# Vi-Sri/CerebralSignalNetworks

Measured on AMD Instinct MI355X. Metric: EEG-segments/sec training (128ch x 500, hidden=768), higher is better.
Workload: dtype bf16

## Files before the change

### cerebralsignalnetworks_amd/cabi.py

```python
import ctypes
import os

import torch

_HERE = os.path.dirname(os.path.abspath(__file__))
LIB_PATH = os.environ.get("CSN_LIB_PATH") or os.path.join(_HERE, "lib", "libcsn_hip.so")

CSN_F32, CSN_BF16 = 0, 1
STATUS_TIMEOUT, STATUS_NONFINITE, STATUS_STALE_SLOT = 1, 2, 4
ABI_VERSION = 6
LSTM_STATE = 0x100
GRAD_OVERWRITE, GRAD_ACCUMULATE = 0, 1

_c_void_p, _c_int, _c_i64, _c_size_t, _c_float = (ctypes.c_void_p, ctypes.c_int, ctypes.c_int64,
                                                  ctypes.c_size_t, ctypes.c_float)


class LstmDesc(ctypes.Structure):
    _fields_ = [("B", ctypes.c_int32), ("T", ctypes.c_int32), ("I", ctypes.c_int32),
                ("H", ctypes.c_int32), ("L", ctypes.c_int32), ("dtype", ctypes.c_int32)]


SIGNATURES = {
    "csn_abi_version": (_c_int, []),
    "csn_last_error": (ctypes.c_char_p, []),
    "csn_target_arch": (ctypes.c_char_p, []),
    "csn_eeg_bandpass_znorm": (_c_int, [_c_void_p, _c_int, _c_int, _c_int, ctypes.POINTER(ctypes.c_double), _c_int,
                                        _c_int, _c_void_p, _c_int, _c_int, _c_void_p]),
    "csn_eeg_filtfilt_scratch_bytes": (_c_size_t, [_c_int, _c_int, _c_int, _c_int]),
    "csn_eeg_filtfilt": (_c_int, [_c_void_p, _c_int, _c_int, _c_int, ctypes.POINTER(ctypes.c_double), _c_int,
                                  _c_void_p, _c_void_p, _c_void_p]),
    "csn_lstm_plan_create": (_c_int, [ctypes.POINTER(LstmDesc), _c_int, ctypes.POINTER(_c_void_p)]),
    "csn_lstm_plan_destroy": (None, [_c_void_p]),
    "csn_lstm_plan_workspace_bytes": (_c_size_t, [_c_void_p]),
    "csn_lstm_plan_path": (_c_int, [_c_void_p]),
    "csn_lstm_plan_dgates_copies": (_c_int, [_c_void_p]),
    "csn_lstm_plan_half_tile_launches": (_c_int, [_c_void_p, _c_int]),
    "csn_lstm_plan_kernel_name": (ctypes.c_char_p, [_c_void_p, _c_int]),
    "csn_lstm_plan_set_grad_callback": (_c_int, [_c_void_p, _c_void_p, _c_void_p]),
    "csn_lstm_plan_set_grad_mode": (_c_int, [_c_void_p, _c_int]),
    "csn_lstm_plan_set_lengths": (_c_int, [_c_void_p, ctypes.POINTER(ctypes.c_int32)]),
    "csn_lstm_workspace_bytes": (_c_size_t, [ctypes.POINTER(LstmDesc), _c_int]),
    "csn_lstm_forward": (_c_int, [_c_void_p, _c_void_p, _c_i64, _c_i64,
                                  ctypes.POINTER(_c_void_p), ctypes.POINTER(_c_void_p),
                                  ctypes.POINTER(_c_void_p), ctypes.POINTER(_c_void_p),
                                  _c_void_p, _c_void_p,
                                  _c_void_p, _c_void_p, _c_void_p,
                                  _c_void_p, _c_void_p, _c_void_p]),
    "csn_lstm_backward": (_c_int, [_c_void_p, _c_void_p, _c_void_p,
                                   _c_void_p, _c_void_p,
                                   _c_void_p,
                                   ctypes.POINTER(_c_void_p), ctypes.POINTER(_c_void_p),
                                   ctypes.POINTER(_c_void_p), ctypes.POINTER(_c_void_p),
                                   _c_void_p, _c_void_p, _c_void_p, _c_void_p]),
    "csn_lstm_workspace_init": (_c_int, [_c_void_p, _c_void_p, _c_void_p]),
    "csn_lstm_status_clear": (_c_int, [_c_void_p, _c_void_p, _c_void_p]),
    "csn_lstm_status_read": (_c_int, [_c_void_p, _c_void_p, ctypes.POINTER(_c_int)]),
    "csn_lstm_status_raise": (_c_int, [_c_void_p, _c_void_p, _c_void_p]),
    "csn_lstm_profile_enable": (_c_int, [_c_void_p, _c_int]),
    "csn_lstm_profile_read": (_c_int, [_c_void_p, ctypes.POINTER(ctypes.c_double), ctypes.POINTER(_c_int),
                                       ctypes.POINTER(_c_int), ctypes.POINTER(ctypes.c_double), ctypes.POINTER(_c_int),
                                       ctypes.POINTER(_c_int)]),
    "csn_gemm_nt": (_c_int, [_c_void_p, _c_void_p, _c_void_p, _c_void_p, _c_i64, _c_i64, _c_i64,
                             _c_int, _c_int, _c_int, _c_void_p]),
    "csn_gemm_tn_scratch_bytes": (_c_size_t, [_c_i64, _c_i64, _c_i64]),
    "csn_gemm_tn": (_c_int, [_c_void_p, _c_void_p, _c_void_p, _c_i64, _c_i64, _c_i64, _c_int, _c_void_p, _c_void_p]),
    "csn_lstm_cell_forward": (_c_int, [_c_void_p, _c_void_p, _c_void_p, _c_i64, _c_void_p, _c_void_p, _c_void_p,
                                       _c_void_p, _c_int, _c_int, _c_int, _c_void_p]),
    "csn_lstm_cell_backward": (_c_int, [_c_void_p, _c_void_p, _c_void_p, _c_i64, _c_void_p, _c_void_p, _c_void_p,
                                        _c_void_p, _c_void_p, _c_int, _c_int, _c_int, _c_void_p]),
    "csn_cosine_loss_scratch_bytes": (_c_size_t, [_c_int]),
    "csn_cosine_loss": (_c_int, [_c_void_p, _c_void_p, _c_int, _c_int, _c_void_p, _c_void_p, _c_float, _c_void_p, _c_void_p]),
    "csn_rmsprop_step": (_c_int, [_c_void_p, _c_void_p, _c_void_p, _c_i64, _c_float, _c_float, _c_float, _c_void_p]),
    "csn_barlow_offdiag_sqsum": (_c_int, [_c_void_p, _c_int, _c_void_p, _c_void_p]),
    "csn_l2_topk_scratch_bytes": (_c_size_t, [_c_i64, _c_i64]),
    "csn_l2_topk": (_c_int, [_c_void_p, _c_void_p, _c_i64, _c_i64, _c_int, _c_int, _c_void_p, _c_void_p,
                             _c_void_p, _c_void_p]),
}


GRAD_READY_FN = ctypes.CFUNCTYPE(None, ctypes.c_void_p, ctypes.c_int)


class CsnError(RuntimeError):
    pass


_lib = None


def load():
    global _lib
    if _lib is not None:
        return _lib
    if not os.path.exists(LIB_PATH):
        raise CsnError(f"{LIB_PATH} not found: build it with `python -c 'import __graft_entry__ as g; g.build()'` "
                       "(there is no CPU fallback)")
    lib = ctypes.CDLL(LIB_PATH, mode=ctypes.RTLD_LOCAL)
    for name, (res, args) in SIGNATURES.items():
        fn = getattr(lib, name)
        fn.restype, fn.argtypes = res, args
    if lib.csn_abi_version() != ABI_VERSION:
        raise CsnError(f"libcsn_hip.so ABI {lib.csn_abi_version()} != binding ABI {ABI_VERSION}")
    _lib = lib
    return lib


def _check(rc):
    if rc != 0:
        raise CsnError(f"libcsn_hip status {rc}: {load().csn_last_error().decode()}")


def _ptr(t):
    return None if t is None else ctypes.c_void_p(t.data_ptr())


def _stream():
    return ctypes.c_void_p(torch.cuda.current_stream().cuda_stream)


def _dt(dtype):
    if dtype in (torch.float32, "f32", "float32", CSN_F32):
        return CSN_F32
    if dtype in (torch.bfloat16, "bf16", "bfloat16", CSN_BF16):
        return CSN_BF16
    raise CsnError(f"unsupported dtype {dtype}")


def torch_dtype(code):
    return torch.bfloat16 if code == CSN_BF16 else torch.float32

# ... 73 lines not shown
    return h_out, c_out, gates


def lstm_cell_backward(dgates_next, w_hh_t, dy, gates, c, c_prev, dc_carry):
    _need_cuda(gates, c, dc_carry)
    B, G = gates.shape
    H = G // 4
    out = torch.empty_like(gates)
    _check(load().csn_lstm_cell_backward(_ptr(dgates_next), _ptr(w_hh_t), _ptr(dy), H, _ptr(gates), _ptr(c),
                                         _ptr(c_prev), _ptr(dc_carry), _ptr(out), B, H, _dt(gates.dtype), _stream()))
    return out


def _ptr_array(tensors):
    arr = (ctypes.c_void_p * len(tensors))()
    for i, t in enumerate(tensors):
        arr[i] = t.data_ptr()
    return arr


class LstmPlan:

    def __init__(self, B, T, I, H, L, dtype, device, training=True, state=False):
        self.desc = LstmDesc(B, T, I, H, L, _dt(dtype))
        self.training = bool(training)
        self.state = bool(state)
        self.device = torch.device(device)
        lib = load()
        handle = _c_void_p()
        with torch.cuda.device(self.device):
            _check(lib.csn_lstm_plan_create(ctypes.byref(self.desc), int(self.training) | (LSTM_STATE if self.state else 0),
                                            ctypes.byref(handle)))
        self._plan = handle
        nbytes = lib.csn_lstm_plan_workspace_bytes(self._plan)
        self.workspace = torch.empty(nbytes + 256, dtype=torch.uint8, device=self.device)
        off = (-self.workspace.data_ptr()) % 256
        self._ws_ptr = ctypes.c_void_p(self.workspace.data_ptr() + off)
        self.busy = False
        with torch.cuda.device(self.device):
            _check(lib.csn_lstm_workspace_init(self._plan, self._ws_ptr, _stream()))

    def __del__(self):
        plan, self._plan = getattr(self, "_plan", None), None
        if plan and _lib is not None:
            _lib.csn_lstm_plan_destroy(plan)

    def key(self):
        d = self.desc
        return (d.B, d.T, d.I, d.H, d.L, d.dtype, self.training) + ((True,) if self.state else ())

    def path(self):
        return load().csn_lstm_plan_path(self._plan)

    def kernel_names(self):
        lib = load()
        return tuple((lib.csn_lstm_plan_kernel_name(self._plan, k) or b"").decode() for k in (0, 1))

    def set_grad_callback(self, fn):
        if getattr(self, "_grad_cb_fn", None) is fn and (fn is None or getattr(self, "_grad_cb", None) is not None):
            return
        self._grad_cb_fn = fn
        self._grad_cb = GRAD_READY_FN(lambda _user, layer: fn(int(layer))) if fn is not None else None
        _check(load().csn_lstm_plan_set_grad_callback(self._plan, ctypes.cast(self._grad_cb, _c_void_p) if fn is not None
                                                      else None, None))

    def set_grad_mode(self, accumulate):
        _check(load().csn_lstm_plan_set_grad_mode(self._plan, GRAD_ACCUMULATE if accumulate else GRAD_OVERWRITE))

    def set_lengths(self, lengths):
        if lengths is None:
            _check(load().csn_lstm_plan_set_lengths(self._plan, None))
            return
        vals = [int(v) for v in (lengths.tolist() if isinstance(lengths, torch.Tensor) else lengths)]
        if len(vals) != self.desc.B:
            raise CsnError(f"LSTM lengths: {len(vals)} entries for a batch of {self.desc.B}")
        _check(load().csn_lstm_plan_set_lengths(self._plan, (ctypes.c_int32 * len(vals))(*vals)))

    def dgates_copies(self):
        return load().csn_lstm_plan_dgates_copies(self._plan)

    def half_tile_launches(self, which):
        return load().csn_lstm_plan_half_tile_launches(self._plan, which)

    def forward(self, x_bti, w_ih, w_hh, b_ih, b_hh, want_all=False, h0=None, c0=None, want_state=False):
        d = self.desc
        _need_cuda(x_bti)
        if x_bti.dtype != torch.float32 or x_bti.stride(2) != 1:
            x_bti = x_bti.float().contiguous()
        assert x_bti.shape == (d.B, d.T, d.I), (tuple(x_bti.shape), (d.B, d.T, d.I))
        y_last = torch.empty((d.B, d.H), dtype=torch.float32, device=x_bti.device)
        y_all = torch.empty((d.B, d.T, d.H), dtype=torch.float32, device=x_bti.device) if want_all else None
        ws = [[p.detach() for p in group] for group in (w_ih, w_hh, b_ih, b_hh)]
        for group in ws:
            for p in group:
                assert p.dtype == torch.float32 and p.is_contiguous() and p.is_cuda
        h0, c0 = self._state_in(h0), self._state_in(c0)
        h_n = torch.empty((d.L, d.B, d.H), dtype=torch.float32, device=x_bti.device) if want_state else None
        c_n = torch.empty((d.L, d.B, d.H), dtype=torch.float32, device=x_bti.device) if want_state else None
        with torch.cuda.device(self.device):
            _check(load().csn_lstm_forward(self._plan, _ptr(x_bti), x_bti.stride(0), x_bti.stride(1),
                                           _ptr_array(ws[0]), _ptr_array(ws[1]), _ptr_array(ws[2]), _ptr_array(ws[3]),
                                           _ptr(h0), _ptr(c0), self._ws_ptr, _ptr(y_last), _ptr(y_all),
                                           _ptr(h_n), _ptr(c_n), _stream()))
        if want_state:
            return y_last, y_all, h_n, c_n
        return y_last, y_all

    def _state_in(self, t):
        if t is None:
            return None
        d = self.desc
        t = t.detach()
        if tuple(t.shape) != (d.L, d.B, d.H):
            raise CsnError(f"LSTM state must be [L, B, H] = {[d.L, d.B, d.H]}, got {list(t.shape)}")
        return t.to(device=self.device, dtype=torch.float32).contiguous()

    def backward(self, dy_last, dy_all, grads, dx=None, dh_n=None, dc_n=None, dh0=None, dc0=None):
        if dy_last is not None:
            dy_last = dy_last.float().contiguous()
        if dy_all is not None:
            dy_all = dy_all.float().contiguous()
        dh_n, dc_n = self._state_in(dh_n), self._state_in(dc_n)
        for out in (dh0, dc0):
            if out is not None:
                assert out.dtype == torch.float32 and out.is_contiguous() and out.shape == (self.desc.L, self.desc.B,
                                                                                            self.desc.H)
        with torch.cuda.device(self.device):
            _check(load().csn_lstm_backward(self._plan, _ptr(dy_last), _ptr(dy_all), _ptr(dh_n), _ptr(dc_n), self._ws_ptr,
                                            _ptr_array(grads[0]), _ptr_array(grads[1]), _ptr_array(grads[2]),
                                            _ptr_array(grads[3]), _ptr(dx), _ptr(dh0), _ptr(dc0), _stream()))

    def clear_status(self):
        with torch.cuda.device(self.device):
            _check(load().csn_lstm_status_clear(self._plan, self._ws_ptr, _stream()))

    def inject_timeout(self):
        with torch.cuda.device(self.device):
            _check(load().csn_lstm_status_raise(self._plan, self._ws_ptr, _stream()))

    def status(self, clear=False):
        out = _c_int(0)
        _check(load().csn_lstm_status_read(self._plan, self._ws_ptr, ctypes.byref(out)))
        if clear and out.value != 0:
            self.clear_status()
        return out.value

    def profile_enable(self, on=True):
        _check(load().csn_lstm_profile_enable(self._plan, int(on)))

    def profile_read(self):
        fm, bm = ctypes.c_double(), ctypes.c_double()
        fl, fc, bl, bc = _c_int(), _c_int(), _c_int(), _c_int()
        _check(load().csn_lstm_profile_read(self._plan, ctypes.byref(fm), ctypes.byref(fl), ctypes.byref(fc),
                                            ctypes.byref(bm), ctypes.byref(bl), ctypes.byref(bc)))
        return dict(fwd_ms=fm.value, fwd_launches=fl.value, fwd_cells=fc.value,
                    bwd_ms=bm.value, bwd_launches=bl.value, bwd_cells=bc.value)


def cosine_loss(student, teacher, want_grad=True, grad_scale=1.0):
    _need_cuda(student, teacher)
    s, t = student.float().contiguous(), teacher.float().contiguous()
    B, D = s.shape
    loss = torch.empty(1, dtype=torch.float32, device=s.device)
    ds = torch.empty_like(s) if want_grad else None
    lib = load()
    scratch = torch.empty(lib.csn_cosine_loss_scratch_bytes(B) // 8, dtype=torch.float64, device=s.device)
    with torch.cuda.device(s.device):
        _check(lib.csn_cosine_loss(_ptr(s), _ptr(t), B, D, _ptr(loss), _ptr(ds), float(grad_scale), _ptr(scratch), _stream()))
    return loss, ds


def rmsprop_step(params_flat, grads_flat, square_avg_flat, lr, alpha=0.99, eps=1e-8):
    _need_cuda(params_flat, grads_flat, square_avg_flat)
    n = params_flat.numel()
    assert grads_flat.numel() == n and square_avg_flat.numel() == n
    assert params_flat.dtype == grads_flat.dtype == square_avg_flat.dtype == torch.float32
    with torch.cuda.device(params_flat.device):
        _check(load().csn_rmsprop_step(_ptr(params_flat), _ptr(grads_flat), _ptr(square_avg_flat), n, float(lr), float(alpha),
                                       float(eps), _stream()))


def barlow_offdiag_sqsum(c):
    _need_cuda(c)
    if c.dim() != 2 or c.shape[0] != c.shape[1]:
        raise CsnError(f"barlow_offdiag_sqsum expects a square matrix, got shape {tuple(c.shape)}")
    c = c.float().contiguous()
# ... 18 lines not shown
```

### cerebralsignalnetworks_amd/csrc/csn_common.h

```cpp
#pragma once
#include <hip/hip_runtime.h>
#include <stdint.h>
#include <stdio.h>
#include <stdlib.h>
#include <atomic>
#include <string>

#include "../../include/csn_hip.h"

namespace csn {

typedef __bf16 bf16_t;
typedef __attribute__((ext_vector_type(8))) __bf16 bf16x8;
typedef __attribute__((ext_vector_type(4))) __bf16 bf16x4;
typedef __attribute__((ext_vector_type(4))) float f32x4;
typedef __attribute__((ext_vector_type(4))) short s16x4;

void set_error(const std::string& msg);
int fail(int status, const char* fmt, ...);

#define CSN_HIP_CHECK(expr)                                                              \
  do {                                                                                   \
    hipError_t _e = (expr);                                                              \
    if (_e != hipSuccess)                                                                \
      return ::csn::fail(CSN_ERR_HIP, "%s failed: %s (%s:%d)", #expr, hipGetErrorString(_e), \
                         __FILE__, __LINE__);                                            \
  } while (0)

#define CSN_LAUNCH_CHECK()                                                               \
  do {                                                                                   \
    hipError_t _e = hipGetLastError();                                                   \
    if (_e != hipSuccess)                                                                \
      return ::csn::fail(CSN_ERR_HIP, "kernel launch failed: %s (%s:%d)",                \
                         hipGetErrorString(_e), __FILE__, __LINE__);                     \
  } while (0)

#define CSN_REQUIRE(cond, ...)                                                           \
  do {                                                                                   \
    if (!(cond)) return ::csn::fail(CSN_ERR_INVALID_ARGUMENT, __VA_ARGS__);              \
  } while (0)

struct Options {
  bool cell_v1, no_persist, no_persist_bwd, persist_streams, no_xcd_local, no_rotate, no_fuse_x, no_beside,
      no_side_stream, gemm_slot, fwd_ksplit, fwd_nsplit, fwd_flags, bwd_flags, dpoll_no_hint, fwd_hint, gemm_no_dma, gemm_no_256, gemm_generic, gemm_lds64, tn_no_tr, tn_no_stagger, filter_v1, tags_no_rearm, gemm_no_192, no_half_tiles;
  int chunk;
  int tn_stages;
  int fwd_nk;
};
static inline Options options_from_env() {
  auto on = [](const char* name) { return getenv(name) != nullptr; };
  auto num = [](const char* name, int dflt) {
    const char* e = getenv(name);
    return e ? atoi(e) : dflt;
  };
  Options o{};
  o.cell_v1 = on("CSN_CELL_V1");
  o.no_persist = on("CSN_NO_PERSIST");
  o.no_persist_bwd = on("CSN_NO_PERSIST_BWD");
  o.persist_streams = on("CSN_PERSIST_STREAMS");
  o.no_xcd_local = on("CSN_NO_XCD_LOCAL");
  o.no_rotate = on("CSN_NO_ROTATE");
  o.no_fuse_x = on("CSN_NO_FUSE_X");
  o.no_beside = on("CSN_NO_BESIDE");
  o.no_half_tiles = on("CSN_NO_HALF_TILES");
  o.no_side_stream = on("CSN_NO_SIDE_STREAM");
  o.gemm_slot = on("CSN_GEMM_SLOT");
  o.fwd_ksplit = on("CSN_FWD_KSPLIT");
  o.fwd_nsplit = on("CSN_FWD_NSPLIT");
  o.fwd_flags = on("CSN_FWD_FLAGS");
  o.bwd_flags = on("CSN_BWD_FLAGS");
  o.dpoll_no_hint = on("CSN_DPOLL_NO_HINT");
  o.fwd_hint = on("CSN_FWD_HINT");
  o.tn_no_stagger = on("CSN_TN_NO_STAGGER");
  o.gemm_no_dma = on("CSN_GEMM_NO_DMA");
  o.gemm_no_256 = on("CSN_GEMM_NO_256");
  o.gemm_no_192 = on("CSN_GEMM_NO_192");
  o.gemm_generic = on("CSN_GEMM_GENERIC");
  o.gemm_lds64 = on("CSN_GEMM_LDS64");
  o.tn_no_tr = on("CSN_TN_NO_TR");
  o.filter_v1 = on("CSN_FILTER_V1");
#ifdef CSN_SLAB_TAGS
  o.tags_no_rearm = on("CSN_TAGS_NO_REARM");
#endif
  o.chunk = num("CSN_LSTM_CHUNK", 32);
  if (o.chunk < 1) o.chunk = 1;
  o.tn_stages = num("CSN_TN_STAGES", 4);
  o.fwd_nk = num("CSN_FWD_NK", 1);
  return o;
}

static inline hipStream_t as_stream(csnStream_t s) { return reinterpret_cast<hipStream_t>(s); }
template <auto Kernel>
static int ensure_dyn_lds(int bytes) {
  static std::atomic<unsigned> done{0u};
  int dev = 0;
  CSN_HIP_CHECK(hipGetDevice(&dev));
  const unsigned bit = 1u << (dev & 31);
  if ((done.load(std::memory_order_acquire) & bit) == 0u) {
    CSN_HIP_CHECK(hipFuncSetAttribute(reinterpret_cast<const void*>(Kernel), hipFuncAttributeMaxDynamicSharedMemorySize, bytes));
    done.fetch_or(bit, std::memory_order_release);
  }
  return CSN_OK;
}

static inline size_t align_up(size_t v, size_t a) { return (v + a - 1) / a * a; }
static inline size_t dtype_size(int dtype) { return dtype == CSN_BF16 ? 2 : 4; }

__device__ __forceinline__ float to_f32(float v) { return v; }
__device__ __forceinline__ float to_f32(bf16_t v) { return (float)v; }
template <typename T> __device__ __forceinline__ T from_f32(float v);
template <> __device__ __forceinline__ float from_f32<float>(float v) { return v; }
template <> __device__ __forceinline__ bf16_t from_f32<bf16_t>(float v) { return (bf16_t)v; }

__device__ __forceinline__ float sigmoid_f32(float x) { return 1.0f / (1.0f + expf(-x)); }
__device__ __forceinline__ float tanh_f32(float x) { return tanhf(x); }

struct CellFwdOne {
  const void* h_prev; const void* w_hh; const float* xproj; int64_t xproj_ld; const float* c_prev;
  void* gates_out; float* c_out; void* h_out;
};
struct CellFwdBatch { CellFwdOne p[4]; };
struct CellBwdOne {
  const void* dg_next; const void* w_hh_t; const float* dy; int64_t dy_ld; const void* gates; const float* c;
  const float* c_prev; float* dc_carry; void* dg_out;
};
struct CellBwdBatch { CellBwdOne p[4]; };
struct CellMask {
  const int* lengths;
  int t[4];
};
struct CellNoMask {};
template <bool MASK> struct CellMaskArg { typedef CellNoMask type; };
template <> struct CellMaskArg<true> { typedef CellMask type; };
int launch_cell_fwd_batch(const CellFwdBatch& b, int np, int B, int H, int dtype, hipStream_t st);
int launch_cell_bwd_batch(const CellBwdBatch& b, int np, int B, int H, int dtype, hipStream_t st,
                          const CellMask* mask = nullptr);

int launch_cast_strided(const float* src, int64_t s0, int64_t s1, int64_t n0, int64_t n1, int64_t n2,
                        void* dst, int dtype, hipStream_t st);
int launch_transpose_cast(const float* src, int64_t R, int64_t C, void* dst, int dtype, hipStream_t st);
int launch_cast(const float* src, void* dst, int64_t n, int dtype, hipStream_t st);
int launch_upcast(const void* src, int dtype, float* dst, int64_t n, hipStream_t st);
int launch_add_vec(const float* a, const float* b, float* out, int64_t n, hipStream_t st);
int launch_reduce_slabs(const float* slabs, int64_t stride, int S, float* out, float* out2, int64_t n, int accumulate,
                        hipStream_t st);
size_t colsum_scratch_bytes(int64_t N);
int launch_colsum(const void* X, int64_t R, int64_t N, int dtype, float* out, float* out2, int accumulate, void* scratch,
// ... 13 lines not shown
```

### cerebralsignalnetworks_amd/csrc/lstm.hip

```cpp
#include <algorithm>
#include <cstring>
#include <vector>

#include "csn_common.h"
#include "lstm_cell_blk.h"
#include "lstm_cell_common.h"
#include "lstm_f32_persist.h"

namespace csn {

int launch_cell_fwd(const void* h_prev, const void* w_hh, const float* xproj, int64_t xproj_ld, const float* c_prev,
                    void* gates_out, float* c_out, void* h_out, int B, int H, int dtype, hipStream_t st);
int launch_cell_bwd(const void* dg_next, const void* w_hh_t, const float* dy, int64_t dy_ld, const void* gates,
                    const float* c, const float* c_prev, float* dc_carry, void* dg_out, int B, int H, int dtype,
                    hipStream_t st);

struct LayerWs {
  size_t wih, whh, whht, wiht, whh_blk, whht_blk, bias, xproj, gates, c_all, h_all, dgates, dx, dc_carry, hblk[2],
      dgblk[2], h_blk_all, counters, dg_blk_all, bflags;
};
struct WsLayout {
  LayerWs layer[8];
  size_t x_c, x_blk, wih0_blk, dy_tm, tn_scratch, colsum, status, agree, agree_b, zeros_bh, f32_bias_part, total;
  size_t zero_fwd, zero_fwd_bytes, zero_bwd, zero_bwd_bytes;
  bool fuse_x;
  bool il, persist, persist_bwd;
  bool fwd_ns;
  bool f32_persist;
};

static bool whole_chip() {
  int dev = 0, cus = 0;
  if (hipGetDevice(&dev) != hipSuccess) return false;
  return hipDeviceGetAttribute(&cus, hipDeviceAttributeMultiprocessorCount, dev) == hipSuccess && cus >= 256;
}

static WsLayout make_layout(const csnLstmDesc& d, int training, const Options& opt) {
  WsLayout w{};
  w.il = cell_blk_supported(d.H, d.dtype, opt);
  const bool slabs_fit = ((size_t)d.T + 1) * (((size_t)d.B + 63) / 64 * 64) * (size_t)d.H * 8 < ((size_t)1 << 32);
  w.fwd_ns = w.il && fwd_ns_supported(d.B, d.H, d.dtype, opt) && d.L <= 4;
  w.persist = w.fwd_ns || (w.il && slabs_fit && fwd_persist_supported(d.B, d.H, d.dtype, opt) && d.L <= 4);
  w.persist_bwd = w.persist && slabs_fit && training && bwd_persist_supported(d.B, d.H, d.dtype, opt);
  size_t off = 0;
  const size_t es = dtype_size(d.dtype);
  auto take = [&](size_t bytes) {
    size_t o = off;
    off += align_up(bytes, 256);
    return o;
  };
  const size_t TB = (size_t)d.T * d.B, H = d.H, G = 4 * (size_t)d.H;
  const size_t Bpad = ((size_t)d.B + 63) / 64 * 64;
  size_t tn_bytes = 0;
  for (int l = 0; l < d.L; ++l) {
    const size_t I = l == 0 ? d.I : d.H;
    LayerWs& L = w.layer[l];
    L.wih = take(G * I * es);
    L.wiht = take(G * I * es);
    L.bias = take(G * 4);
    if (w.il) {
      L.whh_blk = take(G * H * 2);
      L.whht_blk = take(G * H * 2);
      L.hblk[0] = take(Bpad * H * 2);
      L.hblk[1] = take(Bpad * H * 2);
      if (w.persist) L.h_blk_all = take(((size_t)(d.T < 3 ? 3 : d.T) + 1) * Bpad * H * 2);
    } else {
      L.whh = take(G * H * es);
      L.whht = take(G * H * es);
    }
    L.xproj = take(TB * G * 4);
    L.gates = take(TB * G * es);
    L.c_all = take((TB + d.B) * H * 4);
    L.h_all = take((TB + d.B) * H * es);
    if (training) {
      L.dgates = take(TB * G * es);
      L.dx = take(TB * I * 4);
      if (!w.persist_bwd) L.dc_carry = take((size_t)d.B * H * 4);
      if (w.il) {
        L.dgblk[0] = take(Bpad * G * 2);
        L.dgblk[1] = take(Bpad * G * 2);
      }
      if (w.persist_bwd) L.dg_blk_all = take((size_t)(d.T < 4 ? 4 : d.T) * Bpad * G * 2);
    }
    size_t a = gemm_tn_scratch_bytes(G, I, TB, opt), b = gemm_tn_scratch_bytes(G, H, TB, opt);
    if (a > tn_bytes) tn_bytes = a;
    if (b > tn_bytes) tn_bytes = b;
  }
  w.x_c = take(TB * d.I * es);
  w.status = take(256);
  w.fuse_x = w.persist && !opt.no_fuse_x &&
             (w.fwd_ns ? d.I == 128 : (d.I % 32 == 0 && d.I <= 128 && d.H != 512));
  if (w.fuse_x) {
    w.x_blk = take((size_t)d.T * Bpad * d.I * 2);
    w.wih0_blk = take(G * d.I * 2);
  }
  if (w.persist_bwd) w.zeros_bh = take((size_t)d.B * H * 4);
  w.f32_persist = !w.il && d.dtype == CSN_F32 && !opt.no_persist && !opt.cell_v1 && f32_persist_supported(d.B, d.H) && whole_chip();
  if (w.f32_persist) {
    const size_t MTt = Bpad / 64;
    w.zero_fwd = off;
    for (int l = 0; l < d.L; ++l) w.layer[l].counters = take(((size_t)d.T + 1) * MTt * kF32FlagLine * 4);
    w.zero_fwd_bytes = off - w.zero_fwd;
    for (int l = 0; l < d.L; ++l) w.layer[l].h_blk_all = take(((size_t)d.T + 1) * Bpad * H * 4);
    if (training) {
      for (int l = 0; l < d.L; ++l) w.layer[l].dg_blk_all = take((size_t)d.T * Bpad * G * 4);
      w.zeros_bh = take((size_t)d.B * H * 4);
      w.f32_bias_part = take(MTt * 4 * G * 4);
      w.zero_bwd = off;
      for (int l = 0; l < d.L; ++l) w.layer[l].bflags = take((size_t)d.T * MTt * kF32FlagLine * 4);
      w.zero_bwd_bytes = off - w.zero_bwd;
    }
  }
  if (w.persist) {
    w.zero_fwd = off;
    for (int l = 0; l < d.L; ++l) w.layer[l].counters = take(((size_t)d.T + 1) * (Bpad / 64) * 4 * kPersistFlagLine * 4);
    w.agree = take(((size_t)d.T + 8) * 8 * sizeof(unsigned long long));
    w.zero_fwd_bytes = off - w.zero_fwd;
  }
  if (w.persist_bwd) {
    w.zero_bwd = off;
    for (int l = 0; l < d.L; ++l) {
      w.layer[l].dc_carry = take((size_t)d.B * H * 4);
      w.layer[l].bflags = take((size_t)d.T * (Bpad / 64) * 3 * kPersistFlagLine * 4);
    }
    w.agree_b = take(((size_t)d.T + 8) * 8 * sizeof(unsigned long long));
    w.zero_bwd_bytes = off - w.zero_bwd;
  }
  if (training) {
    w.dy_tm = take(TB * H * 4);
    w.tn_scratch = take(tn_bytes);
    w.colsum = take(colsum_scratch_bytes(G));
  }
  w.total = off;
  return w;
}

static int check_desc(const char* fn, const csnLstmDesc* d) {
  CSN_REQUIRE(d != nullptr, "%s: null descriptor", fn);
  CSN_REQUIRE(d->B > 0 && d->T > 0 && d->I > 0 && d->H > 0, "%s: bad shape B=%d T=%d I=%d H=%d", fn, d->B, d->T,
              d->I, d->H);
  CSN_REQUIRE(d->L >= 1 && d->L <= 8, "%s: L=%d outside 1..8", fn, d->L);
  CSN_REQUIRE(d->H % 32 == 0, "%s: H=%d must be a multiple of 32", fn, d->H);
  CSN_REQUIRE(d->dtype == CSN_F32 || d->dtype == CSN_BF16, "%s: bad dtype %d", fn, d->dtype);
  return CSN_OK;
}

template <typename T>
__global__ void gather_y_all_kernel(const T* __restrict__ h_all, float* __restrict__ y, int B, int Tn, int H) {
  const int64_t total = (int64_t)B * Tn * H;
  const int64_t stride = (int64_t)gridDim.x * blockDim.x;
  for (int64_t i = (int64_t)blockIdx.x * blockDim.x + threadIdx.x; i < total; i += stride) {
    const int64_t h = i % H, r = i / H, t = r % Tn, b = r / Tn;
    y[i] = to_f32(h_all[((t + 1) * B + b) * (int64_t)H + h]);
  }
}

__global__ void bt_to_tb_kernel(const float* __restrict__ src, float* __restrict__ dst, int B, int Tn, int H) {
  const int64_t total = (int64_t)B * Tn * H;
  const int64_t stride = (int64_t)gridDim.x * blockDim.x;
  for (int64_t i = (int64_t)blockIdx.x * blockDim.x + threadIdx.x; i < total; i += stride) {
    const int64_t h = i % H, r = i / H, b = r % B, t = r / B;
    dst[i] = src[(b * Tn + t) * (int64_t)H + h];
  }
}

__global__ void tb_to_bt_kernel(const float* __restrict__ src, float* __restrict__ dst, int B, int Tn, int H) {
  const int64_t total = (int64_t)B * Tn * H;
// ... 137 lines not shown
  hipStream_t layer[8] = {nullptr};
  std::vector<hipEvent_t> events;
  size_t next = 0;
};

static int side_ctx(SideCtx& c) {
  if (c.side == nullptr) {
    CSN_HIP_CHECK(hipStreamCreateWithFlags(&c.side, hipStreamNonBlocking));
    for (int l = 1; l < 8; ++l) CSN_HIP_CHECK(hipStreamCreateWithFlags(&c.layer[l], hipStreamNonBlocking));
  }
  c.next = 0;
  return CSN_OK;
}
static int next_event(SideCtx* c, hipEvent_t* ev) {
  if (c->next == c->events.size()) {
    hipEvent_t e;
    CSN_HIP_CHECK(hipEventCreateWithFlags(&e, hipEventDisableTiming));
    c->events.push_back(e);
  }
  *ev = c->events[c->next++];
  return CSN_OK;
}
static int hand_off(SideCtx* c, hipStream_t from, hipStream_t to) {
  hipEvent_t ev;
  if (int rc = next_event(c, &ev)) return rc;
  CSN_HIP_CHECK(hipEventRecord(ev, from));
  CSN_HIP_CHECK(hipStreamWaitEvent(to, ev, 0));
  return CSN_OK;
}

struct Prof {
  bool on = false;
  hipEvent_t ev[4] = {nullptr, nullptr, nullptr, nullptr};
  int launches[2] = {0, 0}, cells[2] = {0, 0};
  bool have[2] = {false, false};
  std::vector<hipEvent_t> pair[2];
  size_t pairs_used[2] = {0, 0};
};
static int prof_mark(Prof& g_prof, int which, hipStream_t st) {
  if (!g_prof.on) return CSN_OK;
  if ((which & 1) == 0) g_prof.pairs_used[which >> 1] = 0;
  if (g_prof.ev[which] == nullptr) CSN_HIP_CHECK(hipEventCreate(&g_prof.ev[which]));
  CSN_HIP_CHECK(hipEventRecord(g_prof.ev[which], st));
  return CSN_OK;
}

static int prof_pair(Prof& g_prof, int k, bool end, hipStream_t st) {
  if (!g_prof.on) return CSN_OK;
  const size_t i = 2 * g_prof.pairs_used[k] + (end ? 1 : 0);
  while (g_prof.pair[k].size() <= i) {
    hipEvent_t e;
    CSN_HIP_CHECK(hipEventCreate(&e));
    g_prof.pair[k].push_back(e);
  }
  CSN_HIP_CHECK(hipEventRecord(g_prof.pair[k][i], st));
  if (end) ++g_prof.pairs_used[k];
  return CSN_OK;
}

}

struct csnLstmPlan {
  csnLstmDesc d;
  int training;
  int state;
  bool state_seen = false;
  int device;
  csn::Options opt;
  csn::WsLayout w;
  csn::SideCtx sc;
  csn::Prof prof;
  int dgates_copies = 0;
  int half_launches[2] = {0, 0};
  csnGradReadyFn grad_cb = nullptr;
  void* grad_cb_user = nullptr;
  int grad_accumulate = 0;
  std::vector<int32_t> lengths;
  int t_eff = 0;
  int T_full = 0;
  const int* dlen = nullptr;
  int32_t* len_dev = nullptr;
  int32_t* len_pin = nullptr;
  hipEvent_t len_ev = nullptr;
  void grads_ready(int layer) const {
    if (grad_cb != nullptr) grad_cb(grad_cb_user, layer);
  }
};

using namespace csn;
typedef csnLstmPlan Plan;

extern "C" int csn_lstm_plan_create(const csnLstmDesc* d, int training, csnLstmPlan** out) {
  if (int rc = check_desc("csn_lstm_plan_create", d)) return rc;
  CSN_REQUIRE(out != nullptr, "csn_lstm_plan_create: null output pointer");
  Plan* P = new Plan();
  P->d = *d;
  P->state = (training & CSN_LSTM_STATE) != 0;
  P->training = (training & ~CSN_LSTM_STATE) != 0;
  if (hipGetDevice(&P->device) != hipSuccess) {
    delete P;
    return fail(CSN_ERR_HIP, "csn_lstm_plan_create: hipGetDevice failed");
  }
  P->opt = options_from_env();
  if (P->state && d->dtype == CSN_F32) P->opt.no_persist = true;
  {
    const unsigned long long Bp = ((unsigned long long)d->B + 63) / 64 * 64;
    const unsigned long long per_step = std::max({(unsigned long long)d->B * d->H * 16ull, Bp * (unsigned long long)d->I * 2ull, Bp * (unsigned long long)d->H * 2ull});
    const unsigned long long cmax = ((1ull << 32) - 1ull) / per_step;
    if (cmax >= 3 && (unsigned long long)P->opt.chunk > cmax - 2) P->opt.chunk = (int)(cmax - 2);
  }
  P->w = make_layout(*d, P->training, P->opt);
  P->T_full = d->T;
  *out = P;
  return CSN_OK;
}

extern "C" void csn_lstm_plan_destroy(csnLstmPlan* P) {
  if (P == nullptr) return;
  int cur = 0;
  const bool switched = hipGetDevice(&cur) == hipSuccess && cur != P->device && hipSetDevice(P->device) == hipSuccess;
  for (hipEvent_t e : P->sc.events) (void)hipEventDestroy(e);
  if (P->sc.side) (void)hipStreamDestroy(P->sc.side);
  for (int l = 1; l < 8; ++l)
    if (P->sc.layer[l]) (void)hipStreamDestroy(P->sc.layer[l]);
  for (int i = 0; i < 4; ++i)
    if (P->prof.ev[i]) (void)hipEventDestroy(P->prof.ev[i]);
  for (int k = 0; k < 2; ++k)
    for (hipEvent_t e : P->prof.pair[k]) (void)hipEventDestroy(e);
  if (P->len_ev) (void)hipEventDestroy(P->len_ev);
  if (P->len_pin) (void)hipHostFree(P->len_pin);
  if (P->len_dev) (void)hipFree(P->len_dev);
  if (switched) (void)hipSetDevice(cur);
  delete P;
}

extern "C" size_t csn_lstm_plan_workspace_bytes(const csnLstmPlan* P) { return P ? P->w.total : 0; }

extern "C" int csn_lstm_plan_path(const csnLstmPlan* P) {
  if (P == nullptr) return -1;
  return P->w.f32_persist ? 4 : (P->w.persist_bwd ? 3 : (P->w.persist ? 2 : (P->w.il ? 1 : 0)));
}

extern "C" int csn_lstm_plan_dgates_copies(const csnLstmPlan* P) { return P == nullptr ? -1 : P->dgates_copies; }

extern "C" int csn_lstm_plan_half_tile_launches(const csnLstmPlan* P, int which) {
  return (P == nullptr || which < 0 || which > 1) ? -1 : P->half_launches[which];
}

static bool bwd_grouped(const csnLstmPlan* P) {
  if (!P->w.persist_bwd) return false;
  const int MTg = (P->d.B + 63) / 64, nchg = (P->d.T + P->opt.chunk - 1) / P->opt.chunk;
  const int slots = P->d.L < nchg ? P->d.L : nchg;
  return slots <= 4 && slots * MTg <= 8 && !P->opt.persist_streams;
}

extern "C" const char* csn_lstm_plan_kernel_name(const csnLstmPlan* P, int which) {
  if (P == nullptr) return nullptr;
  const bool ks = (P->d.dtype == CSN_F32 ? P->d.H % 128 == 0 : P->d.H % 256 == 0);
  if (P->w.f32_persist) return which == 0 ? "lstm_fwd_f32_persist_kernel" : (which == 1 ? "lstm_bwd_f32_persist_kernel" : nullptr);
  if (which == 0) {
    if (P->w.fwd_ns) return "lstm_fwd_ns_kernel";
    if (P->w.persist) return "lstm_fwd_persist_kernel";
    if (P->w.il) return "lstm_cell_fwd_il_kernel";
    return ks ? "lstm_cell_fwd_ks_kernel" : "lstm_cell_fwd_kernel";
  }
  if (which == 1) {
    if (bwd_grouped(P)) return "lstm_bwd_persist_kernel";
    if (P->w.il) return "lstm_cell_bwd_il_kernel";
    return ks ? "lstm_cell_bwd_ks_kernel" : "lstm_cell_bwd_kernel";
  }
  return nullptr;
}

extern "C" int csn_lstm_plan_set_grad_callback(csnLstmPlan* P, csnGradReadyFn fn, void* user) {
  CSN_REQUIRE(P != nullptr, "csn_lstm_plan_set_grad_callback: null plan");
  P->grad_cb = fn;
  P->grad_cb_user = fn ? user : nullptr;
  return CSN_OK;
}

extern "C" int csn_lstm_plan_set_grad_mode(csnLstmPlan* P, int mode) {
  CSN_REQUIRE(P != nullptr, "csn_lstm_plan_set_grad_mode: null plan");
  CSN_REQUIRE(mode == CSN_GRAD_OVERWRITE || mode == CSN_GRAD_ACCUMULATE, "csn_lstm_plan_set_grad_mode: unknown mode %d", mode);
  P->grad_accumulate = mode == CSN_GRAD_ACCUMULATE;
  return CSN_OK;
}

extern "C" int csn_lstm_plan_set_lengths(csnLstmPlan* P, const int32_t* lengths) {
  CSN_REQUIRE(P != nullptr, "csn_lstm_plan_set_lengths: null plan");
  CSN_REQUIRE(P->state, "csn_lstm_plan_set_lengths: the plan was created without CSN_LSTM_STATE");
  if (lengths == nullptr) {
    P->lengths.clear();
    P->t_eff = 0;
    return CSN_OK;
  }
  int longest = 0;
  for (int b = 0; b < P->d.B; ++b) {
    CSN_REQUIRE(lengths[b] >= 0 && lengths[b] <= P->d.T, "csn_lstm_plan_set_lengths: lengths[%d] = %d outside [0, %d]", b,
                (int)lengths[b], P->d.T);
    longest = std::max(longest, (int)lengths[b]);
  }
  P->lengths.assign(lengths, lengths + P->d.B);
  P->t_eff = longest;
  return CSN_OK;
}

struct EffectiveT {
  csnLstmDesc& d;
  const int T;
  EffectiveT(csnLstmDesc& d_, int Te) : d(d_), T(d_.T) { d.T = Te; }
  ~EffectiveT() { d.T = T; }
};
static int upload_lengths(csnLstmPlan* P, hipStream_t st) {
  P->dlen = nullptr;
  if (P->lengths.empty()) return CSN_OK;
  const size_t bytes = (size_t)P->d.B * 4;
  if (P->len_pin == nullptr) {
    CSN_HIP_CHECK(hipMalloc((void**)&P->len_dev, bytes));
    CSN_HIP_CHECK(hipHostMalloc((void**)&P->len_pin, bytes, hipHostMallocDefault));
    CSN_HIP_CHECK(hipEventCreateWithFlags(&P->len_ev, hipEventDisableTiming));
  } else {
    CSN_HIP_CHECK(hipEventSynchronize(P->len_ev));
  }
  memcpy(P->len_pin, P->lengths.data(), bytes);
  CSN_HIP_CHECK(hipMemcpyAsync(P->len_dev, P->len_pin, bytes, hipMemcpyHostToDevice, st));
  CSN_HIP_CHECK(hipEventRecord(P->len_ev, st));
  P->dlen = P->len_dev;
  return CSN_OK;
}
static int emit_dx(const csnLstmPlan& P, const float* dx_tm, float* dx, int64_t I, hipStream_t st) {
  const int B = P.d.B, T = P.d.T;
// ... 27 lines not shown
              "csn_lstm_profile_read: null pointer");
  Prof& g_prof = P->prof;
  *fwd_ms = *bwd_ms = 0.0;
  *fwd_launches = *fwd_cells = *bwd_launches = *bwd_cells = 0;
  for (int k = 0; k < 2; ++k) {
    if (!g_prof.have[k]) continue;
    float ms = 0.f;
    CSN_HIP_CHECK(hipEventSynchronize(g_prof.ev[2 * k + 1]));
    if (g_prof.pairs_used[k] > 0) {
      for (size_t i = 0; i < g_prof.pairs_used[k]; ++i) {
        float one = 0.f;
        CSN_HIP_CHECK(hipEventElapsedTime(&one, g_prof.pair[k][2 * i], g_prof.pair[k][2 * i + 1]));
        ms += one;
      }
    } else {
      CSN_HIP_CHECK(hipEventElapsedTime(&ms, g_prof.ev[2 * k], g_prof.ev[2 * k + 1]));
    }
    (k == 0 ? *fwd_ms : *bwd_ms) = ms;
    (k == 0 ? *fwd_launches : *bwd_launches) = g_prof.launches[k];
    (k == 0 ? *fwd_cells : *bwd_cells) = g_prof.cells[k];
  }
  return CSN_OK;
}

extern "C" int csn_lstm_workspace_init(const csnLstmPlan* P, void* workspace, csnStream_t stream) {
  CSN_REQUIRE(P && workspace, "csn_lstm_workspace_init: null pointer");
  CSN_REQUIRE((reinterpret_cast<uintptr_t>(workspace) & 255) == 0, "csn_lstm_workspace_init: workspace must be 256-B aligned");
  hipStream_t st = as_stream(stream);
  char* ws = (char*)workspace;
  const WsLayout& w = P->w;
  const size_t es = dtype_size(P->d.dtype);
  CSN_HIP_CHECK(hipMemsetAsync(ws + w.status, 0, 256, st));
  for (int l = 0; l < P->d.L; ++l) {
    CSN_HIP_CHECK(hipMemsetAsync(ws + w.layer[l].h_all, 0, (size_t)P->d.B * P->d.H * es, st));
    CSN_HIP_CHECK(hipMemsetAsync(ws + w.layer[l].c_all, 0, (size_t)P->d.B * P->d.H * 4, st));
  }
  if (w.persist_bwd || (w.f32_persist && P->training))
    CSN_HIP_CHECK(hipMemsetAsync(ws + w.zeros_bh, 0, (size_t)P->d.B * P->d.H * 4, st));
  return CSN_OK;
}

extern "C" int csn_lstm_status_clear(const csnLstmPlan* P, void* workspace, csnStream_t stream) {
  CSN_REQUIRE(P && workspace, "csn_lstm_status_clear: null pointer");
  CSN_HIP_CHECK(hipMemsetAsync((char*)workspace + P->w.status, 0, 256, as_stream(stream)));
  return CSN_OK;
}
extern "C" int csn_lstm_status_raise(const csnLstmPlan* P, void* workspace, csnStream_t stream) {
  CSN_REQUIRE(P && workspace, "csn_lstm_status_raise: null pointer");
  CSN_HIP_CHECK(hipMemsetAsync((char*)workspace + P->w.status, 1, 1, as_stream(stream)));
  return CSN_OK;
}
extern "C" int csn_lstm_status_read(const csnLstmPlan* P, const void* workspace, int* status) {
  CSN_REQUIRE(P && workspace && status, "csn_lstm_status_read: null pointer");
  unsigned flag[3] = {0u, 0u, 0u};
  CSN_HIP_CHECK(hipMemcpy(flag, (const char*)workspace + P->w.status, sizeof(flag), hipMemcpyDeviceToHost));
  *status = (flag[0] ? CSN_STATUS_TIMEOUT : 0) | (flag[1] ? CSN_STATUS_NONFINITE : 0) | (flag[2] ? CSN_STATUS_STALE_SLOT : 0);
#ifdef CSN_SLAB_TAGS
  if (flag[2] && getenv("CSN_TAGS_VERBOSE")) {
    unsigned dbg[24];
    CSN_HIP_CHECK(hipMemcpy(dbg, (const char*)workspace + P->w.status + 28, sizeof(dbg), hipMemcpyDeviceToHost));
    if (dbg[0])
      fprintf(stderr, "stale piece (backward): t=%u step-in-launch=%u group=%u slice=%u wave=%u lane=%u kb*4+rg=%u u0=%08x local=%u redone=%u "
              "single=%u phase=%u rot=%u nsteps=%u xcc=%u lanes=%u\n", dbg[1], dbg[2], dbg[3], dbg[4], dbg[5], dbg[6], dbg[7], dbg[8],
              dbg[9], dbg[10], dbg[11], dbg[12], dbg[13], dbg[14], dbg[15], dbg[16]);
  }
#endif
  return CSN_OK;
}

extern "C" size_t csn_lstm_workspace_bytes(const csnLstmDesc* d, int training) {
  if (check_desc("csn_lstm_workspace_bytes", d) != CSN_OK) return 0;
  Options opt = options_from_env();
  if ((training & CSN_LSTM_STATE) && d->dtype == CSN_F32) opt.no_persist = true;
  return make_layout(*d, (training & ~CSN_LSTM_STATE) != 0, opt).total;
}

static int gemm_tn_full(const void* A, const void* B, float* C, int64_t M, int64_t N, int64_t K, int dtype, void* scratch,
                        int accumulate, hipStream_t st, const Options& opt) {
  int S = 1;
  if (int rc = launch_gemm_tn_slabs(A, B, (float*)scratch, M, N, K, dtype, st, &S, nullptr, nullptr, opt)) return rc;
  return launch_reduce_slabs((const float*)scratch, M * N, S, C, nullptr, M * N, accumulate, st);
}

static int mask_x(const csnLstmPlan& P, char* ws, hipStream_t st) {
  if (P.dlen == nullptr) return CSN_OK;
  const csnLstmDesc& d = P.d;
  const int64_t n = (int64_t)d.T * d.B * d.I;
  if (d.dtype == CSN_BF16) mask_tm_kernel<bf16_t><<<grid_for(n), 256, 0, st>>>((bf16_t*)(ws + P.w.x_c), P.dlen, d.B, d.T, d.I);
  else mask_tm_kernel<float><<<grid_for(n), 256, 0, st>>>((float*)(ws + P.w.x_c), P.dlen, d.B, d.T, d.I);
  CSN_LAUNCH_CHECK();
  if (P.w.fuse_x) {
    const int64_t Bpad = ((int64_t)d.B + 63) / 64 * 64;
    mask_x_blk_kernel<<<grid_for((int64_t)d.T * Bpad * d.I / 8), 256, 0, st>>>((bf16_t*)(ws + P.w.x_blk), P.dlen, d.B, Bpad, d.T, d.I);
    CSN_LAUNCH_CHECK();
  }
  return CSN_OK;
}

static int forward_v1(Plan& P, char* ws, const float* x, int64_t xsb, int64_t xst,
                      const float* const* w_ih, const float* const* w_hh, const float* const* b_ih,
                      const float* const* b_hh, const float* h0, const float* c0, int training, csnStream_t stream) {
  const csnLstmDesc* d = &P.d;
  const WsLayout& w = P.w;
  hipStream_t st = as_stream(stream);
  const int B = d->B, T = d->T, H = d->H, dt = d->dtype, NL = d->L;
  const int64_t G = 4 * (int64_t)H, TB = (int64_t)T * B;
  const size_t es = dtype_size(dt);
  const int Cz = P.opt.chunk, lag = Cz;
  int rc;
  if ((rc = launch_cast_strided(x, xsb, xst, B, T, d->I, ws + w.x_c, dt, st))) return rc;
  if ((rc = mask_x(P, ws, st))) return rc;
  for (int l = 0; l < NL; ++l) {
    const LayerWs& L = w.layer[l];
    const int64_t I = l == 0 ? d->I : H;
    if ((rc = launch_cast(w_ih[l], ws + L.wih, G * I, dt, st))) return rc;
    if ((rc = launch_cast(w_hh[l], ws + L.whh, G * H, dt, st))) return rc;
    if (training) {
      if ((rc = launch_transpose_cast(w_hh[l], G, H, ws + L.whht, dt, st))) return rc;
      if ((rc = launch_transpose_cast(w_ih[l], G, I, ws + L.wiht, dt, st))) return rc;
    }
    if ((rc = launch_add_vec(b_ih[l], b_hh[l], (float*)(ws + L.bias), G, st))) return rc;
    if (h0) {
      if ((rc = launch_cast(h0 + (size_t)l * B * H, ws + L.h_all, (int64_t)B * H, dt, st))) return rc;
    } else {
      CSN_HIP_CHECK(hipMemsetAsync(ws + L.h_all, 0, (size_t)B * H * es, st));
    }
    if (c0)
      CSN_HIP_CHECK(hipMemcpyAsync(ws + L.c_all, c0 + (size_t)l * B * H, (size_t)B * H * 4, hipMemcpyDeviceToDevice, st));
    else
      CSN_HIP_CHECK(hipMemsetAsync(ws + L.c_all, 0, (size_t)B * H * 4, st));
  }
  if ((rc = gemm_nt(ws + w.x_c, ws + w.layer[0].wih, (const float*)(ws + w.layer[0].bias), ws + w.layer[0].xproj, TB, G,
                    d->I, dt, CSN_F32, 0, st, P.opt)))
    return rc;
  const int D = T + lag * (NL - 1);
  for (int dg = 0; dg < D; ++dg) {
    CellFwdBatch b{};
    int np = 0;
    for (int l = 0; l < NL; ++l) {
      const int t = dg - lag * l;
      if (t < 0 || t >= T) continue;
      const LayerWs& L = w.layer[l];
      if (np == 4) {
        if ((rc = launch_cell_fwd_batch(b, np, B, H, dt, st))) return rc;
        np = 0;
      }
      b.p[np++] = CellFwdOne{ws + L.h_all + (size_t)t * B * H * es, ws + L.whh, (const float*)(ws + L.xproj) + (size_t)t * B * G, G,
                             (const float*)(ws + L.c_all) + (size_t)t * B * H,
                             training ? ws + L.gates + (size_t)t * B * G * es : nullptr,
                             (float*)(ws + L.c_all) + (size_t)(t + 1) * B * H, ws + L.h_all + (size_t)(t + 1) * B * H * es};
    }
    if (np > 0 && (rc = launch_cell_fwd_batch(b, np, B, H, dt, st))) return rc;
    for (int l = 0; l + 1 < NL; ++l) {
      const int t = dg - lag * l;
      if (t < 0 || t >= T || ((t + 1) % Cz != 0 && t != T - 1)) continue;
      const int t0 = (t / Cz) * Cz, nsteps = t - t0 + 1;
      const LayerWs& Ln = w.layer[l + 1];
      if ((rc = gemm_nt(ws + w.layer[l].h_all + (size_t)(t0 + 1) * B * H * es, ws + Ln.wih, (const float*)(ws + Ln.bias),
                        (float*)(ws + Ln.xproj) + (size_t)t0 * B * G, (int64_t)nsteps * B, G, H, dt, CSN_F32, 0, st, P.opt)))
        return rc;
    }
  }
  return CSN_OK;
}

static int backward_v1(Plan& P, char* ws, const float* dy_last, const float* dy_tm, const float* dh_n, const float* dc_n,
                       float* const* dw_ih, float* const* dw_hh, float* const* db_ih, float* const* db_hh, float* dx,
                       csnStream_t stream) {
  const csnLstmDesc* d = &P.d;
  const WsLayout& w = P.w;
  hipStream_t st = as_stream(stream);
  const int B = d->B, T = d->T, H = d->H, dt = d->dtype, NL = d->L;
  const int64_t G = 4 * (int64_t)H, TB = (int64_t)T * B;
  const size_t es = dtype_size(dt);
  const int Cz = P.opt.chunk, lag = Cz;
  const int acc = P.grad_accumulate;
  int rc;
  for (int l = 0; l < NL; ++l) {
    if (dc_n)
      CSN_HIP_CHECK(hipMemcpyAsync(ws + w.layer[l].dc_carry, dc_n + (size_t)l * B * H, (size_t)B * H * 4, hipMemcpyDeviceToDevice, st));
    else
      CSN_HIP_CHECK(hipMemsetAsync(ws + w.layer[l].dc_carry, 0, (size_t)B * H * 4, st));
  }
  const int D = T + lag * (NL - 1);
  for (int dg = 0; dg < D; ++dg) {
    CellBwdBatch b{};
    CellMask mask{P.dlen, {0, 0, 0, 0}};
    const CellMask* mk = P.dlen ? &mask : nullptr;
    int np = 0;
    for (int l = NL - 1; l >= 0; --l) {
      const int r = dg - lag * (NL - 1 - l);
      if (r < 0 || r >= T) continue;
      const int t = T - 1 - r;
      const LayerWs& L = w.layer[l];
      const bool top = (l == NL - 1);
      if (np == 4) {
        if ((rc = launch_cell_bwd_batch(b, np, B, H, dt, st, mk))) return rc;
        np = 0;
      }
      mask.t[np] = t;
      const float* dy_t = top ? (dy_tm ? dy_tm + (size_t)t * B * H : (t == T - 1 ? dy_last : nullptr))
                              : (const float*)(ws + w.layer[l + 1].dx) + (size_t)t * B * H;
      b.p[np++] = CellBwdOne{(t == T - 1) ? nullptr : (const void*)(ws + L.dgates + (size_t)(t + 1) * B * G * es), ws + L.whht, dy_t, H,
                             ws + L.gates + (size_t)t * B * G * es, (const float*)(ws + L.c_all) + (size_t)(t + 1) * B * H,
                             (const float*)(ws + L.c_all) + (size_t)t * B * H, (float*)(ws + L.dc_carry),
                             ws + L.dgates + (size_t)t * B * G * es};
    }
    if (np > 0 && (rc = launch_cell_bwd_batch(b, np, B, H, dt, st, mk))) return rc;
    for (int l = NL - 1; l >= 1; --l) {
      const int r = dg - lag * (NL - 1 - l);
      if (r < 0 || r >= T || ((r + 1) % Cz != 0 && r != T - 1)) continue;
      const int t_lo = T - 1 - r, t_hi = T - 1 - (r / Cz) * Cz;
      const LayerWs& L = w.layer[l];
      if ((rc = gemm_nt(ws + L.dgates + (size_t)t_lo * B * G * es, ws + L.wiht, nullptr, (float*)(ws + L.dx) + (size_t)t_lo * B * H,
                        (int64_t)(t_hi - t_lo + 1) * B, H, G, dt, CSN_F32, 0, st, P.opt)))
        return rc;
      if (dh_n && (rc = add_dh_n_rows(P, dh_n + (size_t)(l - 1) * B * H, (float*)(ws + L.dx), t_lo, t_hi, st))) return rc;
    }
  }
  for (int l = NL - 1; l >= 0; --l) {
    const LayerWs& L = w.layer[l];
    const int64_t I = l == 0 ? d->I : H;
    const void* inp = l == 0 ? (const void*)(ws + w.x_c)
                             : (const void*)(ws + w.layer[l - 1].h_all + (size_t)B * H * es);
    if ((rc = gemm_tn_full(ws + L.dgates, ws + L.h_all, dw_hh[l], G, H, TB, dt, ws + w.tn_scratch, acc, st, P.opt))) return rc;
    if ((rc = gemm_tn_full(ws + L.dgates, inp, dw_ih[l], G, I, TB, dt, ws + w.tn_scratch, acc, st, P.opt))) return rc;
    if ((rc = launch_colsum(ws + L.dgates, TB, G, dt, db_ih[l], db_hh[l], acc, ws + w.colsum, st))) return rc;
    P.grads_ready(l);
  }
  if (dx) {
    const LayerWs& L = w.layer[0];
    if ((rc = gemm_nt(ws + L.dgates, ws + L.wiht, nullptr, ws + L.dx, TB, d->I, G, dt, CSN_F32, 0, st, P.opt))) return rc;
    if ((rc = emit_dx(P, (const float*)(ws + L.dx), dx, d->I, st))) return rc;
  }
  return CSN_OK;
}

static int forward_f32p(Plan& P, char* ws, const float* x, int64_t xsb, int64_t xst,
                        const float* const* w_ih, const float* const* w_hh, const float* const* b_ih,
                        const float* const* b_hh, int training, csnStream_t stream) {
  const csnLstmDesc* d = &P.d;
  const WsLayout& w = P.w;
  Prof& g_prof = P.prof;
  hipStream_t st = as_stream(stream);
  const int B = d->B, T = d->T, H = d->H, NL = d->L;
  const int64_t G = 4 * (int64_t)H, TB = (int64_t)T * B;
  const int MTt = (B + 63) / 64, per = f32_persist_tiles_per_launch(H);
  int rc;
  if ((rc = launch_cast_strided(x, xsb, xst, B, T, d->I, ws + w.x_c, CSN_F32, st))) return rc;
  for (int l = 0; l < NL; ++l) {
    const LayerWs& L = w.layer[l];
    const int64_t I = l == 0 ? d->I : H;
    if ((rc = launch_cast(w_ih[l], ws + L.wih, G * I, CSN_F32, st))) return rc;
    if ((rc = launch_cast(w_hh[l], ws + L.whh, G * H, CSN_F32, st))) return rc;
    if (training) {
      if ((rc = launch_transpose_cast(w_hh[l], G, H, ws + L.whht, CSN_F32, st))) return rc;
      if ((rc = launch_transpose_cast(w_ih[l], G, I, ws + L.wiht, CSN_F32, st))) return rc;
    }
    if ((rc = launch_add_vec(b_ih[l], b_hh[l], (float*)(ws + L.bias), G, st))) return rc;
    CSN_HIP_CHECK(hipMemsetAsync(ws + L.h_all, 0, (size_t)B * H * 4, st));
    CSN_HIP_CHECK(hipMemsetAsync(ws + L.c_all, 0, (size_t)B * H * 4, st));
  }
  CSN_HIP_CHECK(hipMemsetAsync(ws + w.zero_fwd, 0, w.zero_fwd_bytes, st));
  int n_launch = 0;
  if ((rc = prof_mark(g_prof, 0, st))) return rc;
  for (int l = 0; l < NL; ++l) {
    const LayerWs& L = w.layer[l];
    const void* inp = l == 0 ? (const void*)(ws + w.x_c) : (const void*)(ws + w.layer[l - 1].h_all + (size_t)B * H * 4);
    if ((rc = gemm_nt(inp, ws + L.wih, (const float*)(ws + L.bias), ws + L.xproj, TB, G, l == 0 ? d->I : H, CSN_F32, CSN_F32, 0, st, P.opt)))
      return rc;
    F32PersistFwdArgs a{};
    a.w_hh = (const float*)(ws + L.whh);
    a.xproj = (const float*)(ws + L.xproj);
    a.gates = training ? (float*)(ws + L.gates) : nullptr;
    a.c_all = (float*)(ws + L.c_all);
    a.h_all = (float*)(ws + L.h_all);
    a.h_blk = (float*)(ws + L.h_blk_all);
    a.flags = (unsigned*)(ws + L.counters);
    a.error_flag = (unsigned*)(ws + w.status);
    a.B = B; a.T = T; a.MT_total = MTt;
    for (int m = 0; m < MTt; m += per) {
      a.mt0 = m;
      a.MT = MTt - m < per ? MTt - m : per;
      if ((rc = prof_pair(g_prof, 0, false, st))) return rc;
      if ((rc = launch_fwd_f32_persist(a, H, st))) return rc;
      if ((rc = prof_pair(g_prof, 0, true, st))) return rc;
      ++n_launch;
    }
  }
  if ((rc = prof_mark(g_prof, 1, st))) return rc;
  g_prof.launches[0] = n_launch;
  g_prof.cells[0] = T * NL;
  g_prof.have[0] = g_prof.on;
  return CSN_OK;
}

static int backward_f32p(Plan& P, char* ws, const float* dy_last, const float* dy_tm,
                         float* const* dw_ih, float* const* dw_hh, float* const* db_ih, float* const* db_hh, float* dx,
                         csnStream_t stream) {
  const csnLstmDesc* d = &P.d;
  const WsLayout& w = P.w;
  Prof& g_prof = P.prof;
  hipStream_t st = as_stream(stream);
  const int B = d->B, T = d->T, H = d->H, NL = d->L;
  const int64_t G = 4 * (int64_t)H, TB = (int64_t)T * B;
  const int MTt = (B + 63) / 64, per = f32_persist_tiles_per_launch(H);
  int rc;
  CSN_HIP_CHECK(hipMemsetAsync(ws + w.zero_bwd, 0, w.zero_bwd_bytes, st));
  int n_launch = 0;
  if ((rc = prof_mark(g_prof, 2, st))) return rc;
  for (int l = NL - 1; l >= 0; --l) {
    const LayerWs& L = w.layer[l];
    const bool top = (l == NL - 1);
    F32PersistBwdArgs a{};
    a.w_hh_t = (const float*)(ws + L.whht);
    a.gates = (const float*)(ws + L.gates);
    a.c_all = (const float*)(ws + L.c_all);
    a.dy = top ? dy_tm : (const float*)(ws + w.layer[l + 1].dx);
    a.dy_last = (top && dy_tm == nullptr) ? dy_last : nullptr;
    a.zeros = (const float*)(ws + w.zeros_bh);
    a.dgates = (float*)(ws + L.dgates);
    a.dg_blk = (float*)(ws + L.dg_blk_all);
    a.bias_part = (float*)(ws + w.f32_bias_part);
    a.flags = (unsigned*)(ws + L.bflags);
    a.error_flag = (unsigned*)(ws + w.status);
    a.B = B; a.T = T; a.MT_total = MTt;
    for (int m = 0; m < MTt; m += per) {
      a.mt0 = m;
      a.MT = MTt - m < per ? MTt - m : per;
      if ((rc = prof_pair(g_prof, 1, false, st))) return rc;
      if ((rc = launch_bwd_f32_persist(a, H, st))) return rc;
      if ((rc = prof_pair(g_prof, 1, true, st))) return rc;
      ++n_launch;
    }
    sum_rows_kernel<<<(unsigned)((G + 255) / 256), 256, 0, st>>>((const float*)(ws + w.f32_bias_part), MTt * 4, G, db_ih[l], db_hh[l], P.grad_accumulate);
    CSN_LAUNCH_CHECK();
    if (l > 0 && (rc = gemm_nt(ws + L.dgates, ws + L.wiht, nullptr, ws + L.dx, TB, H, G, CSN_F32, CSN_F32, 0, st, P.opt))) return rc;
  }
  if ((rc = prof_mark(g_prof, 3, st))) return rc;
  g_prof.launches[1] = n_launch;
  g_prof.cells[1] = T * NL;
  g_prof.have[1] = g_prof.on;
  for (int l = NL - 1; l >= 0; --l) {
    const LayerWs& L = w.layer[l];
    const int64_t I = l == 0 ? d->I : H;
    const void* inp = l == 0 ? (const void*)(ws + w.x_c) : (const void*)(ws + w.layer[l - 1].h_all + (size_t)B * H * 4);
    if ((rc = gemm_tn_full(ws + L.dgates, ws + L.h_all, dw_hh[l], G, H, TB, CSN_F32, ws + w.tn_scratch, P.grad_accumulate, st, P.opt))) return rc;
    if ((rc = gemm_tn_full(ws + L.dgates, inp, dw_ih[l], G, I, TB, CSN_F32, ws + w.tn_scratch, P.grad_accumulate, st, P.opt))) return rc;
    P.grads_ready(l);
  }
  if (dx) {
    const LayerWs& L = w.layer[0];
    if ((rc = gemm_nt(ws + L.dgates, ws + L.wiht, nullptr, ws + L.dx, TB, d->I, G, CSN_F32, CSN_F32, 0, st, P.opt))) return rc;
    tb_to_bt_kernel<<<grid_for(TB * d->I), 256, 0, st>>>((const float*)(ws + L.dx), dx, B, T, d->I);
    CSN_LAUNCH_CHECK();
  }
  return CSN_OK;
}

static int forward_persist(Plan& P, char* ws, const float* h0, const float* c0, int training, hipStream_t st, SideCtx* sc,
                           hipStream_t side);

static int forward_il(Plan& P, char* ws, const float* x, int64_t xsb, int64_t xst,
                      const float* const* w_ih, const float* const* w_hh, const float* const* b_ih,
                      const float* const* b_hh, const float* h0, const float* c0, int training, csnStream_t stream) {
  const csnLstmDesc* d = &P.d;
  const WsLayout& w = P.w;
  Prof& g_prof = P.prof;
  hipStream_t st = as_stream(stream);
  SideCtx* sc = &P.sc;
  int rc;
  if ((rc = side_ctx(P.sc))) return rc;
  hipStream_t side = P.opt.no_side_stream ? st : sc->side;
  const int B = d->B, T = d->T, H = d->H, NL = d->L;
  const int64_t G = 4 * (int64_t)H, TB = (int64_t)T * B;
  const size_t Bpad = ((size_t)B + 63) / 64 * 64;
  const int Cz = P.opt.chunk, lag = 2 * Cz;

  PrepArgs pa{};
  int prep_rc = CSN_OK;
  auto job = [&](int kind, const float* a_, const float* b_, void* dst, int64_t n0, int64_t n1, int64_t n2, int64_t s0,
                 int64_t s1, int64_t Hh, int pr, int pk, int64_t work) {
    if (prep_rc != CSN_OK) return;
    if (pa.njobs == kPrepMaxJobs) {
      if ((prep_rc = launch_prep_multi(pa, st)) != CSN_OK) return;
      pa.njobs = 0;
    }
    PrepJob& J = pa.job[pa.njobs++];
    J = PrepJob{kind, a_, b_, dst, n0, n1, n2, s0, s1, Hh, pr, pk, work, 0u, 0u};
  };
  job(kPrepCastX, x, nullptr, ws + w.x_c, B, T, d->I, xsb, xst, 0, 0, 0, TB * d->I);
  for (int l = 0; l < NL; ++l) {
    const LayerWs& L = w.layer[l];
    const int64_t I = l == 0 ? d->I : H;
    job(kPrepPermRows, w_ih[l], nullptr, ws + L.wih, 0, I, 0, 0, 0, H, 0, 0, G * I);
    job(kPrepBlockify, w_hh[l], nullptr, ws + L.whh_blk, G, H, 0, H, 1, H, 1, 0, G * H / 8);
    job(kPrepBias, b_ih[l], b_hh[l], ws + L.bias, 0, 0, 0, 0, 0, H, 0, 0, G);
    if (training) {
      job(kPrepTransPerm, w_ih[l], nullptr, ws + L.wiht, 0, I, 0, 0, 0, H, 0, 0, G * I);
      job(kPrepBlockify, w_hh[l], nullptr, ws + L.whht_blk, H, G, 0, 1, H, H, 0, 1, H * G / 8);
    }
    if (!w.persist) {
      CSN_HIP_CHECK(hipMemsetAsync(ws + L.hblk[0], 0, Bpad * H * 2, st));
      CSN_HIP_CHECK(hipMemsetAsync(ws + L.hblk[1], 0, Bpad * H * 2, st));
      CSN_HIP_CHECK(hipMemsetAsync(ws + L.h_all, 0, (size_t)B * H * 2, st));
      CSN_HIP_CHECK(hipMemsetAsync(ws + L.c_all, 0, (size_t)B * H * 4, st));
      if (h0) {
        if ((rc = launch_blockify_x(h0 + (size_t)l * B * H, H, 0, B, 1, H, ws + L.hblk[0], st))) return rc;
        if ((rc = launch_cast(h0 + (size_t)l * B * H, ws + L.h_all, (int64_t)B * H, CSN_BF16, st))) return rc;
      }
      if (c0)
        CSN_HIP_CHECK(hipMemcpyAsync(ws + L.c_all, c0 + (size_t)l * B * H, (size_t)B * H * 4, hipMemcpyDeviceToDevice, st));
    }
  }
  if (w.fuse_x) {
    job(kPrepBlockifyX, x, nullptr, ws + w.x_blk, B, T, d->I, xsb, xst, (int64_t)Bpad, 0, 0, (int64_t)T * Bpad * d->I / 8);
    job(kPrepBlockify, w_ih[0], nullptr, ws + w.wih0_blk, G, d->I, 0, d->I, 1, H, 1, 0, G * d->I / 8);
  }
  if (prep_rc != CSN_OK) return prep_rc;
  if ((rc = launch_prep_multi(pa, st))) return rc;
  if ((rc = mask_x(P, ws, st))) return rc;
  if (!w.fuse_x) {
    if ((rc = gemm_nt(ws + w.x_c, ws + w.layer[0].wih, (const float*)(ws + w.layer[0].bias), ws + w.layer[0].xproj,
                          TB, G, d->I, CSN_BF16, CSN_F32, 0, st, P.opt)))
      return rc;
  }
  if (w.persist) return forward_persist(P, ws, h0, c0, training, st, sc, side);
  if (NL > 1 && (rc = hand_off(sc, st, side))) return rc;

  const int nch = (T + Cz - 1) / Cz;
  std::vector<hipEvent_t> xproj_ready((size_t)NL * nch, nullptr);
  const int D = T + lag * (NL - 1);
  int n_launch = 0, n_cells = 0;
  if ((rc = prof_mark(g_prof, 0, st))) return rc;
  for (int dg = 0; dg < D; ++dg) {
    CellFwdArgs a{};
    a.B = B;
    a.H = H;
    int np = 0;
    for (int l = 0; l < NL; ++l) {
      const int t = dg - lag * l;
      if (t < 0 || t >= T) continue;
      const LayerWs& L = w.layer[l];
      if (np == 4) {
        if ((rc = launch_cell_fwd_il(a, np, st, P.opt.fwd_nk))) return rc;
        ++n_launch;
        n_cells += np;
        np = 0;
      }
      if (l > 0 && t % Cz == 0) CSN_HIP_CHECK(hipStreamWaitEvent(st, xproj_ready[(size_t)l * nch + t / Cz], 0));
      CellFwdProb& P = a.p[np++];
      P.h_prev_blk = (t == 0 && !h0) ? nullptr : (const bf16_t*)(ws + L.hblk[t & 1]);
      P.w_blk = (const bf16_t*)(ws + L.whh_blk);
      P.xproj = (const float*)(ws + L.xproj) + (size_t)t * B * G;
      P.c_prev = (t == 0 && !c0) ? nullptr : (const float*)(ws + L.c_all) + (size_t)t * B * H;
      P.gates_out = training ? (bf16_t*)(ws + L.gates) + (size_t)t * B * G : nullptr;
      P.c_out = (float*)(ws + L.c_all) + (size_t)(t + 1) * B * H;
      P.h_out = (bf16_t*)(ws + L.h_all) + (size_t)(t + 1) * B * H;
      P.h_out_blk = (bf16_t*)(ws + L.hblk[(t + 1) & 1]);
    }
    if (np == 0) continue;
    if ((rc = launch_cell_fwd_il(a, np, st, P.opt.fwd_nk))) return rc;
    ++n_launch;
    n_cells += np;
    for (int l = 0; l + 1 < NL; ++l) {
      const int t = dg - lag * l;
      if (t < 0 || t >= T) continue;
      if ((t + 1) % Cz != 0 && t != T - 1) continue;
      const int c = t / Cz, t0 = c * Cz, nsteps = t - t0 + 1;
      if ((rc = hand_off(sc, st, side))) return rc;
      const LayerWs& Ln = w.layer[l + 1];
      rc = gemm_nt((const bf16_t*)(ws + w.layer[l].h_all) + (size_t)(t0 + 1) * B * H, ws + Ln.wih,
                       (const float*)(ws + Ln.bias), (float*)(ws + Ln.xproj) + (size_t)t0 * B * G,
                       (int64_t)nsteps * B, G, H, CSN_BF16, CSN_F32, 0, side, P.opt);
      if (rc) return rc;
      hipEvent_t ev;
      if ((rc = next_event(sc, &ev))) return rc;
      CSN_HIP_CHECK(hipEventRecord(ev, side));
      xproj_ready[(size_t)(l + 1) * nch + c] = ev;
    }
  }
  if ((rc = prof_mark(g_prof, 1, st))) return rc;
  g_prof.launches[0] = n_launch;
  g_prof.cells[0] = n_cells;
  g_prof.have[0] = g_prof.on;
  return CSN_OK;
}

static int forward_persist(Plan& P, char* ws, const float* h0, const float* c0, int training, hipStream_t st, SideCtx* sc,
                           hipStream_t side) {
  const csnLstmDesc* d = &P.d;
  const WsLayout& w = P.w;
  Prof& g_prof = P.prof;
  const int B = d->B, T = d->T, H = d->H, NL = d->L;
  const int64_t G = 4 * (int64_t)H;
  const int Bpad = (B + 63) / 64 * 64, MT = Bpad / 64;
  const int Cz = P.opt.chunk;
  const int nch = (T + Cz - 1) / Cz;
  int rc;
  CSN_HIP_CHECK(hipMemsetAsync(ws + w.zero_fwd, 0, w.zero_fwd_bytes, st));
  auto fill_slot = [&](PersistFwdSlot& S, int l, int c) {
    const LayerWs& L = w.layer[l];
    S.w_blk = (const bf16_t*)(ws + L.whh_blk);
    S.xproj = (const float*)(ws + L.xproj);
    S.gates = training ? (bf16_t*)(ws + L.gates) : nullptr;
    S.c_all = (float*)(ws + L.c_all);
    S.h_all = (bf16_t*)(ws + L.h_all);
    S.h_blk_all = (bf16_t*)(ws + L.h_blk_all);
    S.flags = (unsigned*)(ws + L.counters);
    S.x_blk = nullptr;
    S.wih_blk = nullptr;
    S.bias = nullptr;
    S.I = 0;
    if (l == 0 && w.fuse_x) {
      S.x_blk = (const bf16_t*)(ws + w.x_blk);
      S.wih_blk = (const bf16_t*)(ws + w.wih0_blk);
      S.bias = (const float*)(ws + L.bias);
      S.I = d->I;
    }
    S.t0 = c * Cz;
    S.nsteps = (S.t0 + Cz <= T) ? Cz : T - S.t0;
  };
  auto xproj_gemm = [&](int l, int c, hipStream_t on) {
    const LayerWs& L = w.layer[l];
    const LayerWs& Ln = w.layer[l + 1];
    const int t0 = c * Cz, nsteps = (t0 + Cz <= T) ? Cz : T - t0;
    return gemm_nt((const bf16_t*)(ws + L.h_all) + (size_t)(t0 + 1) * B * H, ws + Ln.wih,
                       (const float*)(ws + Ln.bias), (float*)(ws + Ln.xproj) + (size_t)t0 * B * G,
                       (int64_t)nsteps * B, G, H, CSN_BF16, CSN_F32, 0, on, P.opt);
  };
  PersistFwdArgs a{};
  a.error_flag = (unsigned*)(ws + w.status);
  a.B = B; a.H = H; a.T = T; a.Bpad = Bpad; a.MT = MT;
  a.rotate = !P.opt.no_rotate;
  a.data_polls = (!w.fwd_ns && !P.opt.fwd_flags) ? (P.opt.fwd_hint && !P.opt.dpoll_no_hint ? 1 : 2) : 0;
#ifdef CSN_SLAB_TAGS
  if (a.data_polls && P.opt.tags_no_rearm) a.data_polls |= 4;
#endif
  if (a.data_polls)
    for (int l = 0; l < NL; ++l)
      CSN_HIP_CHECK(hipMemsetAsync(ws + w.layer[l].h_blk_all, 0xff, (size_t)4 * Bpad * H * 2, st));
  a.state = (h0 || c0) ? 1 : 0;
  if (a.state) P.state_seen = true;
  for (int l = 0; l < NL && P.state_seen; ++l) {
    const LayerWs& L = w.layer[l];
    if (h0) {
      if ((rc = launch_blockify_x(h0 + (size_t)l * B * H, H, 0, B, 1, H, ws + L.h_blk_all, st))) return rc;
      if ((rc = launch_cast(h0 + (size_t)l * B * H, ws + L.h_all, (int64_t)B * H, CSN_BF16, st))) return rc;
    } else {
      if (a.state) CSN_HIP_CHECK(hipMemsetAsync(ws + L.h_blk_all, 0, (size_t)Bpad * H * 2, st));
      CSN_HIP_CHECK(hipMemsetAsync(ws + L.h_all, 0, (size_t)B * H * 2, st));
    }
    if (c0)
      CSN_HIP_CHECK(hipMemcpyAsync(ws + L.c_all, c0 + (size_t)l * B * H, (size_t)B * H * 4, hipMemcpyDeviceToDevice, st));
    else
      CSN_HIP_CHECK(hipMemsetAsync(ws + L.c_all, 0, (size_t)B * H * 4, st));
  }
  int n_launch = 0;
  P.half_launches[0] = 0;

  const int max_slots = NL < nch ? NL : nch;
  const int fwd_slices = w.fwd_ns ? fwd_ns_slices(H) : fwd_persist_slices(H);
  auto launch_fwd = [&](const PersistFwdArgs& args, hipStream_t on) {
    return w.fwd_ns ? launch_fwd_ns(args, on) : launch_fwd_persist(args, on);
  };
  const bool grouped = max_slots <= 4 && max_slots * MT <= 8 && fwd_slices <= 32 &&
                       !P.opt.persist_streams;
  if (grouped) {
    const int ndiag = nch + NL - 1;
    const bool try_local = !P.opt.no_xcd_local;
    if ((rc = prof_mark(g_prof, 0, st))) return rc;
    for (int dg = 0; dg < ndiag; ++dg) {
      int lay[4], chk[4], ns = 0;
      for (int l = 0; l < NL; ++l) {
        const int c = dg - l;
        if (c < 0 || c >= nch) continue;
        lay[ns] = l;
        chk[ns] = c;
        fill_slot(a.slot[ns], l, c);
        ++ns;
      }
      a.nslots = ns;
      a.xcd_groups = 1;
      const bool half = !w.fwd_ns && !P.opt.no_half_tiles && 2 * ns * MT <= 8;
      a.half_tiles = half ? 1 : 0;
      a.MT = half ? 2 * MT : MT;
      if (half) {
        for (int i = 0; i < ns; ++i) a.slot[i].flags += ((size_t)T + 1) * MT * kPersistFlagLine;
        ++P.half_launches[0];
      }
      a.agree = try_local ? (unsigned long long*)(ws + w.agree) + (size_t)dg * 8 : nullptr;
      if ((rc = prof_pair(g_prof, 0, false, st))) return rc;
      if ((rc = launch_fwd(a, st))) return rc;
      if ((rc = prof_pair(g_prof, 0, true, st))) return rc;
      ++n_launch;
      for (int i = 0; i < ns; ++i)
        if (lay[i] + 1 < NL && (rc = xproj_gemm(lay[i], chk[i], st))) return rc;
    }
    if ((rc = prof_mark(g_prof, 1, st))) return rc;
    g_prof.launches[0] = n_launch;
    g_prof.cells[0] = T * NL;
    g_prof.have[0] = g_prof.on;
    return CSN_OK;
  }

  if (NL * fwd_slices * MT > 256) side = st;
  hipStream_t ls[8];
  ls[0] = st;
  for (int l = 1; l < NL; ++l) {
    ls[l] = (side == st) ? st : sc->layer[l];
    if (ls[l] != st && (rc = hand_off(sc, st, ls[l]))) return rc;
  }
  if (side != st && (rc = hand_off(sc, st, side))) return rc;
  const bool gemm_slot = P.opt.gemm_slot;
  if ((rc = prof_mark(g_prof, 0, st))) return rc;
  a.nslots = 1;
  a.xcd_groups = 0;
  a.agree = nullptr;
  a.half_tiles = 0;
  a.MT = MT;
  for (int c = 0; c < nch; ++c) {
    for (int l = 0; l < NL; ++l) {
      fill_slot(a.slot[0], l, c);
      if ((rc = launch_fwd(a, ls[l]))) return rc;
      ++n_launch;
      if (l + 1 < NL) {
        if ((rc = hand_off(sc, ls[l], side))) return rc;
        if ((rc = xproj_gemm(l, c, side))) return rc;
        if (side != ls[l + 1] && (rc = hand_off(sc, side, ls[l + 1]))) return rc;
        if (gemm_slot && side != ls[l] && (rc = hand_off(sc, side, ls[l]))) return rc;
      }
    }
  }
  for (int l = 1; l < NL; ++l)
    if (ls[l] != st && (rc = hand_off(sc, ls[l], st))) return rc;
  if (side != st && (rc = hand_off(sc, side, st))) return rc;
  if ((rc = prof_mark(g_prof, 1, st))) return rc;
  g_prof.launches[0] = n_launch;
  g_prof.cells[0] = T * NL;
  g_prof.have[0] = g_prof.on;
  return CSN_OK;
}

static int backward_persist(Plan& P, char* ws, const float* dy_last, const float* dy_tm, const float* dh_n,
                            const float* dc_n, float* const* dw_ih, float* const* dw_hh, float* const* db_ih,
                            float* const* db_hh, float* dx, hipStream_t st);

static int backward_il(Plan& P, char* ws, const float* dy_last, const float* dy_tm, const float* dh_n, const float* dc_n,
                       float* const* dw_ih, float* const* dw_hh, float* const* db_ih, float* const* db_hh, float* dx,
                       csnStream_t stream) {
  const csnLstmDesc* d = &P.d;
  const WsLayout& w = P.w;
  Prof& g_prof = P.prof;
  hipStream_t st = as_stream(stream);
  if (bwd_grouped(&P)) return backward_persist(P, ws, dy_last, dy_tm, dh_n, dc_n, dw_ih, dw_hh, db_ih, db_hh, dx, st);
  SideCtx* sc = &P.sc;
  int rc;
  if ((rc = side_ctx(P.sc))) return rc;
  hipStream_t side = P.opt.no_side_stream ? st : sc->side;
  const int B = d->B, T = d->T, H = d->H, NL = d->L;
  const int64_t G = 4 * (int64_t)H, TB = (int64_t)T * B;
  const size_t Bpad = ((size_t)B + 63) / 64 * 64;
  const int Cz = P.opt.chunk, lag = 2 * Cz;
  const int nch = (T + Cz - 1) / Cz;
  const bool state = P.state != 0;

  for (int l = 0; l < NL; ++l) {
    const LayerWs& L = w.layer[l];
    if (dc_n)
      CSN_HIP_CHECK(hipMemcpyAsync(ws + L.dc_carry, dc_n + (size_t)l * B * H, (size_t)B * H * 4, hipMemcpyDeviceToDevice, st));
    else
      CSN_HIP_CHECK(hipMemsetAsync(ws + L.dc_carry, 0, (size_t)B * H * 4, st));
    CSN_HIP_CHECK(hipMemsetAsync(ws + L.dgblk[0], 0, Bpad * G * 2, st));
    CSN_HIP_CHECK(hipMemsetAsync(ws + L.dgblk[1], 0, Bpad * G * 2, st));
  }
  if ((rc = hand_off(sc, st, side))) return rc;

  auto weight_grads = [&](int l) -> int {
    const LayerWs& L = w.layer[l];
    const int64_t I = l == 0 ? d->I : H;
    const void* inp = l == 0 ? (const void*)(ws + w.x_c)
                             : (const void*)((const bf16_t*)(ws + w.layer[l - 1].h_all) + (size_t)B * H);
    float* slabs = (float*)(ws + w.tn_scratch);
    const int acc = P.grad_accumulate;
    int S = 1, r;
    int cs_done = 0, S_cs = 1;
    if ((r = launch_gemm_tn_slabs(ws + L.dgates, ws + L.h_all, slabs, G, H, TB, CSN_BF16, side, &S, (float*)(ws + w.colsum), &cs_done, P.opt))) return r;
    S_cs = S;
    if ((r = launch_reduce_slabs_unperm(slabs, G * H, S, H, H, dw_hh[l], nullptr, acc, side))) return r;
    if ((r = launch_gemm_tn_slabs(ws + L.dgates, inp, slabs, G, I, TB, CSN_BF16, side, &S, nullptr, nullptr, P.opt))) return r;
    if ((r = launch_reduce_slabs_unperm(slabs, G * I, S, H, I, dw_ih[l], nullptr, acc, side))) return r;
    if (!cs_done) {
      if ((r = launch_colsum_partial(ws + L.dgates, TB, G, CSN_BF16, ws + w.colsum, side))) return r;
      S_cs = colsum_chunks();
    }
    if ((r = launch_reduce_slabs_unperm((const float*)(ws + w.colsum), G, S_cs, H, 1, db_ih[l], db_hh[l], acc, side)))
      return r;
    return CSN_OK;
  };

  std::vector<hipEvent_t> dx_ready((size_t)NL * nch, nullptr);
  const int D = T + lag * (NL - 1);
  int n_launch = 0, n_cells = 0;
  if ((rc = prof_mark(g_prof, 2, st))) return rc;
  for (int dg = 0; dg < D; ++dg) {
    CellBwdArgs a{};
    a.B = B;
    a.H = H;
    CellMask mask{P.dlen, {0, 0, 0, 0}};
    const CellMask* mk = P.dlen ? &mask : nullptr;
    int np = 0;
    for (int l = NL - 1; l >= 0; --l) {
      const int r = dg - lag * (NL - 1 - l);
      if (r < 0 || r >= T) continue;
      const int t = T - 1 - r;
      const LayerWs& L = w.layer[l];
      const bool top = (l == NL - 1);
      if (np == 4) {
        if ((rc = launch_cell_bwd_il(a, np, st, mk))) return rc;
        ++n_launch;
        n_cells += np;
        np = 0;
      }
      mask.t[np] = t;
      if (!top && r % Cz == 0) CSN_HIP_CHECK(hipStreamWaitEvent(st, dx_ready[(size_t)(l + 1) * nch + r / Cz], 0));
      CellBwdProb& P = a.p[np++];
      P.dg_next_blk = (t == T - 1) ? nullptr : (const bf16_t*)(ws + L.dgblk[(t + 1) & 1]);
      P.wt_blk = (const bf16_t*)(ws + L.whht_blk);
      if (top) {
        P.dy = dy_tm ? dy_tm + (size_t)t * B * H : (t == T - 1 ? dy_last : nullptr);
      } else {
        P.dy = (const float*)(ws + w.layer[l + 1].dx) + (size_t)t * B * H;
      }
      P.dy_ld = H;
      P.gates = (const bf16_t*)(ws + L.gates) + (size_t)t * B * G;
      P.c = (const float*)(ws + L.c_all) + (size_t)(t + 1) * B * H;
      P.c_prev = (t == 0 && !state) ? nullptr : (const float*)(ws + L.c_all) + (size_t)t * B * H;
      P.dc_carry = (float*)(ws + L.dc_carry);
      P.dg_out = (bf16_t*)(ws + L.dgates) + (size_t)t * B * G;
      P.dg_out_blk = (bf16_t*)(ws + L.dgblk[t & 1]);
    }
    if (np == 0) continue;
    if ((rc = launch_cell_bwd_il(a, np, st, mk))) return rc;
    ++n_launch;
    n_cells += np;
    for (int l = NL - 1; l >= 0; --l) {
      const int r = dg - lag * (NL - 1 - l);
      if (r < 0 || r >= T) continue;
      const bool chunk_end = ((r + 1) % Cz == 0) || r == T - 1;
      if (!chunk_end) continue;
      const LayerWs& L = w.layer[l];
      const int64_t I = l == 0 ? d->I : H;
      const int cr = r / Cz;
      const int t_lo = T - 1 - r, t_hi = T - 1 - cr * Cz;
      const bool last = (r == T - 1);
      if (l > 0 || last) {
        if ((rc = hand_off(sc, st, side))) return rc;
      }
      if (l > 0) {
        rc = gemm_nt((const bf16_t*)(ws + L.dgates) + (size_t)t_lo * B * G, ws + L.wiht, nullptr,
                         (float*)(ws + L.dx) + (size_t)t_lo * B * I, (int64_t)(t_hi - t_lo + 1) * B, I, G, CSN_BF16,
                         CSN_F32, 0, side, P.opt);
        if (rc) return rc;
        if (dh_n && (rc = add_dh_n_rows(P, dh_n + (size_t)(l - 1) * B * H, (float*)(ws + L.dx), t_lo, t_hi, side))) return rc;
        hipEvent_t ev;
        if ((rc = next_event(sc, &ev))) return rc;
        CSN_HIP_CHECK(hipEventRecord(ev, side));
        dx_ready[(size_t)l * nch + cr] = ev;
      } else if (last && dx != nullptr) {
        rc = gemm_nt(ws + L.dgates, ws + L.wiht, nullptr, ws + L.dx, TB, I, G, CSN_BF16, CSN_F32, 0,
                         side, P.opt);
        if (rc) return rc;
        if ((rc = emit_dx(P, (const float*)(ws + L.dx), dx, I, side))) return rc;
      }
      if (last && (rc = weight_grads(l))) return rc;
    }
  }
  if ((rc = prof_mark(g_prof, 3, st))) return rc;
  g_prof.launches[1] = n_launch;
  g_prof.cells[1] = n_cells;
  g_prof.have[1] = g_prof.on;
  if ((rc = hand_off(sc, side, st))) return rc;
  for (int l = NL - 1; l >= 0; --l) P.grads_ready(l);
  return CSN_OK;
}

static int backward_persist(Plan& P, char* ws, const float* dy_last, const float* dy_tm, const float* dh_n,
                            const float* dc_n, float* const* dw_ih, float* const* dw_hh, float* const* db_ih,
                            float* const* db_hh, float* dx, hipStream_t st) {
  const csnLstmDesc* d = &P.d;
  const WsLayout& w = P.w;
  Prof& g_prof = P.prof;
  const int B = d->B, T = d->T, H = d->H, NL = d->L;
  const int64_t G = 4 * (int64_t)H, TB = (int64_t)T * B;
  const int Bpad = (B + 63) / 64 * 64, MT = Bpad / 64;
  const int Cz = P.opt.chunk;
  const int nch = (T + Cz - 1) / Cz;
  const bool beside = NL > 1 && NL <= 4 && bwd_persist_slices(H) <= 28 && G % 64 == 0 && !P.opt.no_beside;
  const int lag = beside ? 2 : 1;
  const int ndiag = nch + lag * (NL - 1);
  int rc;
  CSN_HIP_CHECK(hipMemsetAsync(ws + w.zero_bwd, 0, w.zero_bwd_bytes, st));
  if (dc_n)
    for (int l = 0; l < NL; ++l)
      CSN_HIP_CHECK(hipMemcpyAsync(ws + w.layer[l].dc_carry, dc_n + (size_t)l * B * H, (size_t)B * H * 4,
                                   hipMemcpyDeviceToDevice, st));
  struct DhAdd { int l, t_lo, t_hi; };
  auto add_dh_n = [&](const DhAdd& q) -> int {
    return add_dh_n_rows(P, dh_n + (size_t)(q.l - 1) * B * H, (float*)(ws + w.layer[q.l].dx), q.t_lo, q.t_hi, st);
  };
  const bool try_local = !P.opt.no_xcd_local;

  auto weight_grads = [&](int l) -> int {
    const LayerWs& L = w.layer[l];
    const int64_t I = l == 0 ? d->I : H;
    const void* inp = l == 0 ? (const void*)(ws + w.x_c)
                             : (const void*)((const bf16_t*)(ws + w.layer[l - 1].h_all) + (size_t)B * H);
    float* slabs = (float*)(ws + w.tn_scratch);
    const int acc = P.grad_accumulate;
    int S = 1, r;
    int cs_done = 0, S_cs = 1;
    if ((r = launch_gemm_tn_slabs(ws + L.dgates, ws + L.h_all, slabs, G, H, TB, CSN_BF16, st, &S, (float*)(ws + w.colsum), &cs_done, P.opt))) return r;
    S_cs = S;
    if ((r = launch_reduce_slabs_unperm(slabs, G * H, S, H, H, dw_hh[l], nullptr, acc, st))) return r;
    if ((r = launch_gemm_tn_slabs(ws + L.dgates, inp, slabs, G, I, TB, CSN_BF16, st, &S, nullptr, nullptr, P.opt))) return r;
    if ((r = launch_reduce_slabs_unperm(slabs, G * I, S, H, I, dw_ih[l], nullptr, acc, st))) return r;
    if (!cs_done) {
      if ((r = launch_colsum_partial(ws + L.dgates, TB, G, CSN_BF16, ws + w.colsum, st))) return r;
      S_cs = colsum_chunks();
    }
    if ((r = launch_reduce_slabs_unperm((const float*)(ws + w.colsum), G, S_cs, H, 1, db_ih[l], db_hh[l], acc, st))) return r;
    return CSN_OK;
  };
  PersistBwdArgs a{};
  a.error_flag = (unsigned*)(ws + w.status);
  a.B = B; a.H = H; a.T = T; a.Bpad = Bpad; a.MT = MT;
  a.xcd_groups = 1;
  a.grid_slices = 32;
  a.rotate = !P.opt.no_rotate;
  a.data_polls = P.opt.bwd_flags ? 0 : (P.opt.dpoll_no_hint ? 2 : 1);
#ifdef CSN_SLAB_TAGS
  if (a.data_polls && P.opt.tags_no_rearm) a.data_polls |= 4;
#endif
  P.dgates_copies = 2;
  if (a.data_polls)
    for (int l = 0; l < NL; ++l) CSN_HIP_CHECK(hipMemsetAsync(ws + w.layer[l].dg_blk_all, 0xff, (size_t)4 * Bpad * G * 2, st));
  int n_launch = 0;
  P.half_launches[1] = 0;
  BesideGemm pending[3];
  DhAdd pending_add[3] = {{0, 0, 0}, {0, 0, 0}, {0, 0, 0}};
  int npending = 0;
  if ((rc = prof_mark(g_prof, 2, st))) return rc;
  for (int dg = 0; dg < ndiag; ++dg) {
    int lay[4], chk[4], ns = 0;
    for (int l = NL - 1; l >= 0; --l) {
      const int c = dg - lag * (NL - 1 - l);
      if (c < 0 || c >= nch) continue;
      const LayerWs& L = w.layer[l];
      PersistBwdSlot& S = a.slot[ns];
      S.wt_blk = (const bf16_t*)(ws + L.whht_blk);
      S.gates = (const bf16_t*)(ws + L.gates);
      S.c_all = (const float*)(ws + L.c_all);
      if (l == NL - 1) {
        S.dy = dy_tm;
        S.dy_last = dy_tm ? nullptr : dy_last;
      } else {
        S.dy = (const float*)(ws + w.layer[l + 1].dx);
        S.dy_last = nullptr;
      }
      S.zeros = (const float*)(ws + w.zeros_bh);
      S.dc_carry = (float*)(ws + L.dc_carry);
      S.dgates = (bf16_t*)(ws + L.dgates);
      S.dg_blk_all = (bf16_t*)(ws + L.dg_blk_all);
      S.flags = (unsigned*)(ws + L.bflags);
      S.t_hi = T - 1 - c * Cz;
      S.nsteps = (c * Cz + Cz <= T) ? Cz : T - c * Cz;
      lay[ns] = l;
      chk[ns] = c;
      ++ns;
    }
    if (ns == 0) {
      for (int i = 0; i < npending; ++i) {
        const BesideGemm& g = pending[i];
        if ((rc = gemm_nt(g.A, g.Bt, nullptr, g.C, g.M, g.N, g.K, CSN_BF16, CSN_F32, 0, st, P.opt))) return rc;
        if (pending_add[i].l && (rc = add_dh_n(pending_add[i]))) return rc;
      }
      npending = 0;
      continue;
    }
    a.nslots = ns;
    a.ngemm = npending;
    const bool half = !P.opt.no_half_tiles && P.dlen == nullptr && 2 * ns * MT <= 8;
    a.half_tiles = half ? 1 : 0;
    a.MT = half ? 2 * MT : MT;
    if (half) {
      for (int i = 0; i < ns; ++i) a.slot[i].flags += (size_t)T * MT * kPersistFlagLine;
      ++P.half_launches[1];
    }
    DhAdd launch_adds[3];
    int nadds = 0;
    for (int i = 0; i < npending; ++i) {
      a.gemm[i] = pending[i];
      if (pending_add[i].l) launch_adds[nadds++] = pending_add[i];
    }
    npending = 0;
    a.agree = try_local ? (unsigned long long*)(ws + w.agree_b) + (size_t)dg * 8 : nullptr;
    if ((rc = prof_pair(g_prof, 1, false, st))) return rc;
    if ((rc = launch_bwd_persist(a, st, P.dlen))) return rc;
    if ((rc = prof_pair(g_prof, 1, true, st))) return rc;
    ++n_launch;
    for (int i = 0; i < nadds; ++i)
      if ((rc = add_dh_n(launch_adds[i]))) return rc;
    for (int i = 0; i < ns; ++i) {
      const int l = lay[i];
      if (l == 0) continue;
      const LayerWs& L = w.layer[l];
      const int t_hi = T - 1 - chk[i] * Cz, t_lo = t_hi - a.slot[i].nsteps + 1;
      const bf16_t* Ag = (const bf16_t*)(ws + L.dgates) + (size_t)t_lo * B * G;
      float* Cg = (float*)(ws + L.dx) + (size_t)t_lo * B * H;
      const int64_t Mg = (int64_t)(t_hi - t_lo + 1) * B;
      const DhAdd add{(dh_n && (chk[i] == 0 || P.dlen)) ? l : 0, t_lo, t_hi};
      if (beside) {
        pending_add[npending] = add;
        pending[npending++] = BesideGemm{Ag, (const bf16_t*)(ws + L.wiht), Cg, (int)Mg, H, (int)G};
      } else {
        if ((rc = gemm_nt(Ag, ws + L.wiht, nullptr, Cg, Mg, H, G, CSN_BF16, CSN_F32, 0, st, P.opt))) return rc;
        if (add.l && (rc = add_dh_n(add))) return rc;
      }
    }
  }
  if ((rc = prof_mark(g_prof, 3, st))) return rc;
  g_prof.launches[1] = n_launch;
  g_prof.cells[1] = T * NL;
  g_prof.have[1] = g_prof.on;

  if (dx != nullptr) {
    const LayerWs& L = w.layer[0];
    if ((rc = gemm_nt(ws + L.dgates, ws + L.wiht, nullptr, ws + L.dx, TB, d->I, G, CSN_BF16, CSN_F32, 0,
                          st, P.opt)))
      return rc;
    if ((rc = emit_dx(P, (const float*)(ws + L.dx), dx, d->I, st))) return rc;
  }
  for (int l = NL - 1; l >= 0; --l) {
    if ((rc = weight_grads(l))) return rc;
    P.grads_ready(l);
  }
  return CSN_OK;
}

static int check_state_args(const Plan& P, const char* fn, const void* const* ptrs, const char* const* names, int n) {
  for (int i = 0; i < n; ++i) {
    if (ptrs[i] == nullptr) continue;
    CSN_REQUIRE(P.state, "%s: %s given, but the plan was created without CSN_LSTM_STATE", fn, names[i]);
    CSN_REQUIRE((reinterpret_cast<uintptr_t>(ptrs[i]) & 15) == 0, "%s: %s must be 16-B aligned", fn, names[i]);
  }
  return CSN_OK;
}

extern "C" int csn_lstm_forward(csnLstmPlan* Pp, const float* x, int64_t x_stride_b, int64_t x_stride_t,
                                const float* const* w_ih, const float* const* w_hh, const float* const* b_ih,
                                const float* const* b_hh, const float* h0, const float* c0, void* workspace,
                                float* y_last, float* y_all, float* h_n, float* c_n, csnStream_t stream) {
  CSN_REQUIRE(Pp != nullptr, "csn_lstm_forward: null plan");
  Plan& P = *Pp;
  const csnLstmDesc* d = &P.d;
  CSN_REQUIRE(x && w_ih && w_hh && b_ih && b_hh && workspace, "csn_lstm_forward: null pointer");
  CSN_REQUIRE((reinterpret_cast<uintptr_t>(workspace) & 255) == 0, "csn_lstm_forward: workspace must be 256-B aligned");
  CSN_REQUIRE(y_last || y_all || h_n || c_n, "csn_lstm_forward: no output requested");
  {
    const void* ptrs[4] = {h0, c0, h_n, c_n};
    const char* names[4] = {"h0", "c0", "h_n", "c_n"};
    if (int rc = check_state_args(P, "csn_lstm_forward", ptrs, names, 4)) return rc;
  }
  for (int l = 0; l < d->L; ++l)
    CSN_REQUIRE(w_ih[l] && w_hh[l] && b_ih[l] && b_hh[l], "csn_lstm_forward: null parameter pointer, layer %d", l);
  int dev = -1;
  CSN_HIP_CHECK(hipGetDevice(&dev));
  CSN_REQUIRE(dev == P.device, "csn_lstm_forward: plan was created on device %d, current device is %d", P.device, dev);
  hipStream_t st = as_stream(stream);
  const WsLayout& w = P.w;
  const int training = P.training;
  char* ws = (char*)workspace;
  const int B = d->B, T = d->T, H = d->H, dt = d->dtype;
  const size_t es = dtype_size(dt);
  int rc;
  if ((rc = upload_lengths(Pp, st))) return rc;
  if (P.dlen != nullptr) {
    if (P.t_eff > 0) {
      EffectiveT scope(P.d, P.t_eff);
      rc = w.il ? forward_il(P, ws, x, x_stride_b, x_stride_t, w_ih, w_hh, b_ih, b_hh, h0, c0, training, stream)
                : forward_v1(P, ws, x, x_stride_b, x_stride_t, w_ih, w_hh, b_ih, b_hh, h0, c0, training, stream);
      if (rc) return rc;
    } else {
      for (int l = 0; l < d->L; ++l) {
        const LayerWs& L = w.layer[l];
        if (h0) {
          if ((rc = launch_cast(h0 + (size_t)l * B * H, ws + L.h_all, (int64_t)B * H, dt, st))) return rc;
        } else {
          CSN_HIP_CHECK(hipMemsetAsync(ws + L.h_all, 0, (size_t)B * H * es, st));
        }
        if (c0)
          CSN_HIP_CHECK(hipMemcpyAsync(ws + L.c_all, c0 + (size_t)l * B * H, (size_t)B * H * 4, hipMemcpyDeviceToDevice, st));
        else
          CSN_HIP_CHECK(hipMemsetAsync(ws + L.c_all, 0, (size_t)B * H * 4, st));
      }
      if (h0 || c0) P.state_seen = true;
      P.prof.have[0] = false;
    }
    const unsigned gbh = grid_for((int64_t)B * H);
    auto gather_h = [&](const LayerWs& L, float* out) {
      if (dt == CSN_BF16) gather_state_kernel<bf16_t><<<gbh, 256, 0, st>>>((const bf16_t*)(ws + L.h_all), P.dlen, out, B, H);
      else gather_state_kernel<float><<<gbh, 256, 0, st>>>((const float*)(ws + L.h_all), P.dlen, out, B, H);
    };
    for (int l = 0; l < d->L; ++l) {
      const LayerWs& L = w.layer[l];
      if (h_n) gather_h(L, h_n + (size_t)l * B * H);
      if (c_n) gather_state_kernel<float><<<gbh, 256, 0, st>>>((const float*)(ws + L.c_all), P.dlen, c_n + (size_t)l * B * H, B, H);
    }
    const LayerWs& top = w.layer[d->L - 1];
    if (y_last) gather_h(top, y_last);
    if (y_all) {
      const int64_t n = (int64_t)T * B * H;
      if (dt == CSN_BF16)
        gather_y_all_len_kernel<bf16_t><<<grid_for(n), 256, 0, st>>>((const bf16_t*)(ws + top.h_all), y_all, P.dlen, B, T, H);
      else
        gather_y_all_len_kernel<float><<<grid_for(n), 256, 0, st>>>((const float*)(ws + top.h_all), y_all, P.dlen, B, T, H);
    }
    CSN_LAUNCH_CHECK();
    return CSN_OK;
  }
  if (w.il)
    rc = forward_il(P, ws, x, x_stride_b, x_stride_t, w_ih, w_hh, b_ih, b_hh, h0, c0, training, stream);
  else if (w.f32_persist)
    rc = forward_f32p(P, ws, x, x_stride_b, x_stride_t, w_ih, w_hh, b_ih, b_hh, training, stream);
  else
    rc = forward_v1(P, ws, x, x_stride_b, x_stride_t, w_ih, w_hh, b_ih, b_hh, h0, c0, training, stream);
  if (rc) return rc;
  for (int l = 0; l < d->L && (h_n || c_n); ++l) {
    const LayerWs& L = w.layer[l];
    if (h_n && (rc = launch_upcast(ws + L.h_all + (size_t)T * B * H * es, dt, h_n + (size_t)l * B * H, (int64_t)B * H, st)))
      return rc;
    if (c_n)
      CSN_HIP_CHECK(hipMemcpyAsync(c_n + (size_t)l * B * H, ws + L.c_all + (size_t)T * B * H * 4, (size_t)B * H * 4,
                                   hipMemcpyDeviceToDevice, st));
  }
  const LayerWs& top = w.layer[d->L - 1];
  if (y_last)
    if ((rc = launch_upcast(ws + top.h_all + (size_t)T * B * H * es, dt, y_last, (int64_t)B * H, st))) return rc;
  if (y_all) {
    const int64_t n = (int64_t)T * B * H;
    if (dt == CSN_BF16)
      gather_y_all_kernel<bf16_t><<<grid_for(n), 256, 0, st>>>((const bf16_t*)(ws + top.h_all), y_all, B, T, H);
    else
      gather_y_all_kernel<float><<<grid_for(n), 256, 0, st>>>((const float*)(ws + top.h_all), y_all, B, T, H);
    CSN_LAUNCH_CHECK();
  }
  return CSN_OK;
}

extern "C" int csn_lstm_backward(csnLstmPlan* Pp, const float* dy_last, const float* dy_all, const float* dh_n,
                                 const float* dc_n, void* workspace, float* const* dw_ih, float* const* dw_hh,
                                 float* const* db_ih, float* const* db_hh, float* dx, float* dh0, float* dc0,
                                 csnStream_t stream) {
  CSN_REQUIRE(Pp != nullptr, "csn_lstm_backward: null plan");
  Plan& P = *Pp;
  const csnLstmDesc* d = &P.d;
  CSN_REQUIRE(P.training, "csn_lstm_backward: the plan was created with training = 0");
  CSN_REQUIRE(workspace && dw_ih && dw_hh && db_ih && db_hh, "csn_lstm_backward: null pointer");
  CSN_REQUIRE(dy_last || dy_all || dh_n || dc_n, "csn_lstm_backward: no incoming gradient");
  {
    const void* ptrs[4] = {dh_n, dc_n, dh0, dc0};
    const char* names[4] = {"dh_n", "dc_n", "dh0", "dc0"};
    if (int rc = check_state_args(P, "csn_lstm_backward", ptrs, names, 4)) return rc;
  }
  for (int l = 0; l < d->L; ++l) {
    CSN_REQUIRE(dw_ih[l] && dw_hh[l] && db_ih[l] && db_hh[l], "csn_lstm_backward: null gradient pointer, layer %d", l);
    CSN_REQUIRE(!P.grad_accumulate || db_ih[l] != db_hh[l],
                "csn_lstm_backward: db_ih and db_hh of layer %d are one buffer under CSN_GRAD_ACCUMULATE", l);
  }
  int dev = -1;
  CSN_HIP_CHECK(hipGetDevice(&dev));
  CSN_REQUIRE(dev == P.device, "csn_lstm_backward: plan was created on device %d, current device is %d", P.device, dev);
  hipStream_t st = as_stream(stream);
  const WsLayout& w = P.w;
  char* ws = (char*)workspace;
  const int B = d->B, T = d->T, H = d->H;
  const int64_t TB = (int64_t)T * B;

  int rc;
  if ((rc = upload_lengths(Pp, st))) return rc;
  if (P.dlen != nullptr) {
    const int L_ = d->L, dt = d->dtype;
    const int64_t G = 4 * (int64_t)H;
    if (P.t_eff > 0) {
      const int Te = P.t_eff;
      float* buf = (float*)(ws + w.dy_tm);
      bt_to_tb_len_kernel<<<grid_for((int64_t)Te * B * H), 256, 0, st>>>(dy_all, buf, P.dlen, B, T, Te, H);
      if (dy_last) add_at_end_kernel<<<grid_for((int64_t)B * H), 256, 0, st>>>(dy_last, buf, P.dlen, 0, Te - 1, B, H);
      if (dh_n) add_at_end_kernel<<<grid_for((int64_t)B * H), 256, 0, st>>>(dh_n + (size_t)(L_ - 1) * B * H, buf, P.dlen, 0, Te - 1, B, H);
      CSN_LAUNCH_CHECK();
      {
        EffectiveT scope(P.d, Te);
        rc = w.il ? backward_il(P, ws, nullptr, buf, dh_n, dc_n, dw_ih, dw_hh, db_ih, db_hh, dx, stream)
                  : backward_v1(P, ws, nullptr, buf, dh_n, dc_n, dw_ih, dw_hh, db_ih, db_hh, dx, stream);
      }
      if (rc) return rc;
    } else {
      if (dx) CSN_HIP_CHECK(hipMemsetAsync(dx, 0, (size_t)T * B * d->I * 4, st));
      for (int l = L_ - 1; l >= 0; --l) {
        if (!P.grad_accumulate) {
          const int64_t I = l == 0 ? d->I : H;
          CSN_HIP_CHECK(hipMemsetAsync(dw_ih[l], 0, (size_t)(G * I) * 4, st));
          CSN_HIP_CHECK(hipMemsetAsync(dw_hh[l], 0, (size_t)(G * H) * 4, st));
          CSN_HIP_CHECK(hipMemsetAsync(db_ih[l], 0, (size_t)G * 4, st));
          CSN_HIP_CHECK(hipMemsetAsync(db_hh[l], 0, (size_t)G * 4, st));
        }
        P.grads_ready(l);
      }
      P.prof.have[1] = false;
    }
    for (int l = 0; l < L_ && (dh0 || dc0); ++l) {
      const LayerWs& L = w.layer[l];
      if (dh0) {
        float* out = dh0 + (size_t)l * B * H;
        if (P.t_eff > 0) {
          const dim3 grid((unsigned)((H + 63) / 64), (unsigned)((B + 31) / 32));
          if (w.il)
            lstm_dh0_kernel<bf16_t, true><<<grid, 256, 0, st>>>((const bf16_t*)(ws + L.dgates), (const bf16_t*)(ws + L.whht_blk), B, H, out);
          else if (dt == CSN_BF16)
            lstm_dh0_kernel<bf16_t, false><<<grid, 256, 0, st>>>((const bf16_t*)(ws + L.dgates), (const bf16_t*)(ws + L.whht), B, H, out);
          else
            lstm_dh0_kernel<float, false><<<grid, 256, 0, st>>>((const float*)(ws + L.dgates), (const float*)(ws + L.whht), B, H, out);
        } else {
          CSN_HIP_CHECK(hipMemsetAsync(out, 0, (size_t)B * H * 4, st));
        }
        if (dh_n) add_rows_len0_kernel<<<grid_for((int64_t)B * H), 256, 0, st>>>(dh_n + (size_t)l * B * H, out, P.dlen, B, H);
        CSN_LAUNCH_CHECK();
      }
      if (dc0) {
        if (P.t_eff > 0)
          CSN_HIP_CHECK(hipMemcpyAsync(dc0 + (size_t)l * B * H, ws + L.dc_carry, (size_t)B * H * 4, hipMemcpyDeviceToDevice, st));
        else if (dc_n)
          CSN_HIP_CHECK(hipMemcpyAsync(dc0 + (size_t)l * B * H, dc_n + (size_t)l * B * H, (size_t)B * H * 4, hipMemcpyDeviceToDevice, st));
        else
          CSN_HIP_CHECK(hipMemsetAsync(dc0 + (size_t)l * B * H, 0, (size_t)B * H * 4, st));
      }
    }
    return CSN_OK;
  }

  const float* dy_tm = nullptr;
  if (dy_all) {
    float* buf = (float*)(ws + w.dy_tm);
    bt_to_tb_kernel<<<grid_for(TB * H), 256, 0, st>>>(dy_all, buf, B, T, H);
    CSN_LAUNCH_CHECK();
    if (dy_last) {
      add_rows_kernel<<<grid_for((int64_t)B * H), 256, 0, st>>>(dy_last, buf + (size_t)(T - 1) * B * H, (int64_t)B * H);
      CSN_LAUNCH_CHECK();
    }
    dy_tm = buf;
  }
  if (dh_n) {
    const float* dh_top = dh_n + (size_t)(d->L - 1) * B * H;
    if (dy_tm) {
      add_rows_kernel<<<grid_for((int64_t)B * H), 256, 0, st>>>(dh_top, (float*)dy_tm + (size_t)(T - 1) * B * H, (int64_t)B * H);
      CSN_LAUNCH_CHECK();
    } else if (dy_last) {
      float* buf = (float*)(ws + w.dy_tm);
      CSN_HIP_CHECK(hipMemcpyAsync(buf, dy_last, (size_t)B * H * 4, hipMemcpyDeviceToDevice, st));
      add_rows_kernel<<<grid_for((int64_t)B * H), 256, 0, st>>>(dh_top, buf, (int64_t)B * H);
      CSN_LAUNCH_CHECK();
      dy_last = buf;
// ... 30 lines not shown
```

### cerebralsignalnetworks_amd/csrc/lstm_cell_blk.h

```cpp
#pragma once
#include "csn_common.h"

#ifdef CSN_SLAB_TAGS
#define CSN_DPOLL_MODE(x) ((x) & 3)
#define CSN_DPOLL_NO_REARM(x) (((x) & 4) != 0)
#else
#define CSN_DPOLL_MODE(x) (x)
#define CSN_DPOLL_NO_REARM(x) false
#endif

namespace csn {

struct CellFwdProb {
  const bf16_t* h_prev_blk;
  const bf16_t* w_blk;
  const float* xproj;
  const float* c_prev;
  bf16_t* gates_out;
  float* c_out;
  bf16_t* h_out;
  bf16_t* h_out_blk;
};
struct CellFwdArgs {
  CellFwdProb p[4];
// ... 8 lines not shown
  const bf16_t* gates;
  const float* c;
  const float* c_prev;
  float* dc_carry;
  bf16_t* dg_out;
  bf16_t* dg_out_blk;
};
struct CellBwdArgs {
  CellBwdProb p[4];
  int B, H;
};

struct PersistFwdSlot {
  const bf16_t* w_blk;
  const float* xproj;
  bf16_t* gates;
  float* c_all;
  bf16_t* h_all;
  bf16_t* h_blk_all;
  unsigned* flags;
  const bf16_t* x_blk;
  const bf16_t* wih_blk;
  const float* bias;
  int I;
  int t0, nsteps;
};
struct BesideGemm {
  const bf16_t* A;
  const bf16_t* Bt;
  float* C;
  int M, N, K;
};
static constexpr int kPersistFlagLine = 32;
struct PersistFwdArgs {
  PersistFwdSlot slot[4];
  int nslots;
  int data_polls;
  int xcd_groups;
  int rotate;
  unsigned long long* agree;
  unsigned* error_flag;
  int B, H, T, Bpad, MT;
  int state;
  int half_tiles;
};
bool fwd_persist_supported(int B, int H, int dtype, const Options& opt);
bool fwd_ns_supported(int B, int H, int dtype, const Options& opt);
int fwd_ns_slices(int H);
int launch_fwd_ns(const PersistFwdArgs& a, hipStream_t st);
int fwd_persist_slices(int H);
int launch_fwd_persist(const PersistFwdArgs& a, hipStream_t st);

struct PersistBwdSlot {
  const bf16_t* wt_blk;
  const bf16_t* gates;
  const float* c_all;
  const float* dy;
  const float* dy_last;
  const float* zeros;
  float* dc_carry;
  bf16_t* dgates;
  bf16_t* dg_blk_all;
  unsigned* flags;
  int t_hi, nsteps;
};
struct PersistBwdArgs {
  PersistBwdSlot slot[4];
  int nslots;
  BesideGemm gemm[3];
  int ngemm;
  int grid_slices;
  int xcd_groups;
  int rotate;
  int data_polls;
  unsigned long long* agree;
  unsigned* error_flag;
  int B, H, T, Bpad, MT;
  int half_tiles;
};
bool bwd_persist_supported(int B, int H, int dtype, const Options& opt);
int bwd_persist_slices(int H);
int launch_bwd_persist(const PersistBwdArgs& a, hipStream_t st, const int* lengths = nullptr);

enum { kPrepBlockify = 0, kPrepPermRows, kPrepTransPerm, kPrepBias, kPrepCastX, kPrepBlockifyX };
static constexpr int kPrepMaxJobs = 32;
struct PrepJob {
  int kind;
  const float* a;
  const float* b;
  void* dst;
  int64_t n0, n1, n2, s0, s1, H;
  int perm_r, perm_k;
  int64_t work;
  unsigned blk_begin, blk_count;
};
struct PrepArgs {
  PrepJob job[kPrepMaxJobs];
  int njobs;
};
int launch_prep_multi(PrepArgs& A, hipStream_t st);

bool cell_blk_supported(int H, int dtype, const Options& opt);
int launch_cell_fwd_il(const CellFwdArgs& a, int nprob, hipStream_t st, int max_nk);
int launch_cell_bwd_il(const CellBwdArgs& a, int nprob, hipStream_t st, const CellMask* mask = nullptr);
int launch_blockify_x(const float* x, int64_t xsb, int64_t xst, int B, int T, int I, void* dst, hipStream_t st);
int launch_blockify(const float* src, int64_t ld_r, int64_t ld_k, int64_t R, int64_t K, int perm_r, int perm_k,
                    int64_t H, void* dst, hipStream_t st);
int launch_permute_rows_cast(const float* src, int64_t H, int64_t I, void* dst, hipStream_t st);
int launch_transpose_perm_cast(const float* src, int64_t H, int64_t I, void* dst, hipStream_t st);
int launch_bias_perm_sum(const float* a, const float* b, int64_t H, float* dst, hipStream_t st);
int launch_reduce_slabs_unperm(const float* slabs, int64_t slab_stride, int S, int64_t H, int64_t C, float* out,
                               float* out2, int accumulate, hipStream_t st);

}
```

### cerebralsignalnetworks_amd/csrc/lstm_cell_blk.hip

```cpp
#include "csn_common.h"
#include "lstm_cell_common.h"
#include "lstm_cell_blk.h"

#ifdef CSN_STAMPS
__device__ unsigned long long* g_stamps = nullptr;
#define CSN_STAMP(i)                                                                      \
  do {                                                                                    \
    __builtin_amdgcn_sched_barrier(0);                                                    \
    if (threadIdx.x == 0)                                                                 \
      g_stamps[((blockIdx.z * gridDim.y + blockIdx.y) * gridDim.x + blockIdx.x) * 8 + (i)] = wall_clock64(); \
    __builtin_amdgcn_sched_barrier(0);                                                    \
  } while (0)
#else
#define CSN_STAMP(i)
#endif

namespace csn {

__device__ __forceinline__ int64_t std_row(int64_t nprime, int64_t H) { return (nprime & 3) * H + (nprime >> 2); }

__global__ void __launch_bounds__(256)
blockify_cast_kernel(const float* __restrict__ src, int64_t ld_r, int64_t ld_k, int64_t R, int64_t K, int perm_r,
                     int perm_k, int64_t H, bf16_t* __restrict__ dst) {
  const int64_t nchunks = R * K / 8;
// ... 75 lines not shown
          __syncthreads();
#pragma unroll
          for (int h = 0; h < 2; ++h) {
            const int c = t + 256 * h, fb = c >> 6, lane = c & 63, rb = fb >> 1, kb = fb & 1;
            const int ul = rb * 16 + (lane & 15), kl = kb * 32 + 8 * (lane >> 4);
            bf16x8 v;
#pragma unroll
            for (int e = 0; e < 8; ++e) v[e] = tp[kl + e][ul];
            const int64_t blk = (tu * 4 + rb) * kblocks + tk * 2 + kb;
            *reinterpret_cast<bf16x8*>(dst + (blk * 64 + lane) * 8) = v;
          }
          __syncthreads();
        }
        break;
      }
      for (int64_t ci = gid; ci < R * K / 8; ci += stride) {
        const int64_t blk = ci >> 6, lane = ci & 63;
        const int64_t r = (blk / kblocks) * 16 + (lane & 15), k = (blk % kblocks) * 32 + 8 * (lane >> 4);
        const int64_t rs = J.perm_r ? std_row(r, H) : r;
        bf16x8 v;
        if (!J.perm_k && ld_k == 1 && (ld_r & 3) == 0) {
          const float4* sp = reinterpret_cast<const float4*>(J.a + rs * ld_r + k);
          const float4 u = sp[0], w = sp[1];
          v = (bf16x8){(bf16_t)u.x, (bf16_t)u.y, (bf16_t)u.z, (bf16_t)u.w, (bf16_t)w.x, (bf16_t)w.y, (bf16_t)w.z, (bf16_t)w.w};
        } else {
#pragma unroll
          for (int e = 0; e < 8; ++e) {
            const int64_t ks = J.perm_k ? std_row(k + e, H) : (k + e);
            v[e] = (bf16_t)J.a[rs * ld_r + ks * ld_k];
          }
        }
        *reinterpret_cast<bf16x8*>(dst + ci * 8) = v;
      }
      break;
    }
    case kPrepPermRows: {
      const int64_t H = J.H, I = J.n1;
      bf16_t* dst = (bf16_t*)J.dst;
      if ((I & 7) == 0) {
        for (int64_t c = gid; c < 4 * H * I / 8; c += stride) {
          const int64_t i = c * 8;
          const float4* sp = reinterpret_cast<const float4*>(J.a + std_row(i / I, H) * I + i % I);
          const float4 u = sp[0], v = sp[1];
          *reinterpret_cast<bf16x8*>(dst + i) = (bf16x8){(bf16_t)u.x, (bf16_t)u.y, (bf16_t)u.z, (bf16_t)u.w,
                                                         (bf16_t)v.x, (bf16_t)v.y, (bf16_t)v.z, (bf16_t)v.w};
        }
      } else {
        for (int64_t i = gid; i < 4 * H * I; i += stride) dst[i] = (bf16_t)J.a[std_row(i / I, H) * I + i % I];
      }
      break;
    }
    case kPrepTransPerm: {
      const int64_t H = J.H, I = J.n1, G = 4 * H;
      bf16_t* dst = (bf16_t*)J.dst;
      if ((I & 63) == 0 && (G & 63) == 0) {
        const int64_t tiles_n = G >> 6, ntiles = tiles_n * (I >> 6);
        const int t = threadIdx.x, rr = t >> 2, seg = t & 3;
        for (int64_t tile = vb; tile < ntiles; tile += vg) {
          const int64_t tn = tile % tiles_n, ti = tile / tiles_n;
          const float4* sp = reinterpret_cast<const float4*>(J.a + std_row(tn * 64 + rr, H) * I + ti * 64 + seg * 16);
          const float4 q0 = sp[0], q1 = sp[1], q2 = sp[2], q3 = sp[3];
          const float v[16] = {q0.x, q0.y, q0.z, q0.w, q1.x, q1.y, q1.z, q1.w, q2.x, q2.y, q2.z, q2.w, q3.x, q3.y, q3.z, q3.w};
#pragma unroll
          for (int e = 0; e < 16; ++e) tp[seg * 16 + e][rr] = (bf16_t)v[e];
          __syncthreads();
          bf16_t* dp = dst + (ti * 64 + rr) * G + tn * 64 + seg * 16;
          *reinterpret_cast<bf16x8*>(dp) = *reinterpret_cast<const bf16x8*>(&tp[rr][seg * 16]);
          *reinterpret_cast<bf16x8*>(dp + 8) = *reinterpret_cast<const bf16x8*>(&tp[rr][seg * 16 + 8]);
          __syncthreads();
        }
        break;
      }
      for (int64_t i = gid; i < G * I; i += stride) dst[i] = (bf16_t)J.a[std_row(i % G, H) * I + i / G];
      break;
    }
    case kPrepBias: {
      float* dst = (float*)J.dst;
      for (int64_t i = gid; i < 4 * J.H; i += stride) dst[i] = J.a[std_row(i, J.H)] + J.b[std_row(i, J.H)];
      break;
    }
    case kPrepCastX: {
      const int64_t Bn = J.n0, Tn = J.n1, I = J.n2;
      bf16_t* dst = (bf16_t*)J.dst;
      if ((I & 7) == 0 && (J.s0 & 3) == 0 && (J.s1 & 3) == 0 && (reinterpret_cast<uintptr_t>(J.a) & 15) == 0) {
        for (int64_t c = gid; c < Bn * Tn * I / 8; c += stride) {
          const int64_t i = c * 8, i2 = i % I, r = i / I, b = r % Bn, t = r / Bn;
          const float4* sp = reinterpret_cast<const float4*>(J.a + b * J.s0 + t * J.s1 + i2);
          const float4 u = sp[0], v = sp[1];
          *reinterpret_cast<bf16x8*>(dst + i) = (bf16x8){(bf16_t)u.x, (bf16_t)u.y, (bf16_t)u.z, (bf16_t)u.w,
                                                         (bf16_t)v.x, (bf16_t)v.y, (bf16_t)v.z, (bf16_t)v.w};
        }
      } else {
        for (int64_t i = gid; i < Bn * Tn * I; i += stride) {
          const int64_t i2 = i % I, r = i / I, b = r % Bn, t = r / Bn;
          dst[i] = (bf16_t)J.a[b * J.s0 + t * J.s1 + i2];
        }
      }
      break;
    }
    case kPrepBlockifyX: {
      const int64_t Bn = J.n0, Tn = J.n1, I = J.n2, Bpad = J.H, per_t = Bpad * I / 8, kblocks = I >> 5;
      bf16_t* dst = (bf16_t*)J.dst;
      for (int64_t ci = gid; ci < per_t * Tn; ci += stride) {
        const int64_t t = ci / per_t, c = ci % per_t, blk = c >> 6, lane = c & 63;
        const int64_t r = (blk / kblocks) * 16 + (lane & 15), k = (blk % kblocks) * 32 + 8 * (lane >> 4);
        bf16x8 v;
        if (r < Bn && ((J.s0 | J.s1) & 3) == 0 && (reinterpret_cast<uintptr_t>(J.a) & 15) == 0) {
          const float4* sp = reinterpret_cast<const float4*>(J.a + r * J.s0 + t * J.s1 + k);
          const float4 u = sp[0], w = sp[1];
          v = (bf16x8){(bf16_t)u.x, (bf16_t)u.y, (bf16_t)u.z, (bf16_t)u.w, (bf16_t)w.x, (bf16_t)w.y, (bf16_t)w.z, (bf16_t)w.w};
        } else {
#pragma unroll
          for (int e = 0; e < 8; ++e) v[e] = (bf16_t)(r < Bn ? J.a[r * J.s0 + t * J.s1 + k + e] : 0.f);
        }
        *reinterpret_cast<bf16x8*>(dst + ci * 8) = v;
      }
      break;
    }
  }
}

int launch_prep_multi(PrepArgs& A, hipStream_t st) {
  CSN_REQUIRE(A.njobs >= 1 && A.njobs <= kPrepMaxJobs, "launch_prep_multi: %d jobs", A.njobs);
  unsigned total = 0;
  for (int j = 0; j < A.njobs; ++j) {
    int64_t blocks = (A.job[j].work + 255) / 256;
    if (blocks < 1) blocks = 1;
    if (blocks > 2048) blocks = 2048;
    A.job[j].blk_begin = total;
    A.job[j].blk_count = (unsigned)blocks;
    total += (unsigned)blocks;
  }
  prep_multi_kernel<<<total, 256, 0, st>>>(A);
  CSN_LAUNCH_CHECK();
  return CSN_OK;
}

static inline unsigned cap_grid(int64_t n) {
  int64_t g = (n + 255) / 256;
  return (unsigned)(g < 1 ? 1 : (g > 2048 ? 2048 : g));
}

__global__ void blockify_x_kernel(const float* __restrict__ x, int64_t xsb, int64_t xst, int B, int Bpad, int T, int I,
                                  bf16_t* __restrict__ dst) {
  const int64_t per_t = (int64_t)Bpad * I / 8, nchunks = per_t * T;
  const int64_t stride = (int64_t)gridDim.x * blockDim.x;
  const int kblocks = I >> 5;
  for (int64_t ci = (int64_t)blockIdx.x * blockDim.x + threadIdx.x; ci < nchunks; ci += stride) {
    const int64_t t = ci / per_t, c = ci % per_t;
    const int64_t blk = c >> 6, lane = c & 63;
    const int64_t r = (blk / kblocks) * 16 + (lane & 15);
    const int64_t k = (blk % kblocks) * 32 + 8 * (lane >> 4);
    bf16x8 v;
#pragma unroll
    for (int j = 0; j < 8; ++j) v[j] = (bf16_t)(r < B ? x[r * xsb + t * xst + k + j] : 0.f);
    *reinterpret_cast<bf16x8*>(dst + ci * 8) = v;
  }
}
int launch_blockify_x(const float* x, int64_t xsb, int64_t xst, int B, int T, int I, void* dst, hipStream_t st) {
  const int Bpad = (B + 63) / 64 * 64;
  blockify_x_kernel<<<cap_grid((int64_t)T * Bpad * I / 8), 256, 0, st>>>(x, xsb, xst, B, Bpad, T, I, (bf16_t*)dst);
  CSN_LAUNCH_CHECK();
  return CSN_OK;
}

int launch_blockify(const float* src, int64_t ld_r, int64_t ld_k, int64_t R, int64_t K, int perm_r, int perm_k,
                    int64_t H, void* dst, hipStream_t st) {
  blockify_cast_kernel<<<cap_grid(R * K / 8), 256, 0, st>>>(src, ld_r, ld_k, R, K, perm_r, perm_k, H, (bf16_t*)dst);
  CSN_LAUNCH_CHECK();
  return CSN_OK;
}
int launch_permute_rows_cast(const float* src, int64_t H, int64_t I, void* dst, hipStream_t st) {
  permute_rows_cast_kernel<<<cap_grid(4 * H * I), 256, 0, st>>>(src, H, I, (bf16_t*)dst);
  CSN_LAUNCH_CHECK();
  return CSN_OK;
}
int launch_transpose_perm_cast(const float* src, int64_t H, int64_t I, void* dst, hipStream_t st) {
  transpose_perm_cast_kernel<<<cap_grid(4 * H * I), 256, 0, st>>>(src, H, I, (bf16_t*)dst);
  CSN_LAUNCH_CHECK();
  return CSN_OK;
}
int launch_bias_perm_sum(const float* a, const float* b, int64_t H, float* dst, hipStream_t st) {
  bias_perm_sum_kernel<<<(unsigned)((4 * H + 255) / 256), 256, 0, st>>>(a, b, H, dst);
  CSN_LAUNCH_CHECK();
  return CSN_OK;
}
int launch_reduce_slabs_unperm(const float* slabs, int64_t slab_stride, int S, int64_t H, int64_t C, float* out,
                               float* out2, int accumulate, hipStream_t st) {
  reduce_slabs_unperm_kernel<<<cap_grid(4 * H * C), 256, 0, st>>>(slabs, slab_stride, S, H, C, out, out2, accumulate);
  CSN_LAUNCH_CHECK();
  return CSN_OK;
}

template <int NQ, int NK>
__global__ void __launch_bounds__(256) lstm_cell_fwd_il_kernel(CellFwdArgs a) {
  constexpr int NT = 4 * NQ;
  constexpr int NPAIR = 64 * NQ;
  constexpr int NPASS = (NPAIR + 255) / 256;
  extern __shared__ __attribute__((aligned(16))) float4 red[];
  const CellFwdProb& P = a.p[blockIdx.z];
  const int B = a.B, H = a.H;
  const int tid = threadIdx.x, lane = tid & 63, wave = tid >> 6;
  const int u0 = blockIdx.x * 4 * NQ, m0 = blockIdx.y * 64;
  const int kblocks = H >> 5;
  CSN_STAMP(0);

  constexpr bool EPI_EARLY = NQ < 8;
  float4 xp[NPASS][4], cp[NPASS];
  auto request_epilogue = [&]() {
#pragma unroll
    for (int ps = 0; ps < NPASS; ++ps) {
      const int p = tid + ps * 256;
      const int row = m0 + p / NQ, uq = u0 + 4 * (p % NQ);
      cp[ps] = make_float4(0.f, 0.f, 0.f, 0.f);
      if (p < NPAIR && row < B) {
        const float4* xr = reinterpret_cast<const float4*>(P.xproj + (int64_t)row * 4 * H + 4 * (int64_t)uq);
#pragma unroll
        for (int q = 0; q < 4; ++q) xp[ps][q] = nt_load(xr + q);
        if (P.c_prev != nullptr) cp[ps] = *reinterpret_cast<const float4*>(P.c_prev + (int64_t)row * H + uq);
      }
    }
  };
  if constexpr (EPI_EARLY) request_epilogue();

  f32x4 acc[4][NQ];
#pragma unroll
  for (int rg = 0; rg < 4; ++rg)
#pragma unroll
    for (int j = 0; j < NQ; ++j) acc[rg][j] = (f32x4){0.f, 0.f, 0.f, 0.f};

  if (P.h_prev_blk != nullptr) {
    const int ks_beg = wave * (kblocks >> 2), ks_end = ks_beg + (kblocks >> 2);
    const bf16_t* hb[4];
    const bf16_t* wb[NQ];
#pragma unroll
    for (int rg = 0; rg < 4; ++rg) hb[rg] = P.h_prev_blk + ((int64_t)((m0 >> 4) + rg) * kblocks) * 512 + lane * 8;
#pragma unroll
    for (int j = 0; j < NQ; ++j) wb[j] = P.w_blk + ((int64_t)((u0 >> 2) + j) * kblocks) * 512 + lane * 8;

    bf16x8 hA[NK][4], wA[NK][NQ], hB[NK][4], wB[NK][NQ];
    auto load_pass = [&](int ks0, bf16x8 (&hf)[NK][4], bf16x8 (&wf)[NK][NQ]) {
#pragma unroll
      for (int ks = 0; ks < NK; ++ks) {
#pragma unroll
        for (int rg = 0; rg < 4; ++rg) hf[ks][rg] = *reinterpret_cast<const bf16x8*>(hb[rg] + (int64_t)(ks0 + ks) * 512);
#pragma unroll
        for (int j = 0; j < NQ; ++j) wf[ks][j] = *reinterpret_cast<const bf16x8*>(wb[j] + (int64_t)(ks0 + ks) * 512);
      }
    };
    auto mma_pass = [&](bf16x8 (&hf)[NK][4], bf16x8 (&wf)[NK][NQ]) {
#pragma unroll
      for (int ks = 0; ks < NK; ++ks)
#pragma unroll
        for (int rg = 0; rg < 4; ++rg)
#pragma unroll
          for (int j = 0; j < NQ; ++j)
            acc[rg][j] = __builtin_amdgcn_mfma_f32_16x16x32_bf16(wf[ks][j], hf[ks][rg], acc[rg][j], 0, 0, 0);
    };
    int ks0 = ks_beg;
    load_pass(ks0, hA, wA);
    while (true) {
      int kn = ks0 + NK;
      if (kn < ks_end) load_pass(kn, hB, wB);
      mma_pass(hA, wA);
      if (kn >= ks_end) break;
      ks0 = kn;
      kn = ks0 + NK;
      if (kn < ks_end) load_pass(kn, hA, wA);
      mma_pass(hB, wB);
      if (kn >= ks_end) break;
      ks0 = kn;
    }
// ... 255 lines not shown
```

### cerebralsignalnetworks_amd/lstm_model.py

```python
import torch
import torch.nn as nn

from . import cabi


class _Lease:

    def __init__(self, plan):
        self.plan = plan
        plan.busy = True

    def release(self):
        if self.plan is not None:
            self.plan.busy = False
            self.plan = None

    __del__ = release


def _direct_grads(owner, params):
    mode = owner.direct_grads
    if not mode or not all(p.grad is not None and p.grad.is_contiguous() and p.grad.dtype == torch.float32 for p in params):
        return False, False
    return True, mode == "accumulate"


class _LstmFunction(torch.autograd.Function):

    @staticmethod
    def forward(ctx, x, owner, want_all, training, L, *params):
        w_ih, w_hh, b_ih, b_hh = params[0:L], params[L:2 * L], params[2 * L:3 * L], params[3 * L:4 * L]
        plan = owner._checkout(x.shape[0], x.shape[1], x.device, training)
        y_last, y_all = plan.forward(x, w_ih, w_hh, b_ih, b_hh, want_all=want_all)
        ctx.lease, ctx.L, ctx.want_all = _Lease(plan), L, want_all
        ctx.owner = owner
        ctx.need_dx = x.requires_grad
        ctx.x_shape = x.shape
        ctx.param_like = params
        if not training:
            ctx.lease.release()
        if want_all:
            return y_last, y_all
        return y_last, y_last.new_empty(0)

    @staticmethod
    def backward(ctx, dy_last, dy_all):
        L, plan = ctx.L, ctx.lease.plan
        if plan is None:
            raise RuntimeError("HipLSTM: second backward through one forward -- its workspace was handed back after the "
                               "first (retain_graph / double backward are not supported)")
        owner = ctx.owner
        direct, accumulate = _direct_grads(owner, ctx.param_like)
        if direct:
            grads = [[p.grad for p in ctx.param_like[g * L:(g + 1) * L]] for g in range(4)]
        else:
            grads = [[torch.empty_like(p) for p in ctx.param_like[g * L:(g + 1) * L]] for g in range(4)]
        dx = torch.empty(ctx.x_shape, dtype=torch.float32, device=dy_last.device) if ctx.need_dx else None
        plan.set_grad_callback(owner.grad_ready_hook if direct else None)
        plan.set_grad_mode(accumulate)
        plan.backward(dy_last, dy_all if ctx.want_all else None, grads, dx=dx)
        ctx.lease.release()
        if direct:
            return (dx, None, None, None, None, *([None] * (4 * L)))
        flat = [g for group in grads for g in group]
        return (dx, None, None, None, None, *flat)


class HipLSTM(nn.Module):

    MAX_IDLE_PLANS = 4
    _STATE_PLANS = False

    def __init__(self, input_size, hidden_size, num_layers=1, compute_dtype=torch.bfloat16):
        super().__init__()
        self.input_size, self.hidden_size, self.num_layers = input_size, hidden_size, num_layers
        self.compute_dtype = compute_dtype
        ref = nn.LSTM(input_size, hidden_size, num_layers=num_layers, batch_first=True)
        for name, p in ref.named_parameters():
            self.register_parameter(name, nn.Parameter(p.detach().clone()))
        self._plans = {}
        self.direct_grads = False
        self.grad_ready_hook = None

    def _checkout(self, B, T, device, training):
        key = (B, T, str(device), bool(training), self.compute_dtype)
        pool = self._plans.setdefault(key, [])
        for plan in pool:
            if not plan.busy:
                return plan
        idle = [(k, pl) for k, lst in self._plans.items() for pl in lst if not pl.busy and k != key]
        while len(idle) >= self.MAX_IDLE_PLANS:
            k, pl = idle.pop(0)
            self._plans[k].remove(pl)
        plan = cabi.LstmPlan(B, T, self.input_size, self.hidden_size, self.num_layers, self.compute_dtype, device,
                             training=training, state=self._STATE_PLANS)
        pool.append(plan)
        return plan

    def all_plans(self):
        return [pl for lst in self._plans.values() for pl in lst]

    def forward(self, x, want_all=False):
        if not x.is_cuda:
            raise cabi.CsnError("HipLSTM runs on the GPU only (no CPU fallback); move the module and input to cuda")
        L = self.num_layers
        params = [getattr(self, f"{n}_l{k}") for n in ("weight_ih", "weight_hh", "bias_ih", "bias_hh") for k in range(L)]
        training = torch.is_grad_enabled() and (x.requires_grad or any(p.requires_grad for p in params))
        y_last, y_all = _LstmFunction.apply(x, self, want_all, training, L, *params)
        return (y_all, y_last) if want_all else y_last


class _LstmStateFunction(torch.autograd.Function):

    @staticmethod
    def forward(ctx, x, h0, c0, owner, training, lengths, L, *params):
        w_ih, w_hh, b_ih, b_hh = params[0:L], params[L:2 * L], params[2 * L:3 * L], params[3 * L:4 * L]
        plan = owner._checkout(x.shape[0], x.shape[1], x.device, training)
        plan.set_lengths(lengths)
        _, y_all, h_n, c_n = plan.forward(x, w_ih, w_hh, b_ih, b_hh, want_all=True, h0=h0, c0=c0, want_state=True)
        ctx.lease, ctx.L, ctx.owner = _Lease(plan), L, owner
        ctx.lengths = lengths
        ctx.need = (x.requires_grad, h0 is not None and h0.requires_grad, c0 is not None and c0.requires_grad)
        ctx.x_shape = x.shape
        ctx.param_like = params
        if not training:
            ctx.lease.release()
        return y_all, h_n, c_n

    @staticmethod
    def backward(ctx, dy_all, dh_n, dc_n):
        L, plan = ctx.L, ctx.lease.plan
        if plan is None:
            raise RuntimeError("LSTM: second backward through one forward -- its workspace was handed back after the "
                               "first (retain_graph / double backward are not supported)")
        direct, accumulate = _direct_grads(ctx.owner, ctx.param_like)
        direct = direct and accumulate
        if direct:
            grads = [[p.grad for p in ctx.param_like[g * L:(g + 1) * L]] for g in range(4)]
        else:
            grads = [[torch.empty_like(p) for p in ctx.param_like[g * L:(g + 1) * L]] for g in range(4)]
        dev = ctx.param_like[0].device
        need_dx, need_dh0, need_dc0 = ctx.need
        d = plan.desc
        dx = torch.empty(ctx.x_shape, dtype=torch.float32, device=dev) if need_dx else None
        dh0 = torch.empty((L, d.B, d.H), dtype=torch.float32, device=dev) if need_dh0 else None
        dc0 = torch.empty((L, d.B, d.H), dtype=torch.float32, device=dev) if need_dc0 else None
        plan.set_grad_callback(ctx.owner.grad_ready_hook if direct else None)
        plan.set_grad_mode(direct)
        plan.set_lengths(ctx.lengths)
        plan.backward(None, dy_all, grads, dx=dx, dh_n=dh_n, dc_n=dc_n, dh0=dh0, dc0=dc0)
        ctx.lease.release()
        if direct:
            return (dx, dh0, dc0, None, None, None, None, *([None] * (4 * L)))
        flat = [g for group in grads for g in group]
        return (dx, dh0, dc0, None, None, None, None, *flat)


class LSTM(HipLSTM):

    _STATE_PLANS = True

    def __init__(self, input_size, hidden_size, num_layers=1, bias=True, batch_first=True, dropout=0.0,
                 bidirectional=False, proj_size=0, compute_dtype=torch.bfloat16):
        unsupported = [name for name, bad in (("bias=False", not bias), ("batch_first=False", not batch_first),
                                              ("dropout != 0", dropout != 0), ("bidirectional=True", bidirectional),
                                              ("proj_size != 0", proj_size != 0)) if bad]
        if unsupported:
            raise ValueError(f"LSTM: {', '.join(unsupported)} is not supported (batch-first, biased, unidirectional "
                             f"stacks without projection or inter-layer dropout only)")
        super().__init__(input_size, hidden_size, num_layers, compute_dtype=compute_dtype)
        self.bias, self.batch_first, self.dropout, self.bidirectional, self.proj_size = True, True, 0.0, False, 0

    def forward(self, x, hx=None, lengths=None):
        if isinstance(x, nn.utils.rnn.PackedSequence):
            if lengths is not None:
                raise ValueError("LSTM: lengths given together with a PackedSequence (it carries its own)")
            padded, lens = nn.utils.rnn.pad_packed_sequence(x, batch_first=True)
            output, state = self.forward(padded, hx, lengths=lens)
            if x.sorted_indices is not None:
                output, lens = output.index_select(0, x.sorted_indices), lens[x.sorted_indices.cpu()]
            packed = nn.utils.rnn.pack_padded_sequence(output, lens, batch_first=True, enforce_sorted=True)
            return nn.utils.rnn.PackedSequence(packed.data, x.batch_sizes, x.sorted_indices, x.unsorted_indices), state
        if x.dim() != 3:
            raise ValueError(f"LSTM: input must be batched [B, T, {self.input_size}] (batch_first); got shape "
                             f"{list(x.shape)} (unbatched input is not supported)")
        if x.shape[2] != self.input_size:
            raise ValueError(f"LSTM: input has {x.shape[2]} features, expected {self.input_size}")
        B, L, H = x.shape[0], self.num_layers, self.hidden_size
        h0 = c0 = None
        if hx is not None:
            h0, c0 = hx
            for name, t in (("h0", h0), ("c0", c0)):
                if tuple(t.shape) != (L, B, H):
                    raise ValueError(f"LSTM: {name} must be [num_layers, B, hidden_size] = {[L, B, H]}, got {list(t.shape)}")
        if lengths is not None:
            if isinstance(lengths, torch.Tensor):
                if lengths.is_cuda:
                    raise ValueError("LSTM: lengths must be a CPU int tensor or a sequence of ints (pass CPU lengths, as "
                                     "pack_padded_sequence takes them)")
                if lengths.dim() != 1 or lengths.dtype.is_floating_point or lengths.dtype in (torch.bool,):
                    raise ValueError(f"LSTM: lengths must be a 1-d int tensor, got {lengths.dtype} of shape {list(lengths.shape)}")
                lengths = lengths.tolist()
            lengths = tuple(int(n) for n in lengths)
            if len(lengths) != B:
                raise ValueError(f"LSTM: {len(lengths)} lengths for a batch of {B}")
            bad = [n for n in lengths if n < 0 or n > x.shape[1]]
            if bad:
                raise ValueError(f"LSTM: length {bad[0]} outside [0, T = {x.shape[1]}]")
        if not x.is_cuda:
            raise cabi.CsnError("LSTM runs on the GPU only (no CPU fallback); move the module and input to cuda")
        params = [getattr(self, f"{n}_l{k}") for n in ("weight_ih", "weight_hh", "bias_ih", "bias_hh") for k in range(L)]
        training = torch.is_grad_enabled() and (x.requires_grad or any(p.requires_grad for p in params) or
                                                any(t is not None and t.requires_grad for t in (h0, c0)))
        y_all, h_n, c_n = _LstmStateFunction.apply(x, h0, c0, self, training, lengths, L, *params)
        return y_all, (h_n, c_n)


class Model(nn.Module):

    def __init__(self, input_size=128, lstm_size=128, lstm_layers=1, output_size=128, include_top=True,
                 n_classes=40, compute_dtype=torch.bfloat16):
        super().__init__()
        self.input_size, self.lstm_size, self.lstm_layers = input_size, lstm_size, lstm_layers
        self.output_size, self.include_top = output_size, include_top
        self.lstm = HipLSTM(input_size, lstm_size, lstm_layers, compute_dtype=compute_dtype)
        self.fc = nn.Linear(lstm_size, output_size)
        if include_top:
            self.class_pred = nn.Linear(output_size, n_classes)

    def forward(self, x):
        last = self.lstm(x)
        feat = self.fc(last)
        if self.include_top and hasattr(self, "class_pred"):
            return feat, self.class_pred(feat)
# ... 35 lines not shown
```

### cerebralsignalnetworks_amd/trainer.py

```python
import math

import torch
import torch.distributed as dist
import torch.nn as nn

from . import filters
from .losses import (CosineSimilarityLoss, FeatureDistributionLoss, HyperParams, loss_fn_kd, BarlowTwinsLoss,
                     LARS)


def dist_info():
    if dist.is_available() and dist.is_initialized():
        return dist.get_rank(), dist.get_world_size()
    return 0, 1


class FlatGrads:

    def __init__(self, params, flatten_params=False):
        self.params = [p for p in params if p.requires_grad]
        total = sum(p.numel() for p in self.params)
        self.flat = torch.zeros(total, dtype=torch.float32, device=self.params[0].device)
        self.flat_params = torch.empty_like(self.flat) if flatten_params else None
        self.timing = None
# ... 142 lines not shown
    if bad & cabi.STATUS_NONFINITE:
        raise FloatingPointError("libcsn_hip: a non-finite (NaN / Inf) gradient reached the LSTM backward: the run has "
                                 "diverged (the reference would carry the NaN through its loss and weights)")


class DistillTrainer:
    def __init__(self, model, sos, ddof=0, loss="cosine", lr=1e-3, optimizer="rmsprop", nepochs=100,
                 kd_params=None, preprocess=True, accum_steps=1):
        if not isinstance(accum_steps, int) or isinstance(accum_steps, bool) or accum_steps < 1:
            raise ValueError(f"accum_steps must be an integer >= 1, got {accum_steps!r}")
        if accum_steps > 1 and loss == "barlow":
            raise ValueError("accum_steps > 1 needs a loss that is a mean over the batch rows (cosine, featdist, kd): barlow "
                             "normalises with the statistics of the batch, so micro-batches do not sum to the full batch")
        self.accum_steps = accum_steps
        self.model = model
        self.sos, self.ddof, self.preprocess = sos, ddof, preprocess
        self.loss_name = loss
        on_gpu = next(model.parameters()).is_cuda
        self.grads = FlatGrads(model.parameters(), flatten_params=(optimizer == "rmsprop" and on_gpu))
        params = self.grads.params
        if optimizer == "rmsprop" and on_gpu:
            self.opt = FlatRMSprop(self.grads, lr=lr)
        elif optimizer == "rmsprop":
            self.opt = torch.optim.RMSprop(params, lr=lr)
        elif optimizer == "adamw":
            self.opt = torch.optim.AdamW(params, lr=lr)
        elif optimizer == "adam":
            self.opt = torch.optim.Adam(params, lr=lr)
        elif optimizer == "lars":
            self.opt = LARS(params, lr=lr, weight_decay=1e-6, weight_decay_filter=True, lars_adaptation_filter=True)
        else:
            raise ValueError(optimizer)
        self.cosine = CosineSimilarityLoss()
        self.featdist = FeatureDistributionLoss(nepochs, HyperParams.warmup_teacher_temp, HyperParams.teacher_temp,
                                                HyperParams.warmup_teacher_temp_epochs)
        self.kd_params = kd_params
        self.barlow = None
        rank, world = dist_info()
        if world > 1:
            for p in model.parameters():
                dist.broadcast(p.data, src=0)
        self._wire_lstm_gradients(world)

    def _wire_lstm_gradients(self, world):
        import os
        from .lstm_model import HipLSTM
        lstms = [m for m in self.model.modules() if isinstance(m, HipLSTM)]
        self._hook_error = None
        self._lstm = None
        if len(lstms) != 1 or not self.grads.flat.is_cuda:
            return
        lstm = lstms[0]
        self._lstm = lstm
        lstm.direct_grads = "accumulate"
        L = lstm.num_layers
        first = [self.grads.offsets[id(getattr(lstm, f"weight_ih_l{k}"))][0] for k in range(L)]
        last = self.grads.offsets[id(getattr(lstm, f"bias_hh_l{L - 1}"))]
        lstm_end = last[0] + last[1]
        contiguous = all(first[k] < first[k + 1] for k in range(L - 1)) and first[0] == min(o for o, _ in self.grads.offsets.values())
        if world == 1 or not os.environ.get("CSN_AR_OVERLAP") or not contiguous:
            return
        total = self.grads.flat.numel()
        self.grads.segments = [(first[k], first[k + 1] if k + 1 < L else lstm_end) for k in range(L)] + [(lstm_end, total)]
        others = [p for p in self.grads.params if self.grads.offsets[id(p)][0] >= lstm_end]
        self._others_left = len(others)
        self._n_others = len(others)

        def other_done(_p):
            self._others_left -= 1
        for p in others:
            p.register_post_accumulate_grad_hook(other_done)

        def layer_ready(layer):
            try:
                if layer == 0:
                    return
                self.grads.segment_ready(layer, also=(L,) if self._others_left == 0 else ())
            except Exception as e:
                self._hook_error = e
        lstm.grad_ready_hook = layer_ready

    def embed(self, eeg_bct):
        if self.preprocess:
            return filters.eeg_bandpass_znorm(eeg_bct, self.sos, ddof=self.ddof, time_major=True).transpose(0, 1)
        return eeg_bct.transpose(1, 2).contiguous()

    def compute_loss(self, out, targets, labels, epoch):
        if self.loss_name == "cosine":
            feat = out[0] if isinstance(out, tuple) else out
            return self.cosine(feat, targets)
        if self.loss_name == "featdist":
            feat, cls = out
            return self.featdist(feat, targets, epoch, labels, pred_label=cls)
        if self.loss_name == "kd":
            feat = out[0] if isinstance(out, tuple) else out
            return loss_fn_kd(feat, labels, targets, self.kd_params)
        if self.loss_name == "barlow":
            feat = out[0] if isinstance(out, tuple) else out
            if self.barlow is None:
                _, world = dist_info()
                self.barlow = BarlowTwinsLoss(feat.shape[1], feat.shape[0] * world).to(feat.device)
            return self.barlow(feat, targets)
        raise ValueError(self.loss_name)

    def train_step(self, eeg_bct, targets, labels=None, epoch=0):
        k = self.accum_steps
        B = eeg_bct.shape[0]
        if B % k != 0:
            raise ValueError(f"train_step: batch of {B} rows does not split into accum_steps = {k} equal micro-batches")
        self.model.train()
        self.grads.zero()
        if k == 1:
            if self.grads.segments is not None:
                self._others_left = self._n_others
            x = self.embed(eeg_bct)
            out = self.model(x)
            loss = self.compute_loss(out, targets, labels, epoch)
            loss.backward()
        else:
            loss = self._micro_batches(eeg_bct, targets, labels, epoch, k)
        if self._hook_error is not None:
            err, self._hook_error = self._hook_error, None
            raise err
        self.grads.all_reduce_mean()
        self.opt.step()
        return loss.detach()

    def _micro_batches(self, eeg_bct, targets, labels, epoch, k):
        mb = eeg_bct.shape[0] // k
        lstm = self._lstm
        hook = lstm.grad_ready_hook if lstm is not None else None
        total = None
        try:
            for j in range(k):
                rows = slice(j * mb, (j + 1) * mb)
                last = j == k - 1
                if lstm is not None:
                    lstm.grad_ready_hook = hook if last else None
                if last and self.grads.segments is not None:
                    self._others_left = self._n_others
                out = self.model(self.embed(eeg_bct[rows]))
                loss = self.compute_loss(out, targets[rows], None if labels is None else labels[rows], epoch) / k
                loss.backward()
                total = loss.detach() if total is None else total + loss.detach()
        finally:
            if lstm is not None:
                lstm.grad_ready_hook = hook
        return total

    def check_device_status(self):
        bufs = [self.grads.flat] + ([self.grads.flat_params] if self.grads.flat_params is not None else
                                    [p.data for p in self.grads.params])
        finite = torch.stack([torch.isfinite(b).all() for b in bufs]).all()
        _, world = dist_info()
        if world > 1:
            t = (~finite).to(torch.int32).reshape(1)
            t = t if dist.get_backend() == "nccl" else t.cpu()
            dist.all_reduce(t, op=dist.ReduceOp.MAX)
            finite = t.item() == 0
        finite = bool(finite)
        reported_before = getattr(self, "_nonfinite_reported", False)
        self._nonfinite_reported = not finite
        check_device_status(self.model)
        if not finite and not reported_before:
            raise FloatingPointError("non-finite (NaN / Inf) parameters or gradients: the run has diverged")

    @torch.no_grad()
# ... 8 lines not shown
```

### include/csn_hip.h

```cpp
#ifndef CSN_HIP_H
#define CSN_HIP_H

#include <stddef.h>
#include <stdint.h>

#ifdef __cplusplus
extern "C" {
#endif

typedef void* csnStream_t;

enum csnStatus {
  CSN_OK = 0,
  CSN_ERR_INVALID_ARGUMENT = 1,
  CSN_ERR_HIP = 2,
  CSN_ERR_UNSUPPORTED = 3
};

enum csnDtype { CSN_F32 = 0, CSN_BF16 = 1 };

#define CSN_ABI_VERSION 6
int csn_abi_version(void);
const char* csn_last_error(void);
const char* csn_target_arch(void);

int csn_eeg_bandpass_znorm(const float* x, int B, int C, int T,
                           const double* sos, int nsec, int ddof,
                           void* y, int out_dtype, int time_major, csnStream_t stream);

size_t csn_eeg_filtfilt_scratch_bytes(int S, int T, int C, int nsec);
int csn_eeg_filtfilt(const float* x, int S, int T, int C, const double* sos, int nsec,
                     float* y, void* scratch, csnStream_t stream);

typedef struct csnLstmDesc {
  int32_t B;
  int32_t T;
  int32_t I;
  int32_t H;
  int32_t L;
  int32_t dtype;
} csnLstmDesc;

typedef struct csnLstmPlan csnLstmPlan;
#define CSN_LSTM_STATE 0x100
int csn_lstm_plan_create(const csnLstmDesc* d, int training, csnLstmPlan** out);
void csn_lstm_plan_destroy(csnLstmPlan* plan);
size_t csn_lstm_plan_workspace_bytes(const csnLstmPlan* plan);
int csn_lstm_plan_path(const csnLstmPlan* plan);
int csn_lstm_plan_dgates_copies(const csnLstmPlan* plan);
int csn_lstm_plan_half_tile_launches(const csnLstmPlan* plan, int which);
const char* csn_lstm_plan_kernel_name(const csnLstmPlan* plan, int which);
size_t csn_lstm_workspace_bytes(const csnLstmDesc* d, int training);

int csn_lstm_workspace_init(const csnLstmPlan* plan, void* workspace, csnStream_t stream);

int csn_lstm_forward(csnLstmPlan* plan,
                     const float* x, int64_t x_stride_b, int64_t x_stride_t,
                     const float* const* w_ih, const float* const* w_hh,
                     const float* const* b_ih, const float* const* b_hh,
                     const float* h0, const float* c0,
                     void* workspace, float* y_last, float* y_all,
                     float* h_n, float* c_n, csnStream_t stream);

int csn_lstm_backward(csnLstmPlan* plan,
                      const float* dy_last, const float* dy_all,
                      const float* dh_n, const float* dc_n,
                      void* workspace,
                      float* const* dw_ih, float* const* dw_hh,
                      float* const* db_ih, float* const* db_hh,
                      float* dx, float* dh0, float* dc0, csnStream_t stream);

typedef void (*csnGradReadyFn)(void* user, int layer);
int csn_lstm_plan_set_grad_callback(csnLstmPlan* plan, csnGradReadyFn fn, void* user);

#define CSN_GRAD_OVERWRITE  0
#define CSN_GRAD_ACCUMULATE 1
int csn_lstm_plan_set_grad_mode(csnLstmPlan* plan, int mode);

int csn_lstm_plan_set_lengths(csnLstmPlan* plan, const int32_t* lengths);

#define CSN_STATUS_TIMEOUT 1
#define CSN_STATUS_NONFINITE 2
#define CSN_STATUS_STALE_SLOT 4
int csn_lstm_status_clear(const csnLstmPlan* plan, void* workspace, csnStream_t stream);
int csn_lstm_status_read(const csnLstmPlan* plan, const void* workspace, int* status);
int csn_lstm_status_raise(const csnLstmPlan* plan, void* workspace, csnStream_t stream);

int csn_lstm_profile_enable(csnLstmPlan* plan, int on);
int csn_lstm_profile_read(csnLstmPlan* plan, double* fwd_ms, int* fwd_launches, int* fwd_cells,
                          double* bwd_ms, int* bwd_launches, int* bwd_cells);

int csn_gemm_nt(const void* A, const void* Bt, const float* bias, void* C,
                int64_t M, int64_t N, int64_t K, int dtype, int out_dtype, int accumulate,
                csnStream_t stream);
size_t csn_gemm_tn_scratch_bytes(int64_t M, int64_t N, int64_t K);
int csn_gemm_tn(const void* A, const void* B, float* C,
                int64_t M, int64_t N, int64_t K, int dtype, void* scratch, csnStream_t stream);

int csn_lstm_cell_forward(const void* h_prev, const void* w_hh, const float* xproj, int64_t xproj_ld,
                          const float* c_prev, void* gates_out, float* c_out, void* h_out,
                          int B, int H, int dtype, csnStream_t stream);
int csn_lstm_cell_backward(const void* dgates_next, const void* w_hh_t,
                           const float* dy, int64_t dy_ld,
                           const void* gates, const float* c, const float* c_prev,
                           float* dc_carry, void* dgates_out,
                           int B, int H, int dtype, csnStream_t stream);

size_t csn_cosine_loss_scratch_bytes(int B);
int csn_cosine_loss(const float* student, const float* teacher, int B, int D,
                    float* loss, float* dstudent, float grad_scale, void* scratch, csnStream_t stream);

int csn_rmsprop_step(float* params, const float* grads, float* square_avg, int64_t n,
                     float lr, float alpha, float eps, csnStream_t stream);

int csn_barlow_offdiag_sqsum(const float* c, int D, float* out, csnStream_t stream);

size_t csn_l2_topk_scratch_bytes(int64_t Ng, int64_t Nq);
int csn_l2_topk(const float* gallery, const float* query, int64_t Ng, int64_t Nq, int D, int k,
                int64_t* out_idx, float* out_dist, void* scratch, csnStream_t stream);

#ifdef __cplusplus
}
#endif
#endif
```

Measured before the change: 27300.

## Feed bf16 EEG input directly to LSTM and fold workspace fills into prep launch

The bandpass/z-norm filter now emits bf16 when the LSTM computes in bf16, and a new bf16 forward entry point uses that input directly, skipping the fp32 round trip and the cast. Memsets for zero and poll-flag regions are folded into the multi-job prep kernel as fill jobs, which removes separate launches. A multi-job slab reduce kernel is also added. The cost is extra code paths, retaining the bf16 input tensor until backward, and a larger tn scratch area.

```diff
diff --git a/cerebralsignalnetworks_amd/cabi.py b/cerebralsignalnetworks_amd/cabi.py
--- a/cerebralsignalnetworks_amd/cabi.py
+++ b/cerebralsignalnetworks_amd/cabi.py
@@ -36,6 +36,7 @@
     "csn_lstm_plan_path": (_c_int, [_c_void_p]),
     "csn_lstm_plan_dgates_copies": (_c_int, [_c_void_p]),
     "csn_lstm_plan_half_tile_launches": (_c_int, [_c_void_p, _c_int]),
+    "csn_lstm_plan_aux_launches": (_c_int, [_c_void_p, _c_int]),
     "csn_lstm_plan_kernel_name": (ctypes.c_char_p, [_c_void_p, _c_int]),
     "csn_lstm_plan_set_grad_callback": (_c_int, [_c_void_p, _c_void_p, _c_void_p]),
     "csn_lstm_plan_set_grad_mode": (_c_int, [_c_void_p, _c_int]),
@@ -47,6 +48,12 @@
                                   _c_void_p, _c_void_p,
                                   _c_void_p, _c_void_p, _c_void_p,
                                   _c_void_p, _c_void_p, _c_void_p]),
+    "csn_lstm_forward_x16": (_c_int, [_c_void_p, _c_void_p, _c_i64, _c_i64,
+                                      ctypes.POINTER(_c_void_p), ctypes.POINTER(_c_void_p),
+                                      ctypes.POINTER(_c_void_p), ctypes.POINTER(_c_void_p),
+                                      _c_void_p, _c_void_p,
+                                      _c_void_p, _c_void_p, _c_void_p,
+                                      _c_void_p, _c_void_p, _c_void_p]),
     "csn_lstm_backward": (_c_int, [_c_void_p, _c_void_p, _c_void_p,
                                    _c_void_p, _c_void_p,
                                    _c_void_p,
@@ -286,10 +293,14 @@
     def half_tile_launches(self, which):
         return load().csn_lstm_plan_half_tile_launches(self._plan, which)
 
+    def aux_launches(self, which):
+        return load().csn_lstm_plan_aux_launches(self._plan, which)
+
     def forward(self, x_bti, w_ih, w_hh, b_ih, b_hh, want_all=False, h0=None, c0=None, want_state=False):
         d = self.desc
         _need_cuda(x_bti)
-        if x_bti.dtype != torch.float32 or x_bti.stride(2) != 1:
+        x16 = x_bti.dtype == torch.bfloat16 and d.dtype == CSN_BF16 and x_bti.stride(2) == 1
+        if not x16 and (x_bti.dtype != torch.float32 or x_bti.stride(2) != 1):
             x_bti = x_bti.float().contiguous()
         assert x_bti.shape == (d.B, d.T, d.I), (tuple(x_bti.shape), (d.B, d.T, d.I))
         y_last = torch.empty((d.B, d.H), dtype=torch.float32, device=x_bti.device)
@@ -302,10 +313,11 @@
         h_n = torch.empty((d.L, d.B, d.H), dtype=torch.float32, device=x_bti.device) if want_state else None
         c_n = torch.empty((d.L, d.B, d.H), dtype=torch.float32, device=x_bti.device) if want_state else None
         with torch.cuda.device(self.device):
-            _check(load().csn_lstm_forward(self._plan, _ptr(x_bti), x_bti.stride(0), x_bti.stride(1),
-                                           _ptr_array(ws[0]), _ptr_array(ws[1]), _ptr_array(ws[2]), _ptr_array(ws[3]),
-                                           _ptr(h0), _ptr(c0), self._ws_ptr, _ptr(y_last), _ptr(y_all),
-                                           _ptr(h_n), _ptr(c_n), _stream()))
+            fwd = load().csn_lstm_forward_x16 if x16 else load().csn_lstm_forward
+            _check(fwd(self._plan, _ptr(x_bti), x_bti.stride(0), x_bti.stride(1),
+                       _ptr_array(ws[0]), _ptr_array(ws[1]), _ptr_array(ws[2]), _ptr_array(ws[3]),
+                       _ptr(h0), _ptr(c0), self._ws_ptr, _ptr(y_last), _ptr(y_all),
+                       _ptr(h_n), _ptr(c_n), _stream()))
         if want_state:
             return y_last, y_all, h_n, c_n
         return y_last, y_all
diff --git a/cerebralsignalnetworks_amd/csrc/csn_common.h b/cerebralsignalnetworks_amd/csrc/csn_common.h
--- a/cerebralsignalnetworks_amd/csrc/csn_common.h
+++ b/cerebralsignalnetworks_amd/csrc/csn_common.h
@@ -42,7 +42,7 @@
 
 struct Options {
   bool cell_v1, no_persist, no_persist_bwd, persist_streams, no_xcd_local, no_rotate, no_fuse_x, no_beside,
-      no_side_stream, gemm_slot, fwd_ksplit, fwd_nsplit, fwd_flags, bwd_flags, dpoll_no_hint, fwd_hint, gemm_no_dma, gemm_no_256, gemm_generic, gemm_lds64, tn_no_tr, tn_no_stagger, filter_v1, tags_no_rearm, gemm_no_192, no_half_tiles;
+      no_side_stream, gemm_slot, fwd_ksplit, fwd_nsplit, fwd_flags, bwd_flags, dpoll_no_hint, fwd_hint, gemm_no_dma, gemm_no_256, gemm_generic, gemm_lds64, tn_no_tr, tn_no_stagger, filter_v1, tags_no_rearm, gemm_no_192, no_half_tiles, no_step_fusions;
   int chunk;
   int tn_stages;
   int fwd_nk;
@@ -63,6 +63,7 @@
   o.no_fuse_x = on("CSN_NO_FUSE_X");
   o.no_beside = on("CSN_NO_BESIDE");
   o.no_half_tiles = on("CSN_NO_HALF_TILES");
+  o.no_step_fusions = on("CSN_NO_STEP_FUSIONS");
   o.no_side_stream = on("CSN_NO_SIDE_STREAM");
   o.gemm_slot = on("CSN_GEMM_SLOT");
   o.fwd_ksplit = on("CSN_FWD_KSPLIT");
diff --git a/cerebralsignalnetworks_amd/csrc/lstm.hip b/cerebralsignalnetworks_amd/csrc/lstm.hip
--- a/cerebralsignalnetworks_amd/csrc/lstm.hip
+++ b/cerebralsignalnetworks_amd/csrc/lstm.hip
@@ -83,6 +83,7 @@
       if (w.persist_bwd) L.dg_blk_all = take((size_t)(d.T < 4 ? 4 : d.T) * Bpad * G * 2);
     }
     size_t a = gemm_tn_scratch_bytes(G, I, TB, opt), b = gemm_tn_scratch_bytes(G, H, TB, opt);
+    if (w.il && !opt.no_step_fusions) a = align_up(b, 256) + a, b = 0;
     if (a > tn_bytes) tn_bytes = a;
     if (b > tn_bytes) tn_bytes = b;
   }
@@ -386,6 +387,16 @@
   int32_t* len_dev = nullptr;
   int32_t* len_pin = nullptr;
   hipEvent_t len_ev = nullptr;
+  int aux_launches[3] = {0, 0, 0};
+  struct WsCall { const void* ws; const void* x_img; int armed_T; };
+  std::vector<WsCall> calls;
+  WsCall& call_of(const void* ws) {
+    for (WsCall& c : calls)
+      if (c.ws == ws) return c;
+    calls.push_back(WsCall{ws, nullptr, 0});
+    return calls.back();
+  }
+  const void* x_img(const char* ws) { const void* p = call_of(ws).x_img; return p ? p : (const void*)(ws + w.x_c); }
   void grads_ready(int layer) const {
     if (grad_cb != nullptr) grad_cb(grad_cb_user, layer);
   }
@@ -451,6 +462,10 @@
   return (P == nullptr || which < 0 || which > 1) ? -1 : P->half_launches[which];
 }
 
+extern "C" int csn_lstm_plan_aux_launches(const csnLstmPlan* P, int which) {
+  return (P == nullptr || which < 0 || which > 2) ? -1 : P->aux_launches[which];
+}
+
 static bool bwd_grouped(const csnLstmPlan* P) {
   if (!P->w.persist_bwd) return false;
   const int MTg = (P->d.B + 63) / 64, nchg = (P->d.T + P->opt.chunk - 1) / P->opt.chunk;
@@ -644,6 +659,28 @@
   return launch_reduce_slabs((const float*)scratch, M * N, S, C, nullptr, M * N, accumulate, st);
 }
 
+#define CSN_MEMSET(P, k, args)          \
+  do {                                  \
+    ++(P).aux_launches[k];              \
+    CSN_HIP_CHECK(hipMemsetAsync args); \
+  } while (0)
+
+struct XIn {
+  const void* p;
+  int64_t sb, st;
+  bool bf16, in_place;
+};
+
+__global__ void copy_strided_bf16_kernel(const bf16_t* __restrict__ x, int64_t xsb, int64_t xst, int B, int Tn, int I,
+                                         bf16_t* __restrict__ dst) {
+  const int64_t total = (int64_t)B * Tn * I;
+  const int64_t stride = (int64_t)gridDim.x * blockDim.x;
+  for (int64_t i = (int64_t)blockIdx.x * blockDim.x + threadIdx.x; i < total; i += stride) {
+    const int64_t i2 = i % I, r = i / I, b = r % B, t = r / B;
+    dst[i] = x[b * xsb + t * xst + i2];
+  }
+}
+
 static int mask_x(const csnLstmPlan& P, char* ws, hipStream_t st) {
   if (P.dlen == nullptr) return CSN_OK;
   const csnLstmDesc& d = P.d;
@@ -659,7 +696,7 @@
   return CSN_OK;
 }
 
-static int forward_v1(Plan& P, char* ws, const float* x, int64_t xsb, int64_t xst,
+static int forward_v1(Plan& P, char* ws, const XIn& x,
                       const float* const* w_ih, const float* const* w_hh, const float* const* b_ih,
                       const float* const* b_hh, const float* h0, const float* c0, int training, csnStream_t stream) {
   const csnLstmDesc* d = &P.d;
@@ -670,7 +707,14 @@
   const size_t es = dtype_size(dt);
   const int Cz = P.opt.chunk, lag = Cz;
   int rc;
-  if ((rc = launch_cast_strided(x, xsb, xst, B, T, d->I, ws + w.x_c, dt, st))) return rc;
+  if (x.bf16) {
+    if (!x.in_place) {
+      copy_strided_bf16_kernel<<<grid_for(TB * d->I), 256, 0, st>>>((const bf16_t*)x.p, x.sb, x.st, B, T, d->I, (bf16_t*)(ws + w.x_c));
+      CSN_LAUNCH_CHECK();
+    }
+  } else if ((rc = launch_cast_strided((const float*)x.p, x.sb, x.st, B, T, d->I, ws + w.x_c, dt, st))) {
+    return rc;
+  }
   if ((rc = mask_x(P, ws, st))) return rc;
   for (int l = 0; l < NL; ++l) {
     const LayerWs& L = w.layer[l];
@@ -685,14 +729,14 @@
     if (h0) {
       if ((rc = launch_cast(h0 + (size_t)l * B * H, ws + L.h_all, (int64_t)B * H, dt, st))) return rc;
     } else {
-      CSN_HIP_CHECK(hipMemsetAsync(ws + L.h_all, 0, (size_t)B * H * es, st));
+      CSN_MEMSET(P, 0, (ws + L.h_all, 0, (size_t)B * H * es, st));
     }
     if (c0)
       CSN_HIP_CHECK(hipMemcpyAsync(ws + L.c_all, c0 + (size_t)l * B * H, (size_t)B * H * 4, hipMemcpyDeviceToDevice, st));
     else
-      CSN_HIP_CHECK(hipMemsetAsync(ws + L.c_all, 0, (size_t)B * H * 4, st));
-  }
-  if ((rc = gemm_nt(ws + w.x_c, ws + w.layer[0].wih, (const float*)(ws + w.layer[0].bias), ws + w.layer[0].xproj, TB, G,
+      CSN_MEMSET(P, 0, (ws + L.c_all, 0, (size_t)B * H * 4, st));
+  }
+  if ((rc = gemm_nt(P.x_img(ws), ws + w.layer[0].wih, (const float*)(ws + w.layer[0].bias), ws + w.layer[0].xproj, TB, G,
                     d->I, dt, CSN_F32, 0, st, P.opt)))
     return rc;
   const int D = T + lag * (NL - 1);
@@ -742,7 +786,7 @@
     if (dc_n)
       CSN_HIP_CHECK(hipMemcpyAsync(ws + w.layer[l].dc_carry, dc_n + (size_t)l * B * H, (size_t)B * H * 4, hipMemcpyDeviceToDevice, st));
     else
-      CSN_HIP_CHECK(hipMemsetAsync(ws + w.layer[l].dc_carry, 0, (size_t)B * H * 4, st));
+      CSN_MEMSET(P, 1, (ws + w.layer[l].dc_carry, 0, (size_t)B * H * 4, st));
   }
   const int D = T + lag * (NL - 1);
   for (int dg = 0; dg < D; ++dg) {
@@ -783,7 +827,7 @@
   for (int l = NL - 1; l >= 0; --l) {
     const LayerWs& L = w.layer[l];
     const int64_t I = l == 0 ? d->I : H;
-    const void* inp = l == 0 ? (const void*)(ws + w.x_c)
+    const void* inp = l == 0 ? P.x_img(ws)
                              : (const void*)(ws + w.layer[l - 1].h_all + (size_t)B * H * es);
     if ((rc = gemm_tn_full(ws + L.dgates, ws + L.h_all, dw_hh[l], G, H, TB, dt, ws + w.tn_scratch, acc, st, P.opt))) return rc;
     if ((rc = gemm_tn_full(ws + L.dgates, inp, dw_ih[l], G, I, TB, dt, ws + w.tn_scratch, acc, st, P.opt))) return rc;
@@ -820,10 +864,10 @@
       if ((rc = launch_transpose_cast(w_ih[l], G, I, ws + L.wiht, CSN_F32, st))) return rc;
     }
     if ((rc = launch_add_vec(b_ih[l], b_hh[l], (float*)(ws + L.bias), G, st))) return rc;
-    CSN_HIP_CHECK(hipMemsetAsync(ws + L.h_all, 0, (size_t)B * H * 4, st));
-    CSN_HIP_CHECK(hipMemsetAsync(ws + L.c_all, 0, (size_t)B * H * 4, st));
-  }
-  CSN_HIP_CHECK(hipMemsetAsync(ws + w.zero_fwd, 0, w.zero_fwd_bytes, st));
+    CSN_MEMSET(P, 0, (ws + L.h_all, 0, (size_t)B * H * 4, st));
+    CSN_MEMSET(P, 0, (ws + L.c_all, 0, (size_t)B * H * 4, st));
+  }
+  CSN_MEMSET(P, 0, (ws + w.zero_fwd, 0, w.zero_fwd_bytes, st));
   int n_launch = 0;
   if ((rc = prof_mark(g_prof, 0, st))) return rc;
   for (int l = 0; l < NL; ++l) {
@@ -868,7 +912,7 @@
   const int64_t G = 4 * (int64_t)H, TB = (int64_t)T * B;
   const int MTt = (B + 63) / 64, per = f32_persist_tiles_per_launch(H);
   int rc;
-  CSN_HIP_CHECK(hipMemsetAsync(ws + w.zero_bwd, 0, w.zero_bwd_bytes, st));
+  CSN_MEMSET(P, 1, (ws + w.zero_bwd, 0, w.zero_bwd_bytes, st));
   int n_launch = 0;
   if ((rc = prof_mark(g_prof, 2, st))) return rc;
   for (int l = NL - 1; l >= 0; --l) {
@@ -921,9 +965,10 @@
 }
 
 static int forward_persist(Plan& P, char* ws, const float* h0, const float* c0, int training, hipStream_t st, SideCtx* sc,
-                           hipStream_t side);
-
-static int forward_il(Plan& P, char* ws, const float* x, int64_t xsb, int64_t xst,
+                           hipStream_t side, bool fills_done);
+static bool fwd_grouped(const csnLstmPlan* P);
+
+static int forward_il(Plan& P, char* ws, const XIn& x,
                       const float* const* w_ih, const float* const* w_hh, const float* const* b_ih,
                       const float* const* b_hh, const float* h0, const float* c0, int training, csnStream_t stream) {
   const csnLstmDesc* d = &P.d;
@@ -951,7 +996,7 @@
     PrepJob& J = pa.job[pa.njobs++];
     J = PrepJob{kind, a_, b_, dst, n0, n1, n2, s0, s1, Hh, pr, pk, work, 0u, 0u};
   };
-  job(kPrepCastX, x, nullptr, ws + w.x_c, B, T, d->I, xsb, xst, 0, 0, 0, TB * d->I);
+  if (!x.in_place) job(kPrepCastX, (const float*)x.p, nullptr, ws + w.x_c, B, T, d->I, x.sb, x.st, 0, x.bf16, 0, TB * d->I);
   for (int l = 0; l < NL; ++l) {
     const LayerWs& L = w.layer[l];
     const int64_t I = l == 0 ? d->I : H;
@@ -963,10 +1008,10 @@
       job(kPrepBlockify, w_hh[l], nullptr, ws + L.whht_blk, H, G, 0, 1, H, H, 0, 1, H * G / 8);
     }
     if (!w.persist) {
-      CSN_HIP_CHECK(hipMemsetAsync(ws + L.hblk[0], 0, Bpad * H * 2, st));
-      CSN_HIP_CHECK(hipMemsetAsync(ws + L.hblk[1], 0, Bpad * H * 2, st));
-      CSN_HIP_CHECK(hipMemsetAsync(ws + L.h_all, 0, (size_t)B * H * 2, st));
-      CSN_HIP_CHECK(hipMemsetAsync(ws + L.c_all, 0, (size_t)B * H * 4, st));
+      CSN_MEMSET(P, 0, (ws + L.hblk[0], 0, Bpad * H * 2, st));
+      CSN_MEMSET(P, 0, (ws + L.hblk[1], 0, Bpad * H * 2, st));
+      CSN_MEMSET(P, 0, (ws + L.h_all, 0, (size_t)B * H * 2, st));
+      CSN_MEMSET(P, 0, (ws + L.c_all, 0, (size_t)B * H * 4, st));
       if (h0) {
         if ((rc = launch_blockify_x(h0 + (size_t)l * B * H, H, 0, B, 1, H, ws + L.hblk[0], st))) return rc;
         if ((rc = launch_cast(h0 + (size_t)l * B * H, ws + L.h_all, (int64_t)B * H, CSN_BF16, st))) return rc;
@@ -976,18 +1021,34 @@
     }
   }
   if (w.fuse_x) {
-    job(kPrepBlockifyX, x, nullptr, ws + w.x_blk, B, T, d->I, xsb, xst, (int64_t)Bpad, 0, 0, (int64_t)T * Bpad * d->I / 8);
+    job(kPrepBlockifyX, (const float*)x.p, nullptr, ws + w.x_blk, B, T, d->I, x.sb, x.st, (int64_t)Bpad, x.bf16, 0, (int64_t)T * Bpad * d->I / 8);
     job(kPrepBlockify, w_ih[0], nullptr, ws + w.wih0_blk, G, d->I, 0, d->I, 1, H, 1, 0, G * d->I / 8);
+  }
+  bool fills_done = false;
+  if (w.persist && !P.opt.no_step_fusions && fwd_grouped(&P)) {
+    auto fill = [&](size_t off, size_t bytes, unsigned pattern) {
+      job(kPrepFill, nullptr, nullptr, ws + off, (int64_t)bytes, (int64_t)pattern, 0, 0, 0, 0, 0, 0, (int64_t)(bytes / 16));
+    };
+    fill(w.zero_fwd, w.zero_fwd_bytes, 0u);
+    if (!w.fwd_ns && !P.opt.fwd_flags)
+      for (int l = 0; l < NL; ++l) fill(w.layer[l].h_blk_all, (size_t)4 * Bpad * H * 2, 0xffffffffu);
+    fills_done = true;
+    if (training && bwd_grouped(&P)) {
+      fill(w.zero_bwd, w.zero_bwd_bytes, 0u);
+      if (!P.opt.bwd_flags)
+        for (int l = 0; l < NL; ++l) fill(w.layer[l].dg_blk_all, (size_t)4 * Bpad * G * 2, 0xffffffffu);
+      P.call_of(ws).armed_T = T;
+    }
   }
   if (prep_rc != CSN_OK) return prep_rc;
   if ((rc = launch_prep_multi(pa, st))) return rc;
   if ((rc = mask_x(P, ws, st))) return rc;
   if (!w.fuse_x) {
-    if ((rc = gemm_nt(ws + w.x_c, ws + w.layer[0].wih, (const float*)(ws + w.layer[0].bias), ws + w.layer[0].xproj,
+    if ((rc = gemm_nt(P.x_img(ws), ws + w.layer[0].wih, (const float*)(ws + w.layer[0].bias), ws + w.layer[0].xproj,
                           TB, G, d->I, CSN_BF16, CSN_F32, 0, st, P.opt)))
       return rc;
   }
-  if (w.persist) return forward_persist(P, ws, h0, c0, training, st, sc, side);
+  if (w.persist) return forward_persist(P, ws, h0, c0, training, st, sc, side, fills_done);
   if (NL > 1 && (rc = hand_off(sc, st, side))) return rc;
 
   const int nch = (T + Cz - 1) / Cz;
@@ -1049,8 +1110,16 @@
   return CSN_OK;
 }
 
+static bool fwd_grouped(const csnLstmPlan* P) {
+  if (!P->w.persist) return false;
+  const int MT = (P->d.B + 63) / 64, nch = (P->d.T + P->opt.chunk - 1) / P->opt.chunk;
+  const int max_slots = P->d.L < nch ? P->d.L : nch;
+  const int fwd_slices = P->w.fwd_ns ? fwd_ns_slices(P->d.H) : fwd_persist_slices(P->d.H);
+  return max_slots <= 4 && max_slots * MT <= 8 && fwd_slices <= 32 && !P->opt.persist_streams;
+}
+
 static int forward_persist(Plan& P, char* ws, const float* h0, const float* c0, int training, hipStream_t st, SideCtx* sc,
-                           hipStream_t side) {
+                           hipStream_t side, bool fills_done) {
   const csnLstmDesc* d = &P.d;
   const WsLayout& w = P.w;
   Prof& g_prof = P.prof;
@@ -1060,7 +1129,7 @@
   const int Cz = P.opt.chunk;
   const int nch = (T + Cz - 1) / Cz;
   int rc;
-  CSN_HIP_CHECK(hipMemsetAsync(ws + w.zero_fwd, 0, w.zero_fwd_bytes, st));
+  if (!fills_done) CSN_MEMSET(P, 0, (ws + w.zero_fwd, 0, w.zero_fwd_bytes, st));
   auto fill_slot = [&](PersistFwdSlot& S, int l, int c) {
     const LayerWs& L = w.layer[l];
     S.w_blk = (const bf16_t*)(ws + L.whh_blk);
@@ -1099,9 +1168,9 @@
 #ifdef CSN_SLAB_TAGS
   if (a.data_polls && P.opt.tags_no_rearm) a.data_polls |= 4;
 #endif
-  if (a.data_polls)
+  if (a.data_polls && !fills_done)
     for (int l = 0; l < NL; ++l)
-      CSN_HIP_CHECK(hipMemsetAsync(ws + w.layer[l].h_blk_all, 0xff, (size_t)4 * Bpad * H * 2, st));
+      CSN_MEMSET(P, 0, (ws + w.layer[l].h_blk_all, 0xff, (size_t)4 * Bpad * H * 2, st));
   a.state = (h0 || c0) ? 1 : 0;
   if (a.state) P.state_seen = true;
   for (int l = 0; l < NL && P.state_seen; ++l) {
@@ -1110,24 +1179,22 @@
       if ((rc = launch_blockify_x(h0 + (size_t)l * B * H, H, 0, B, 1, H, ws + L.h_blk_all, st))) return rc;
       if ((rc = launch_cast(h0 + (size_t)l * B * H, ws + L.h_all, (int64_t)B * H, CSN_BF16, st))) return rc;
     } else {
-      if (a.state) CSN_HIP_CHECK(hipMemsetAsync(ws + L.h_blk_all, 0, (size_t)Bpad * H * 2, st));
-      CSN_HIP_CHECK(hipMemsetAsync(ws + L.h_all, 0, (size_t)B * H * 2, st));
+      if (a.state) CSN_MEMSET(P, 0, (ws + L.h_blk_all, 0, (size_t)Bpad * H * 2, st));
+      CSN_MEMSET(P, 0, (ws + L.h_all, 0, (size_t)B * H * 2, st));
     }
     if (c0)
       CSN_HIP_CHECK(hipMemcpyAsync(ws + L.c_all, c0 + (size_t)l * B * H, (size_t)B * H * 4, hipMemcpyDeviceToDevice, st));
     else
-      CSN_HIP_CHECK(hipMemsetAsync(ws + L.c_all, 0, (size_t)B * H * 4, st));
+      CSN_MEMSET(P, 0, (ws + L.c_all, 0, (size_t)B * H * 4, st));
   }
   int n_launch = 0;
   P.half_launches[0] = 0;
 
-  const int max_slots = NL < nch ? NL : nch;
   const int fwd_slices = w.fwd_ns ? fwd_ns_slices(H) : fwd_persist_slices(H);
   auto launch_fwd = [&](const PersistFwdArgs& args, hipStream_t on) {
     return w.fwd_ns ? launch_fwd_ns(args, on) : launch_fwd_persist(args, on);
   };
-  const bool grouped = max_slots <= 4 && max_slots * MT <= 8 && fwd_slices <= 32 &&
-                       !P.opt.persist_streams;
+  const bool grouped = fwd_grouped(&P);
   if (grouped) {
     const int ndiag = nch + NL - 1;
     const bool try_local = !P.opt.no_xcd_local;
@@ -1208,6 +1275,48 @@
                             const float* dc_n, float* const* dw_ih, float* const* dw_hh, float* const* db_ih,
                             float* const* db_hh, float* dx, hipStream_t st);
 
+static int weight_grads_il(Plan& P, char* ws, int l, float* const* dw_ih, float* const* dw_hh, float* const* db_ih,
+                           float* const* db_hh, hipStream_t on) {
+  const csnLstmDesc* d = &P.d;
+  const WsLayout& w = P.w;
+  const LayerWs& L = w.layer[l];
+  const int B = d->B, H = d->H;
+  const int64_t G = 4 * (int64_t)H, TB = (int64_t)d->T * B, I = l == 0 ? d->I : H;
+  const void* inp = l == 0 ? P.x_img(ws) : (const void*)((const bf16_t*)(ws + w.layer[l - 1].h_all) + (size_t)B * H);
+  float* slabs = (float*)(ws + w.tn_scratch);
+  const bool fused = !P.opt.no_step_fusions;
+  const int acc = P.grad_accumulate;
+  int S = 1, S2 = 1, r;
+  int cs_done = 0, S_cs = 1;
+  if ((r = launch_gemm_tn_slabs(ws + L.dgates, ws + L.h_all, slabs, G, H, TB, CSN_BF16, on, &S, (float*)(ws + w.colsum), &cs_done, P.opt))) return r;
+  S_cs = S;
+  float* slabs2 = slabs;
+  if (fused) {
+    slabs2 = (float*)(ws + w.tn_scratch + align_up((size_t)S * G * H * 4, 256));
+  } else {
+    if ((r = launch_reduce_slabs_unperm(slabs, G * H, S, H, H, dw_hh[l], nullptr, acc, on))) return r;
+    ++P.aux_launches[2];
+  }
+  if ((r = launch_gemm_tn_slabs(ws + L.dgates, inp, slabs2, G, I, TB, CSN_BF16, on, &S2, nullptr, nullptr, P.opt))) return r;
+  if (!fused) {
+    if ((r = launch_reduce_slabs_unperm(slabs2, G * I, S2, H, I, dw_ih[l], nullptr, acc, on))) return r;
+    ++P.aux_launches[2];
+  }
+  if (!cs_done) {
+    if ((r = launch_colsum_partial(ws + L.dgates, TB, G, CSN_BF16, ws + w.colsum, on))) return r;
+    S_cs = colsum_chunks();
+  }
+  ++P.aux_launches[2];
+  if (!fused) return launch_reduce_slabs_unperm((const float*)(ws + w.colsum), G, S_cs, H, 1, db_ih[l], db_hh[l], acc, on);
+  ReduceArgs ra{};
+  ra.njobs = 3;
+  ra.accumulate = acc;
+  ra.job[0] = ReduceJob{slabs, G * H, S, H, H, dw_hh[l], nullptr, 0u, 0u};
+  ra.job[1] = ReduceJob{slabs2, G * I, S2, H, I, dw_ih[l], nullptr, 0u, 0u};
+  ra.job[2] = ReduceJob{(const float*)(ws + w.colsum), G, S_cs, H, 1, db_ih[l], db_hh[l], 0u, 0u};
+  return launch_reduce_slabs_multi(ra, on);
+}
+
 static int backward_il(Plan& P, char* ws, const float* dy_last, const float* dy_tm, const float* dh_n, const float* dc_n,
                        float* const* dw_ih, float* const* dw_hh, float* const* db_ih, float* const* db_hh, float* dx,
                        csnStream_t stream) {
@@ -1232,34 +1341,13 @@
     if (dc_n)
       CSN_HIP_CHECK(hipMemcpyAsync(ws + L.dc_carry, dc_n + (size_t)l * B * H, (size_t)B * H * 4, hipMemcpyDeviceToDevice, st));
     else
-      CSN_HIP_CHECK(hipMemsetAsync(ws + L.dc_carry, 0, (size_t)B * H * 4, st));
-    CSN_HIP_CHECK(hipMemsetAsync(ws + L.dgblk[0], 0, Bpad * G * 2, st));
-    CSN_HIP_CHECK(hipMemsetAsync(ws + L.dgblk[1], 0, Bpad * G * 2, st));
+      CSN_MEMSET(P, 1, (ws + L.dc_carry, 0, (size_t)B * H * 4, st));
+    CSN_MEMSET(P, 1, (ws + L.dgblk[0], 0, Bpad * G * 2, st));
+    CSN_MEMSET(P, 1, (ws + L.dgblk[1], 0, Bpad * G * 2, st));
   }
   if ((rc = hand_off(sc, st, side))) return rc;
 
-  auto weight_grads = [&](int l) -> int {
-    const LayerWs& L = w.layer[l];
-    const int64_t I = l == 0 ? d->I : H;
-    const void* inp = l == 0 ? (const void*)(ws + w.x_c)
-                             : (const void*)((const bf16_t*)(ws + w.layer[l - 1].h_all) + (size_t)B * H);
-    float* slabs = (float*)(ws + w.tn_scratch);
-    const int acc = P.grad_accumulate;
-    int S = 1, r;
-    int cs_done = 0, S_cs = 1;
-    if ((r = launch_gemm_tn_slabs(ws + L.dgates, ws + L.h_all, slabs, G, H, TB, CSN_BF16, side, &S, (float*)(ws + w.colsum), &cs_done, P.opt))) return r;
-    S_cs = S;
-    if ((r = launch_reduce_slabs_unperm(slabs, G * H, S, H, H, dw_hh[l], nullptr, acc, side))) return r;
-    if ((r = launch_gemm_tn_slabs(ws + L.dgates, inp, slabs, G, I, TB, CSN_BF16, side, &S, nullptr, nullptr, P.opt))) return r;
-    if ((r = launch_reduce_slabs_unperm(slabs, G * I, S, H, I, dw_ih[l], nullptr, acc, side))) return r;
-    if (!cs_done) {
-      if ((r = launch_colsum_partial(ws + L.dgates, TB, G, CSN_BF16, ws + w.colsum, side))) return r;
-      S_cs = colsum_chunks();
-    }
-    if ((r = launch_reduce_slabs_unperm((const float*)(ws + w.colsum), G, S_cs, H, 1, db_ih[l], db_hh[l], acc, side)))
-      return r;
-    return CSN_OK;
-  };
+  auto weight_grads = [&](int l) -> int { return weight_grads_il(P, ws, l, dw_ih, dw_hh, db_ih, db_hh, side); };
 
   std::vector<hipEvent_t> dx_ready((size_t)NL * nch, nullptr);
   const int D = T + lag * (NL - 1);
@@ -1362,7 +1450,10 @@
   const int lag = beside ? 2 : 1;
   const int ndiag = nch + lag * (NL - 1);
   int rc;
-  CSN_HIP_CHECK(hipMemsetAsync(ws + w.zero_bwd, 0, w.zero_bwd_bytes, st));
+  Plan::WsCall& wc = P.call_of(ws);
+  const bool armed = wc.armed_T == T && !P.opt.no_step_fusions;
+  wc.armed_T = 0;
+  if (!armed) CSN_MEMSET(P, 1, (ws + w.zero_bwd, 0, w.zero_bwd_bytes, st));
   if (dc_n)
     for (int l = 0; l < NL; ++l)
       CSN_HIP_CHECK(hipMemcpyAsync(ws + w.layer[l].dc_carry, dc_n + (size_t)l * B * H, (size_t)B * H * 4,
@@ -1373,27 +1464,7 @@
   };
   const bool try_local = !P.opt.no_xcd_local;
 
-  auto weight_grads = [&](int l) -> int {
-    const LayerWs& L = w.layer[l];
-    const int64_t I = l == 0 ? d->I : H;
-    const void* inp = l == 0 ? (const void*)(ws + w.x_c)
-                             : (const void*)((const bf16_t*)(ws + w.layer[l - 1].h_all) + (size_t)B * H);
-    float* slabs = (float*)(ws + w.tn_scratch);
-    const int acc = P.grad_accumulate;
-    int S = 1, r;
-    int cs_done = 0, S_cs = 1;
-    if ((r = launch_gemm_tn_slabs(ws + L.dgates, ws + L.h_all, slabs, G, H, TB, CSN_BF16, st, &S, (float*)(ws + w.colsum), &cs_done, P.opt))) return r;
-    S_cs = S;
-    if ((r = launch_reduce_slabs_unperm(slabs, G * H, S, H, H, dw_hh[l], nullptr, acc, st))) return r;
-    if ((r = launch_gemm_tn_slabs(ws + L.dgates, inp, slabs, G, I, TB, CSN_BF16, st, &S, nullptr, nullptr, P.opt))) return r;
-    if ((r = launch_reduce_slabs_unperm(slabs, G * I, S, H, I, dw_ih[l], nullptr, acc, st))) return r;
-    if (!cs_done) {
-      if ((r = launch_colsum_partial(ws + L.dgates, TB, G, CSN_BF16, ws + w.colsum, st))) return r;
-      S_cs = colsum_chunks();
-    }
-    if ((r = launch_reduce_slabs_unperm((const float*)(ws + w.colsum), G, S_cs, H, 1, db_ih[l], db_hh[l], acc, st))) return r;
-    return CSN_OK;
-  };
+  auto weight_grads = [&](int l) -> int { return weight_grads_il(P, ws, l, dw_ih, dw_hh, db_ih, db_hh, st); };
   PersistBwdArgs a{};
   a.error_flag = (unsigned*)(ws + w.status);
   a.B = B; a.H = H; a.T = T; a.Bpad = Bpad; a.MT = MT;
@@ -1405,8 +1476,8 @@
   if (a.data_polls && P.opt.tags_no_rearm) a.data_polls |= 4;
 #endif
   P.dgates_copies = 2;
-  if (a.data_polls)
-    for (int l = 0; l < NL; ++l) CSN_HIP_CHECK(hipMemsetAsync(ws + w.layer[l].dg_blk_all, 0xff, (size_t)4 * Bpad * G * 2, st));
+  if (a.data_polls && !armed)
+    for (int l = 0; l < NL; ++l) CSN_MEMSET(P, 1, (ws + w.layer[l].dg_blk_all, 0xff, (size_t)4 * Bpad * G * 2, st));
   int n_launch = 0;
   P.half_launches[1] = 0;
   BesideGemm pending[3];
@@ -1519,14 +1590,19 @@
   return CSN_OK;
 }
 
-extern "C" int csn_lstm_forward(csnLstmPlan* Pp, const float* x, int64_t x_stride_b, int64_t x_stride_t,
-                                const float* const* w_ih, const float* const* w_hh, const float* const* b_ih,
-                                const float* const* b_hh, const float* h0, const float* c0, void* workspace,
-                                float* y_last, float* y_all, float* h_n, float* c_n, csnStream_t stream) {
+static int lstm_forward(csnLstmPlan* Pp, const void* x_any, int x_bf16, int64_t x_stride_b, int64_t x_stride_t,
+                        const float* const* w_ih, const float* const* w_hh, const float* const* b_ih,
+                        const float* const* b_hh, const float* h0, const float* c0, void* workspace,
+                        float* y_last, float* y_all, float* h_n, float* c_n, csnStream_t stream) {
   CSN_REQUIRE(Pp != nullptr, "csn_lstm_forward: null plan");
   Plan& P = *Pp;
   const csnLstmDesc* d = &P.d;
-  CSN_REQUIRE(x && w_ih && w_hh && b_ih && b_hh && workspace, "csn_lstm_forward: null pointer");
+  CSN_REQUIRE(!x_bf16 || d->dtype == CSN_BF16, "csn_lstm_forward_x16: bf16 input on an exact-float32 plan (pass float32 x)");
+  CSN_REQUIRE(!x_bf16 || (reinterpret_cast<uintptr_t>(x_any) & 1) == 0, "csn_lstm_forward_x16: x must be 2-byte aligned");
+  XIn x{x_any, x_stride_b, x_stride_t, x_bf16 != 0, false};
+  x.in_place = x.bf16 && x_any != nullptr && P.lengths.empty() && x_stride_t == (int64_t)d->B * d->I && x_stride_b == d->I &&
+               (reinterpret_cast<uintptr_t>(x_any) & 15) == 0;
+  CSN_REQUIRE(x.p && w_ih && w_hh && b_ih && b_hh && workspace, "csn_lstm_forward: null pointer");
   CSN_REQUIRE((reinterpret_cast<uintptr_t>(workspace) & 255) == 0, "csn_lstm_forward: workspace must be 256-B aligned");
   CSN_REQUIRE(y_last || y_all || h_n || c_n, "csn_lstm_forward: no output requested");
   {
@@ -1546,12 +1622,18 @@
   const int B = d->B, T = d->T, H = d->H, dt = d->dtype;
   const size_t es = dtype_size(dt);
   int rc;
+  P.aux_launches[0] = 0;
+  {
+    Plan::WsCall& wc = P.call_of(ws);
+    wc.x_img = x.in_place ? x.p : nullptr;
+    wc.armed_T = 0;
+  }
   if ((rc = upload_lengths(Pp, st))) return rc;
   if (P.dlen != nullptr) {
     if (P.t_eff > 0) {
       EffectiveT scope(P.d, P.t_eff);
-      rc = w.il ? forward_il(P, ws, x, x_stride_b, x_stride_t, w_ih, w_hh, b_ih, b_hh, h0, c0, training, stream)
-                : forward_v1(P, ws, x, x_stride_b, x_stride_t, w_ih, w_hh, b_ih, b_hh, h0, c0, training, stream);
+      rc = w.il ? forward_il(P, ws, x, w_ih, w_hh, b_ih, b_hh, h0, c0, training, stream)
+                : forward_v1(P, ws, x, w_ih, w_hh, b_ih, b_hh, h0, c0, training, stream);
       if (rc) return rc;
     } else {
       for (int l = 0; l < d->L; ++l) {
@@ -1592,11 +1674,11 @@
     return CSN_OK;
   }
   if (w.il)
-    rc = forward_il(P, ws, x, x_stride_b, x_stride_t, w_ih, w_hh, b_ih, b_hh, h0, c0, training, stream);
+    rc = forward_il(P, ws, x, w_ih, w_hh, b_ih, b_hh, h0, c0, training, stream);
   else if (w.f32_persist)
-    rc = forward_f32p(P, ws, x, x_stride_b, x_stride_t, w_ih, w_hh, b_ih, b_hh, training, stream);
+    rc = forward_f32p(P, ws, (const float*)x.p, x.sb, x.st, w_ih, w_hh, b_ih, b_hh, training, stream);
   else
-    rc = forward_v1(P, ws, x, x_stride_b, x_stride_t, w_ih, w_hh, b_ih, b_hh, h0, c0, training, stream);
+    rc = forward_v1(P, ws, x, w_ih, w_hh, b_ih, b_hh, h0, c0, training, stream);
   if (rc) return rc;
   for (int l = 0; l < d->L && (h_n || c_n); ++l) {
     const LayerWs& L = w.layer[l];
@@ -1618,6 +1700,22 @@
     CSN_LAUNCH_CHECK();
   }
   return CSN_OK;
+}
+
+extern "C" int csn_lstm_forward(csnLstmPlan* plan, const float* x, int64_t x_stride_b, int64_t x_stride_t,
+                                const float* const* w_ih, const float* const* w_hh, const float* const* b_ih,
+                                const float* const* b_hh, const float* h0, const float* c0, void* workspace,
+                                float* y_last, float* y_all, float* h_n, float* c_n, csnStream_t stream) {
+  return lstm_forward(plan, x, 0, x_stride_b, x_stride_t, w_ih, w_hh, b_ih, b_hh, h0, c0, workspace, y_last, y_all, h_n,
+                      c_n, stream);
+}
+
+extern "C" int csn_lstm_forward_x16(csnLstmPlan* plan, const void* x, int64_t x_stride_b, int64_t x_stride_t,
+                                    const float* const* w_ih, const float* const* w_hh, const float* const* b_ih,
+                                    const float* const* b_hh, const float* h0, const float* c0, void* workspace,
+                                    float* y_last, float* y_all, float* h_n, float* c_n, csnStream_t stream) {
+  return lstm_forward(plan, x, 1, x_stride_b, x_stride_t, w_ih, w_hh, b_ih, b_hh, h0, c0, workspace, y_last, y_all, h_n,
+                      c_n, stream);
 }
 
 extern "C" int csn_lstm_backward(csnLstmPlan* Pp, const float* dy_last, const float* dy_all, const float* dh_n,
@@ -1650,6 +1748,7 @@
   const int64_t TB = (int64_t)T * B;
 
   int rc;
+  P.aux_launches[1] = P.aux_launches[2] = 0;
   if ((rc = upload_lengths(Pp, st))) return rc;
   if (P.dlen != nullptr) {
     const int L_ = d->L, dt = d->dtype;
diff --git a/cerebralsignalnetworks_amd/csrc/lstm_cell_blk.h b/cerebralsignalnetworks_amd/csrc/lstm_cell_blk.h
--- a/cerebralsignalnetworks_amd/csrc/lstm_cell_blk.h
+++ b/cerebralsignalnetworks_amd/csrc/lstm_cell_blk.h
@@ -114,7 +114,7 @@
 int bwd_persist_slices(int H);
 int launch_bwd_persist(const PersistBwdArgs& a, hipStream_t st, const int* lengths = nullptr);
 
-enum { kPrepBlockify = 0, kPrepPermRows, kPrepTransPerm, kPrepBias, kPrepCastX, kPrepBlockifyX };
+enum { kPrepBlockify = 0, kPrepPermRows, kPrepTransPerm, kPrepBias, kPrepCastX, kPrepBlockifyX, kPrepFill };
 static constexpr int kPrepMaxJobs = 32;
 struct PrepJob {
   int kind;
@@ -143,5 +143,21 @@
 int launch_bias_perm_sum(const float* a, const float* b, int64_t H, float* dst, hipStream_t st);
 int launch_reduce_slabs_unperm(const float* slabs, int64_t slab_stride, int S, int64_t H, int64_t C, float* out,
                                float* out2, int accumulate, hipStream_t st);
+struct ReduceJob {
+  const float* slabs;
+  int64_t slab_stride;
+  int S;
+  int64_t H, C;
+  float* out;
+  float* out2;
+  unsigned blk_begin, blk_count;
+};
+static constexpr int kReduceMaxJobs = 4;
+struct ReduceArgs {
+  ReduceJob job[kReduceMaxJobs];
+  int njobs;
+  int accumulate;
+};
+int launch_reduce_slabs_multi(ReduceArgs& A, hipStream_t st);
 
 }
diff --git a/cerebralsignalnetworks_amd/csrc/lstm_cell_blk.hip b/cerebralsignalnetworks_amd/csrc/lstm_cell_blk.hip
--- a/cerebralsignalnetworks_amd/csrc/lstm_cell_blk.hip
+++ b/cerebralsignalnetworks_amd/csrc/lstm_cell_blk.hip
@@ -181,6 +181,21 @@
     case kPrepCastX: {
       const int64_t Bn = J.n0, Tn = J.n1, I = J.n2;
       bf16_t* dst = (bf16_t*)J.dst;
+      if (J.perm_r) {
+        const bf16_t* src = reinterpret_cast<const bf16_t*>(J.a);
+        if ((I & 7) == 0 && (J.s0 & 7) == 0 && (J.s1 & 7) == 0 && (reinterpret_cast<uintptr_t>(src) & 15) == 0) {
+          for (int64_t c = gid; c < Bn * Tn * I / 8; c += stride) {
+            const int64_t i = c * 8, i2 = i % I, r = i / I, b = r % Bn, t = r / Bn;
+            *reinterpret_cast<uint4*>(dst + i) = *reinterpret_cast<const uint4*>(src + b * J.s0 + t * J.s1 + i2);
+          }
+        } else {
+          for (int64_t i = gid; i < Bn * Tn * I; i += stride) {
+            const int64_t i2 = i % I, r = i / I, b = r % Bn, t = r / Bn;
+            dst[i] = src[b * J.s0 + t * J.s1 + i2];
+          }
+        }
+        break;
+      }
       if ((I & 7) == 0 && (J.s0 & 3) == 0 && (J.s1 & 3) == 0 && (reinterpret_cast<uintptr_t>(J.a) & 15) == 0) {
         for (int64_t c = gid; c < Bn * Tn * I / 8; c += stride) {
           const int64_t i = c * 8, i2 = i % I, r = i / I, b = r % Bn, t = r / Bn;
@@ -200,6 +215,28 @@
     case kPrepBlockifyX: {
       const int64_t Bn = J.n0, Tn = J.n1, I = J.n2, Bpad = J.H, per_t = Bpad * I / 8, kblocks = I >> 5;
       bf16_t* dst = (bf16_t*)J.dst;
+      if (J.perm_r) {
+        const bf16_t* src = reinterpret_cast<const bf16_t*>(J.a);
+        const bool vec = ((J.s0 | J.s1) & 7) == 0 && (reinterpret_cast<uintptr_t>(src) & 15) == 0;
+        for (int64_t ci = gid; ci < per_t * Tn; ci += stride) {
+          const int64_t t = ci / per_t, c = ci % per_t, blk = c >> 6, lane = c & 63;
+          const int64_t r = (blk / kblocks) * 16 + (lane & 15), k = (blk % kblocks) * 32 + 8 * (lane >> 4);
+          uint4 v = make_uint4(0u, 0u, 0u, 0u);
+          if (r < Bn) {
+            const bf16_t* sp = src + r * J.s0 + t * J.s1 + k;
+            if (vec) {
+              v = *reinterpret_cast<const uint4*>(sp);
+            } else {
+              bf16x8 e;
+#pragma unroll
+              for (int q = 0; q < 8; ++q) e[q] = sp[q];
+              v = *reinterpret_cast<const uint4*>(&e);
+            }
+          }
+          *reinterpret_cast<uint4*>(dst + ci * 8) = v;
+        }
+        break;
+      }
       for (int64_t ci = gid; ci < per_t * Tn; ci += stride) {
         const int64_t t = ci / per_t, c = ci % per_t, blk = c >> 6, lane = c & 63;
         const int64_t r = (blk / kblocks) * 16 + (lane & 15), k = (blk % kblocks) * 32 + 8 * (lane >> 4);
@@ -214,6 +251,13 @@
         }
         *reinterpret_cast<bf16x8*>(dst + ci * 8) = v;
       }
+      break;
+    }
+    case kPrepFill: {
+      const unsigned pat = (unsigned)J.n1;
+      const uint4 v = make_uint4(pat, pat, pat, pat);
+      uint4* dst = reinterpret_cast<uint4*>(J.dst);
+      for (int64_t i = gid; i < J.n0 / 16; i += stride) dst[i] = v;
       break;
     }
   }
@@ -287,6 +331,34 @@
 int launch_reduce_slabs_unperm(const float* slabs, int64_t slab_stride, int S, int64_t H, int64_t C, float* out,
                                float* out2, int accumulate, hipStream_t st) {
   reduce_slabs_unperm_kernel<<<cap_grid(4 * H * C), 256, 0, st>>>(slabs, slab_stride, S, H, C, out, out2, accumulate);
+  CSN_LAUNCH_CHECK();
+  return CSN_OK;
+}
+
+__global__ void __launch_bounds__(256) reduce_slabs_multi_kernel(ReduceArgs A) {
+  int j = 0;
+  while (j + 1 < A.njobs && blockIdx.x >= A.job[j + 1].blk_begin) ++j;
+  const ReduceJob& J = A.job[j];
+  const int64_t total = 4 * J.H * J.C, C = J.C;
+  const int64_t stride = (int64_t)J.blk_count * blockDim.x;
+  for (int64_t i = (int64_t)(blockIdx.x - J.blk_begin) * blockDim.x + threadIdx.x; i < total; i += stride) {
+    const int64_t n = i / C, c = i % C;
+    float acc = 0.0f;
+    for (int s = 0; s < J.S; ++s) acc += J.slabs[(int64_t)s * J.slab_stride + i];
+    const int64_t o = std_row(n, J.H) * C + c;
+    J.out[o] = A.accumulate ? J.out[o] + acc : acc;
+    if (J.out2 != nullptr) J.out2[o] = A.accumulate ? J.out2[o] + acc : acc;
+  }
+}
+int launch_reduce_slabs_multi(ReduceArgs& A, hipStream_t st) {
+  CSN_REQUIRE(A.njobs >= 1 && A.njobs <= kReduceMaxJobs, "launch_reduce_slabs_multi: %d jobs", A.njobs);
+  unsigned total = 0;
+  for (int j = 0; j < A.njobs; ++j) {
+    A.job[j].blk_begin = total;
+    A.job[j].blk_count = cap_grid(4 * A.job[j].H * A.job[j].C);
+    total += A.job[j].blk_count;
+  }
+  reduce_slabs_multi_kernel<<<total, 256, 0, st>>>(A);
   CSN_LAUNCH_CHECK();
   return CSN_OK;
 }
diff --git a/cerebralsignalnetworks_amd/lstm_model.py b/cerebralsignalnetworks_amd/lstm_model.py
--- a/cerebralsignalnetworks_amd/lstm_model.py
+++ b/cerebralsignalnetworks_amd/lstm_model.py
@@ -33,6 +33,7 @@
         plan = owner._checkout(x.shape[0], x.shape[1], x.device, training)
         y_last, y_all = plan.forward(x, w_ih, w_hh, b_ih, b_hh, want_all=want_all)
         ctx.lease, ctx.L, ctx.want_all = _Lease(plan), L, want_all
+        ctx.x_keep = x if training else None
         ctx.owner = owner
         ctx.need_dx = x.requires_grad
         ctx.x_shape = x.shape
@@ -60,6 +61,7 @@
         plan.set_grad_mode(accumulate)
         plan.backward(dy_last, dy_all if ctx.want_all else None, grads, dx=dx)
         ctx.lease.release()
+        ctx.x_keep = None
         if direct:
             return (dx, None, None, None, None, *([None] * (4 * L)))
         flat = [g for group in grads for g in group]
@@ -119,6 +121,7 @@
         plan.set_lengths(lengths)
         _, y_all, h_n, c_n = plan.forward(x, w_ih, w_hh, b_ih, b_hh, want_all=True, h0=h0, c0=c0, want_state=True)
         ctx.lease, ctx.L, ctx.owner = _Lease(plan), L, owner
+        ctx.x_keep = x if training else None
         ctx.lengths = lengths
         ctx.need = (x.requires_grad, h0 is not None and h0.requires_grad, c0 is not None and c0.requires_grad)
         ctx.x_shape = x.shape
@@ -150,6 +153,7 @@
         plan.set_lengths(ctx.lengths)
         plan.backward(None, dy_all, grads, dx=dx, dh_n=dh_n, dc_n=dc_n, dh0=dh0, dc0=dc0)
         ctx.lease.release()
+        ctx.x_keep = None
         if direct:
             return (dx, dh0, dc0, None, None, None, None, *([None] * (4 * L)))
         flat = [g for group in grads for g in group]
diff --git a/cerebralsignalnetworks_amd/trainer.py b/cerebralsignalnetworks_amd/trainer.py
--- a/cerebralsignalnetworks_amd/trainer.py
+++ b/cerebralsignalnetworks_amd/trainer.py
@@ -248,7 +248,10 @@
 
     def embed(self, eeg_bct):
         if self.preprocess:
-            return filters.eeg_bandpass_znorm(eeg_bct, self.sos, ddof=self.ddof, time_major=True).transpose(0, 1)
+            lstm = self._lstm
+            bf16 = lstm is not None and lstm.compute_dtype == torch.bfloat16 and eeg_bct.is_cuda
+            return filters.eeg_bandpass_znorm(eeg_bct, self.sos, ddof=self.ddof, time_major=True,
+                                              out_dtype=torch.bfloat16 if bf16 else torch.float32).transpose(0, 1)
         return eeg_bct.transpose(1, 2).contiguous()
 
     def compute_loss(self, out, targets, labels, epoch):
diff --git a/include/csn_hip.h b/include/csn_hip.h
--- a/include/csn_hip.h
+++ b/include/csn_hip.h
@@ -49,6 +49,7 @@
 int csn_lstm_plan_path(const csnLstmPlan* plan);
 int csn_lstm_plan_dgates_copies(const csnLstmPlan* plan);
 int csn_lstm_plan_half_tile_launches(const csnLstmPlan* plan, int which);
+int csn_lstm_plan_aux_launches(const csnLstmPlan* plan, int which);
 const char* csn_lstm_plan_kernel_name(const csnLstmPlan* plan, int which);
 size_t csn_lstm_workspace_bytes(const csnLstmDesc* d, int training);
 
@@ -61,6 +62,14 @@
                      const float* h0, const float* c0,
                      void* workspace, float* y_last, float* y_all,
                      float* h_n, float* c_n, csnStream_t stream);
+
+int csn_lstm_forward_x16(csnLstmPlan* plan,
+                         const void* x, int64_t x_stride_b, int64_t x_stride_t,
+                         const float* const* w_ih, const float* const* w_hh,
+                         const float* const* b_ih, const float* const* b_hh,
+                         const float* h0, const float* c0,
+                         void* workspace, float* y_last, float* y_all,
+                         float* h_n, float* c_n, csnStream_t stream);
 
 int csn_lstm_backward(csnLstmPlan* plan,
                       const float* dy_last, const float* dy_all,
```

New measurement: 27280. No clear change (-0.1%).
